# faris-k/self-supervised-wafermaps

Hardware: AMD Instinct MI355X
Metric: imgs/sec (SimCLR ResNet18, bs=256, 224^2) (higher is better)
Workload: dtype bf16; 1 GPU; SimCLR ResNet-18, 256 wafers/GPU/step, two 3x224x224 views, NT-Xent in-batch negatives, SGD (BASELINE.json configs[1]); per_gpu_batch=256, global_batch=256, parallelism=dp1, hip_graph=True, backward_stage_graphs=1, parallel_branches=two views through the backbone

## Files before the change

include/wafer_hip.h:

```cpp
#ifndef WAFER_HIP_H
#define WAFER_HIP_H

#include <stddef.h>
#include <stdint.h>

#ifdef __cplusplus
extern "C" {
#endif

#define WM_ABI_VERSION 4

#define WM_OK 0
#define WM_EINVAL (-1)
#define WM_EUNSUPPORTED (-2)
#define WM_EWORKSPACE (-3)
#define WM_EALIGN (-4)

#define WM_F32 0
#define WM_BF16 1

int wm_version(void);
const char* wm_error_string(int code);
int wm_fill_zero(void* p, size_t bytes, void* stream);
int wm_mean_f32(const float* x, long long n, float scale, int sqrt_of, float* out, void* stream);
// ... 8 lines not shown
#define WM_IMG_NCHW_F32 0
#define WM_IMG_NHWC_BF16 1
#define WM_IMG_HW_U8 2
#define WM_IMG_S2D_BF16 3

typedef struct WmViewParams {
  int32_t sample;
  int32_t out_slot;
  int32_t op;
  uint32_t noise_seed;
  float noise_p;
  int32_t dpw_h;
  int32_t dpw_w;
  int32_t rot90;
  int32_t vflip;
  int32_t hflip;
  int32_t crop;
  int32_t crop_i, crop_j, crop_h, crop_w;
  int32_t reserved;
} WmViewParams;

int wm_augment_views(const uint8_t* wafers, const int64_t* offsets, const int32_t* heights,
                     const int32_t* widths, int n_wafers, int max_wafer_elems,
                     const WmViewParams* params, int n_views, int img_size, int out_size,
                     int out_format, int normalize, float mean, float std, void* out,
                     void* stream);


size_t wm_knn_topk_workspace_bytes(int nq, int n, int d, int k);
int wm_knn_topk(const void* query, const void* bank, int nq, int n, int d, int dtype, int k,
                int bank_index_base, float* out_sim, int32_t* out_idx, void* workspace,
                size_t workspace_bytes, void* stream);

size_t wm_knn_topk_general_workspace_bytes(int nq, int n, int d, int k);
int wm_knn_topk_general(const float* query, const float* bank, const float* bias, int nq, int n, int d, int k,
                        int bank_index_base, float* out_sim, int32_t* out_idx, void* workspace,
                        size_t workspace_bytes, void* stream);
int wm_knn_topk_general_after(const float* query, const float* bank, const float* bias, int nq, int n, int d, int k,
                              int bank_index_base, const float* after_sim, const int32_t* after_idx, float* out_sim,
                              int32_t* out_idx, void* workspace, size_t workspace_bytes, void* stream);

int wm_knn_topk_many(const void* query, const void* bank, int nq, int n, int d, int dtype, int k, int bank_index_base,
                     float* out_sim, int32_t* out_idx, int batch, void* workspaces, size_t workspace_bytes_per_lane,
                     void* const* streams, int n_streams);

int wm_knn_merge(const float* in_sim, const int32_t* in_idx, int parts, int nq, int k,
                 float* out_sim, int32_t* out_idx, void* stream);

int wm_knn_vote(const float* sim, const int32_t* idx, const int64_t* bank_labels, long long n_labels, int nq, int k,
                int num_classes, float temperature, int64_t* pred_labels, float* scores,
                void* stream);

int wm_l2_normalize(const void* x, int in_dtype, int rows, int d, float eps, void* y,
                    int out_dtype, float* inv_norm, void* stream);
int wm_l2_normalize_bwd(const void* dy, int dy_dtype, const float* y, const float* inv_norm, int rows, int d,
                        void* dx, int out_dtype, const float* scale_dev, void* stream);

int wm_ntxent_fwd(const float* zn, const float* zall, int b_local, int b_global, int rank_offset,
                  int d, float temperature, float* lse, float* loss_rows, void* stream);
size_t wm_ntxent_bwd_workspace_bytes(int b_local, int b_global, int d);
int wm_ntxent_bwd(const float* zn, const float* zall, const float* lse_all, int b_local,
                  int b_global, int rank_offset, int d, float temperature, float grad_scale,
                  float* dzn, void* workspace, size_t workspace_bytes, void* stream);


int wm_conv2d_fwd(const void* x, const void* w_krsc, void* y, int N, int H, int W, int C, int K,
                  int R, int S, int P, int Q, int stride, int pad, void* stream);
int wm_conv2d_fwd_stats_tiles(int N, int H, int W, int C, int K, int R, int S, int P, int Q, int stride, int pad,
                              int rows_per_group);
int wm_conv2d_fwd_stats(const void* x, const void* w_krsc, void* y, int N, int H, int W, int C, int K,
                        int R, int S, int P, int Q, int stride, int pad, float* stat_part,
                        int stat_tiles, int rows_per_group, void* stream);
int wm_conv2d_dgrad(const void* dy, const void* w_crsk, void* dx, int N, int H, int W, int C, int K,
                    int R, int S, int P, int Q, int stride, int pad, void* stream);
int wm_conv2d_dgrad_add(const void* dy, const void* w_crsk, const void* residual, void* dx, int N, int H,
                        int W, int C, int K, int R, int S, int P, int Q, int stride, int pad, void* stream);
int wm_conv2d_dgrad_bnstat_ok(int N, int H, int W, int C, int K, int R, int S, int P, int Q, int stride, int pad,
                              int G);
int wm_conv2d_dgrad_bnstat(const void* dy, const void* w_crsk, const void* residual, void* dx, int N, int H, int W,
                           int C, int K, int R, int S, int P, int Q, int stride, int pad, const void* bn_y,
                           const void* relu_x, const void* relu_mask, const float* gamma, const float* beta,
                           const float* save_mean, const float* save_invstd, int G, float* stat_part, int stat_tiles,
                           void* stream);
int wm_conv2d_wgrad_splits(int N, int H, int W, int C, int K, int R, int S, int P, int Q, int stride, int pad);
int wm_conv2d_wgrad(const void* dy, const void* x, float* dw_slabs, int N, int H, int W, int C, int K,
                    int R, int S, int P, int Q, int stride, int pad, void* stream);
#define WM_ROUTE_F_STATS 1
#define WM_ROUTE_F_RESIDUAL 2
#define WM_ROUTE_F_BIAS 4
#define WM_ROUTE_F_BNB 8
#define WM_ROUTE_F_ACT 16
#define WM_ROUTE_PANEL 1
#define WM_ROUTE_STEM_PATCH 2
#define WM_ROUTE_WGRAD_PATCH64 3
#define WM_ROUTE_PATCH(MODE, BNB) (10 + 2 * (MODE) + ((BNB) ? 1 : 0))
#define WM_ROUTE_IGEMM(BN, CPT, MODE, EPI, BNB) \
  (10000 + ((BN) / 64) * 1000 + (CPT) * 100 + (MODE) * 10 + ((EPI) ? 2 : 0) + ((BNB) ? 1 : 0))
#define WM_ROUTE_WGRAD(BMO, CPT, NT, BIAS) (20000 + ((BMO) / 64) * 1000 + (CPT) * 100 + (NT) * 10 + ((BIAS) ? 1 : 0))
int wm_conv2d_route(int pass, int N, int H, int W, int C, int K, int R, int S, int P, int Q, int stride, int pad,
                    int flags, int group_arg);
int wm_conv2d_fwd_bias_res(const void* x, const void* w_krsc, const float* bias, const void* residual, void* y,
                           int N, int H, int W, int C, int K, int R, int S, int P, int Q, int stride, int pad,
                           void* stream);
int wm_conv2d_wgrad_bias(const void* dy, const void* x, float* dw_slabs, float* dbias_slabs, int N, int H, int W, int C,
                         int K, int R, int S, int P, int Q, int stride, int pad, void* stream);

int wm_linear_bias_gelu_fwd(const void* x, const void* w_krsc, const float* bias, void* pre_out, void* y, int rows,
                            int C, int K, void* stream);
int wm_linear_dgrad_gelu(const void* dy, const void* w_crsk, const void* pre, void* dx, int rows, int C, int K,
                         void* stream);

int wm_mlp_fused_fwd_ok(int rows, int C, int H);
int wm_mlp_fused_fwd(const void* x, const void* w1_krsc, const float* b1, const void* w2_krsc, const float* b2,
                     const void* residual, void* y, int rows, int C, int H, void* stream);
int wm_ln_linear_fwd_ok(int rows, int C, int N);
int wm_ln_linear_fwd(const void* x, const float* ln_gamma, const float* ln_beta, float ln_eps, const void* w_krsc,
                     const float* bias, void* y, int rows, int C, int N, void* stream);
int wm_ln_mlp_fused_fwd(const void* x, const float* ln_gamma, const float* ln_beta, float ln_eps, const void* w1_krsc,
                        const float* b1, const void* w2_krsc, const float* b2, const void* residual, void* y, int rows,
                        int C, int H, void* stream);

int wm_weights_prepare(const float* w_oihw, int K, int C, int R, int S, void* w_krsc, void* w_crsk,
                       void* stream);
typedef struct WmLayoutDesc {
  const float* w;
  uint16_t* krsc;
  uint16_t* crsk;
  float* ws;
  float* grad;
  int32_t K, C, RS, tiles_c, tile0, nsplit;
} WmLayoutDesc;
int wm_layouts_refresh(const WmLayoutDesc* descs_dev, int n_desc, int total_tiles, void* stream);
int wm_wgrad_fold(const WmLayoutDesc* descs_dev, int n_desc, int total_tiles, void* stream);

int wm_wgrad_finalize(const float* dw_slabs, int nsplit, int K, int C, int R, int S, float* grad_oihw,
                      int accumulate, void* stream);
int wm_stem_weights_prepare(const float* w_oihw, int K, void* w_s2d, void* stream);
int wm_stem_wgrad_finalize(const float* dw_s2d_slabs, int nsplit, int K, float* grad_oihw, int accumulate, void* stream);
int wm_image_to_s2d(const void* img, int fmt, int N, int H, int W, void* out, void* stream);
int wm_cast_f32_bf16(const float* x, long long n, void* y, void* stream);

size_t wm_bn_workspace_bytes(long long rows, int C, int G);
int wm_bn_train_fwd(const void* y, const void* residual, const float* gamma, const float* beta,
                    float* running_mean, float* running_var, long long* num_batches_tracked, long long rows, int C, int G, float eps,
                    float momentum, int relu, float* save_mean, float* save_invstd, void* out, void* relu_mask,
                    void* workspace, size_t workspace_bytes, void* stream);
int wm_bn_train_fwd_from_stats(const void* y, const void* residual, const float* gamma, const float* beta,
                               float* running_mean, float* running_var, long long* num_batches_tracked,
                               long long rows, int C, int G, float eps, float momentum, int relu, float* save_mean,
                               float* save_invstd,
                               void* out, void* relu_mask, const float* stat_part, int stat_tiles, void* workspace,
                               size_t workspace_bytes, void* stream);
int wm_bn_train_stats(const void* y, const float* gamma, const float* beta, float* running_mean,
                      float* running_var, long long* num_batches_tracked, long long rows, int C, int G, float eps, float momentum,
                      float* save_mean, float* save_invstd, float* scale, float* shift, const float* stat_part,
                      int stat_tiles, void* workspace, size_t workspace_bytes, void* stream);
int wm_bn_eval_scale_shift(const float* gamma, const float* beta, const float* running_mean,
                           const float* running_var, int C, float eps, float* scale, float* shift, void* stream);
int wm_bn_eval_fwd(const void* y, const void* residual, const float* gamma, const float* beta,
                   const float* running_mean, const float* running_var, long long rows, int C, float eps,
                   int relu, void* out, void* workspace, size_t workspace_bytes, void* stream);
int wm_bn_train_bwd(const void* y, const void* dout, const void* out_relu, int relu_from_y,
                    const float* gamma, const float* beta, const float* save_mean, const float* save_invstd,
                    long long rows, int C, int G, float* dgamma, float* dbeta, int accumulate, void* dy,
                    void* dz, void* workspace, size_t workspace_bytes, void* stream);
int wm_bn_train_bwd_from_stats(const void* y, const void* g, const float* gamma, const float* beta,
                               const float* save_mean, const float* save_invstd, long long rows, int C, int G,
                               float* dgamma, float* dbeta, int accumulate, void* dy, const float* stat_part,
                               int stat_tiles, void* workspace, size_t workspace_bytes, void* stream);
int wm_bn_sync_fwd_sums(const void* y, long long rows, int C, int G, const float* stat_part, int stat_tiles,
                        float* sums, void* workspace, size_t workspace_bytes, void* stream);
int wm_bn_sync_fwd_apply(const void* y, const void* residual, const float* gamma, const float* beta,
                         float* running_mean, float* running_var, long long* num_batches_tracked, long long rows, int C,
                         int G, long long group_count, float eps, float momentum, int relu, float* save_mean,
                         float* save_invstd, void* out, const float* sums, void* workspace, size_t workspace_bytes,
                         void* stream);
int wm_bn_sync_bwd_sums(const void* y, const void* dout, const void* out_relu, int relu_from_y, const float* gamma,
                        const float* beta, const float* save_mean, const float* save_invstd, long long rows, int C,
                        int G, float* dgamma, float* dbeta, int accumulate, float* sums, void* workspace,
                        size_t workspace_bytes, void* stream);
int wm_bn_sync_bwd_apply(const void* y, const void* dout, const void* out_relu, int relu_from_y, const float* gamma,
                         const float* beta, const float* save_mean, const float* save_invstd, long long rows, int C,
                         int G, long long group_count, const float* sums, void* dy, void* dz, void* workspace,
                         size_t workspace_bytes, void* stream);
int wm_bn_relu_maxpool_bwd(const void* y, const void* ysel, const void* pooled_dy, const void* pool_idx, int N,
                           int H, int W, int C, const float* gamma, const float* beta, const float* save_mean,
                           const float* save_invstd, int G, float* dgamma, float* dbeta, int accumulate,
                           void* dy, void* workspace, size_t workspace_bytes, void* stream);
int wm_add_bf16(const void* a, const void* b, long long n, void* out, void* stream);

int wm_maxpool3x3s2_fwd(const void* x, int N, int H, int W, int C, void* y, void* idx, void* stream);
int wm_bn_relu_maxpool3x3s2_fwd(const void* x, const float* scale, const float* shift, int N, int H, int W, int C,
                                int G, void* y, void* idx, void* xsel, void* stream);
int wm_maxpool3x3s2_bwd(const void* dy, const void* idx, int N, int H, int W, int C, void* dx, void* stream);
int wm_gap_fwd(const void* x, int N, int HW, int C, void* y, void* stream);
int wm_gap_bwd(const void* dy, int N, int HW, int C, void* dx, void* stream);

int wm_sgd_step(float* params, const float* grads, float* momentum_buf, long long n, const float* hyper,
                void* stream);

int wm_cross_entropy_fwd_bwd(const void* logits, int dtype, const long long* labels, const float* weight, int B, int C,
                             float* acc2, float* dlogits, void* stream);
int wm_bce_logits_fwd_bwd(const void* logits, int dtype, const float* target, const float* pos_weight, int B, int C,
                          float* loss, float* dlogits, void* stream);

int wm_neg_cosine_fwd_bwd(const void* x0, const void* x1, int dtype, int B, int D, float eps, float* loss, float* dx0,
                          float* dx1, void* stream);

size_t wm_dcl_workspace_bytes(int B);
int wm_dcl_fwd_bwd(const float* z0, const float* z1, int B, int D, float temperature, float sigma, int weighted,
                   float* loss, float* dz0, float* dz1, void* workspace, size_t workspace_bytes, void* stream);

int wm_barlow_twins_fwd_bwd(const float* raw_cc, int D, float scale, float lambda, float diag_weight, float* loss,
                            float* draw_cc, void* stream);
int wm_center_columns(const void* z, const float* mean, long long rows, int C, void* out, void* stream);
int wm_vicreg_variance(const float* var_biased, int N, int D, float eps, float* loss, float* coef, void* stream);

int wm_sinkhorn(const void* out, int dtype, int B, int K, float eps, int iters, float* Q, float* workspace,
                void* stream);

int wm_ntxent_bank_fwd_bwd(const float* q, const float* kpos, const float* bank, int B, int D, int K,
                           float temperature, float* loss, float* dq, float* dk, void* stream);


int wm_layernorm_fwd(const void* x, const float* gamma, const float* beta, float eps, long long rows, int C,
                     void* y, float* mean, float* rstd, void* stream);
int wm_layernorm_bwd(const void* x, const void* dy, const float* gamma, const float* mean, const float* rstd,
                     long long rows, int C, void* dx, float* dgamma, float* dbeta, void* stream);
int wm_layernorm_bwd_add(const void* x, const void* dy, const float* gamma, const float* mean, const float* rstd,
                         long long rows, int C, const void* dres, void* dx, float* dgamma, float* dbeta, void* stream);
int wm_colsum_blocks(long long rows, int C);
int wm_bias_act_bwd_parts(const void* x, const float* bias, const void* dy, int act, long long rows, int C, void* dx,
                          float* part, void* stream);
int wm_layernorm_bwd_blocks(long long rows, int C);
int wm_layernorm_bwd_parts(const void* x, const void* dy, const float* gamma, const float* mean, const float* rstd,
                           long long rows, int C, const void* dres, void* dx, float* part, void* stream);

#define WM_ACT_NONE 0
#define WM_ACT_GELU 1
#define WM_ACT_RELU 2
#define WM_ACT_MISH 3
int wm_bias_act_fwd(const void* x, const float* bias, const void* residual, int act, long long rows, int C,
                    void* y, void* stream);
int wm_bias_act_bwd(const void* x, const float* bias, const void* dy, int act, long long rows, int C, void* dx,
                    float* dbias, void* stream);
int wm_colsum_bf16(const void* x, long long rows, int C, float* out, int accumulate, void* stream);

int wm_tokens_assemble(const void* patches, const float* cls, const float* pos, int N, int np, int D, void* tokens,
                       void* stream);
int wm_patchify(const void* images, int N, int S, int p, void* rows, void* stream);

int wm_attention_fwd(const void* qkv, int B, int S, int H, int head_dim, float scale, void* out, float* lse,
// ... 157 lines not shown
```

self-supervised-wafermaps_amd/_lib.py:

```python
from __future__ import annotations

import ctypes
import os
from ctypes import c_char_p, c_double, c_float, c_int, c_int32, c_longlong, c_size_t, c_uint32, c_void_p
from pathlib import Path

_HERE = Path(__file__).resolve().parent
LIB_PATH = Path(os.environ["WM_HIP_LIB"]) if os.environ.get("WM_HIP_LIB") else _HERE / "libwafer_hip.so"

WM_F32, WM_BF16 = 0, 1
WM_AUG_NONE, WM_AUG_DIENOISE, WM_AUG_DPW, WM_AUG_MEDIAN3 = 0, 1, 2, 3
WM_IMG_NCHW_F32, WM_IMG_NHWC_BF16, WM_IMG_HW_U8, WM_IMG_S2D_BF16 = 0, 1, 2, 3


class WaferHipError(RuntimeError):
    pass


class WmViewParams(ctypes.Structure):

    _fields_ = [
        ("sample", c_int32),
        ("out_slot", c_int32),
        ("op", c_int32),
# ... 32 lines not shown
    "wm_f32_conv2d_dgrad": (c_int, [c_void_p, c_void_p, c_void_p, c_int, c_int, c_int, c_int, c_int, c_int, c_int, c_int, c_int,
                                    c_int, c_int, c_void_p, c_size_t, c_void_p]),
    "wm_f32_conv2d_wgrad_workspace_bytes": (c_size_t, [c_int] * 7),
    "wm_f32_conv2d_wgrad": (c_int, [c_void_p, c_void_p, c_void_p, c_int, c_int, c_int, c_int, c_int, c_int, c_int, c_int, c_int,
                                    c_int, c_int, c_void_p, c_size_t, c_void_p]),
    "wm_f32_colsum": (c_int, [c_void_p, c_longlong, c_int, c_void_p, c_void_p]),
    "wm_f32_bn_bwd": (c_int, [c_void_p, c_void_p, c_void_p, c_void_p, c_void_p, c_void_p, c_longlong, c_int, c_int, c_void_p,
                              c_void_p, c_void_p, c_void_p, c_void_p, c_size_t, c_void_p]),
    "wm_f32_maxpool3x3s2_bwd": (c_int, [c_void_p, c_void_p, c_int, c_int, c_int, c_int, c_void_p, c_void_p]),
    "wm_f32_gap_bwd": (c_int, [c_void_p, c_int, c_int, c_int, c_void_p, c_void_p]),
    "wm_f32_layernorm_bwd_workspace_bytes": (c_size_t, [c_longlong, c_int]),
    "wm_f32_layernorm_bwd": (c_int, [c_void_p, c_void_p, c_void_p, c_float, c_longlong, c_int, c_void_p, c_void_p, c_void_p,
                                     c_void_p, c_size_t, c_void_p]),
    "wm_f32_bias_act_bwd": (c_int, [c_void_p, c_void_p, c_void_p, c_int, c_longlong, c_int, c_void_p, c_void_p]),
    "wm_f32_attention_bwd": (c_int, [c_void_p, c_void_p, c_void_p, c_int, c_int, c_int, c_int, c_float, c_void_p, c_void_p]),
    "wm_f32_loss_bwd": (c_int, [c_void_p, c_void_p, c_longlong, c_int, c_double, c_void_p, c_void_p, c_void_p]),
    "wm_version": (c_int, []),
    "wm_error_string": (c_char_p, [c_int]),
    "wm_ln_linear_fwd_ok": (c_int, [c_int, c_int, c_int]),
    "wm_ln_linear_fwd": (c_int, [c_void_p, c_void_p, c_void_p, c_float, c_void_p, c_void_p, c_void_p, c_int, c_int, c_int, c_void_p]),
    "wm_ln_mlp_fused_fwd": (c_int, [c_void_p, c_void_p, c_void_p, c_float, c_void_p, c_void_p, c_void_p, c_void_p, c_void_p,
                                    c_void_p, c_int, c_int, c_int, c_void_p]),
    "wm_layernorm_bwd_blocks": (c_int, [c_longlong, c_int]),
    "wm_layernorm_bwd_parts": (c_int, [c_void_p, c_void_p, c_void_p, c_void_p, c_void_p, c_longlong, c_int, c_void_p, c_void_p,
                                       c_void_p, c_void_p]),
    "wm_colsum_blocks": (c_int, [c_longlong, c_int]),
    "wm_bias_act_bwd_parts": (c_int, [c_void_p, c_void_p, c_void_p, c_int, c_longlong, c_int, c_void_p, c_void_p, c_void_p]),
    "wm_scale_bf16": (c_int, [c_void_p, c_longlong, c_void_p, c_void_p, c_void_p]),
    "wm_fill_zero": (c_int, [c_void_p, c_size_t, c_void_p]),
    "wm_mean_f32": (c_int, [c_void_p, c_longlong, c_float, c_int, c_void_p, c_void_p]),
    "wm_augment_views": (
        c_int,
        [c_void_p, c_void_p, c_void_p, c_void_p, c_int, c_int, c_void_p, c_int, c_int, c_int, c_int,
         c_int, c_float, c_float, c_void_p, c_void_p],
    ),
    "wm_knn_topk_workspace_bytes": (c_size_t, [c_int, c_int, c_int, c_int]),
    "wm_knn_topk": (
        c_int,
        [c_void_p, c_void_p, c_int, c_int, c_int, c_int, c_int, c_int, c_void_p, c_void_p, c_void_p,
         c_size_t, c_void_p],
    ),
    "wm_knn_topk_many": (
        c_int,
        [c_void_p, c_void_p, c_int, c_int, c_int, c_int, c_int, c_int, c_void_p, c_void_p, c_int, c_void_p, c_size_t,
         c_void_p, c_int],
    ),
    "wm_knn_merge": (c_int, [c_void_p, c_void_p, c_int, c_int, c_int, c_void_p, c_void_p, c_void_p]),
    "wm_knn_vote": (
        c_int,
        [c_void_p, c_void_p, c_void_p, c_longlong, c_int, c_int, c_int, c_float, c_void_p, c_void_p, c_void_p],
    ),
    "wm_l2_normalize": (c_int, [c_void_p, c_int, c_int, c_int, c_float, c_void_p, c_int, c_void_p, c_void_p]),
    "wm_l2_normalize_bwd": (c_int, [c_void_p, c_int, c_void_p, c_void_p, c_int, c_int, c_void_p, c_int, c_void_p, c_void_p]),
    "wm_ntxent_fwd": (
        c_int,
        [c_void_p, c_void_p, c_int, c_int, c_int, c_int, c_float, c_void_p, c_void_p, c_void_p],
    ),
    "wm_ntxent_bwd_workspace_bytes": (c_size_t, [c_int, c_int, c_int]),
    "wm_ntxent_bwd": (
        c_int,
        [c_void_p, c_void_p, c_void_p, c_int, c_int, c_int, c_int, c_float, c_float, c_void_p, c_void_p, c_size_t,
         c_void_p],
    ),
    "wm_conv2d_fwd": (c_int, [c_void_p, c_void_p, c_void_p, c_int, c_int, c_int, c_int, c_int, c_int, c_int, c_int, c_int, c_int, c_int, c_void_p]),
    "wm_conv2d_fwd_stats": (c_int, [c_void_p, c_void_p, c_void_p, c_int, c_int, c_int, c_int, c_int, c_int, c_int, c_int, c_int, c_int, c_int, c_void_p, c_int, c_int, c_void_p]),
    "wm_conv2d_dgrad": (c_int, [c_void_p, c_void_p, c_void_p, c_int, c_int, c_int, c_int, c_int, c_int, c_int, c_int, c_int, c_int, c_int, c_void_p]),
    "wm_conv2d_dgrad_add": (c_int, [c_void_p, c_void_p, c_void_p, c_void_p, c_int, c_int, c_int, c_int, c_int, c_int, c_int, c_int, c_int, c_int, c_int, c_void_p]),
    "wm_conv2d_wgrad": (c_int, [c_void_p, c_void_p, c_void_p, c_int, c_int, c_int, c_int, c_int, c_int, c_int, c_int, c_int, c_int, c_int, c_void_p]),
    "wm_conv2d_fwd_bias_res": (c_int, [c_void_p, c_void_p, c_void_p, c_void_p, c_void_p, c_int, c_int, c_int, c_int, c_int,
                                       c_int, c_int, c_int, c_int, c_int, c_int, c_void_p]),
    "wm_conv2d_wgrad_bias": (c_int, [c_void_p, c_void_p, c_void_p, c_void_p, c_int, c_int, c_int, c_int, c_int, c_int, c_int,
                                     c_int, c_int, c_int, c_int, c_void_p]),
    "wm_weights_prepare": (c_int, [c_void_p, c_int, c_int, c_int, c_int, c_void_p, c_void_p, c_void_p]),
    "wm_wgrad_finalize": (c_int, [c_void_p, c_int, c_int, c_int, c_int, c_int, c_void_p, c_int, c_void_p]),
    "wm_conv2d_wgrad_splits": (c_int, [c_int] * 11),
    "wm_conv2d_route": (c_int, [c_int] * 14),
    "wm_mlp_fused_fwd_ok": (c_int, [c_int, c_int, c_int]),
    "wm_mlp_fused_fwd": (c_int, [c_void_p, c_void_p, c_void_p, c_void_p, c_void_p, c_void_p, c_void_p, c_int, c_int, c_int,
                                c_void_p]),
    "wm_conv2d_fwd_stats_tiles": (c_int, [c_int] * 12),
    "wm_conv2d_dgrad_bnstat_ok": (c_int, [c_int] * 12),
    "wm_conv2d_dgrad_bnstat": (c_int, [c_void_p, c_void_p, c_void_p, c_void_p] + [c_int] * 11 +
                               [c_void_p, c_void_p, c_void_p, c_void_p, c_void_p, c_void_p, c_void_p, c_int, c_void_p, c_int, c_void_p]),
    "wm_bn_train_bwd_from_stats": (
        c_int,
        [c_void_p, c_void_p, c_void_p, c_void_p, c_void_p, c_void_p, c_longlong, c_int, c_int, c_void_p, c_void_p, c_int,
         c_void_p, c_void_p, c_int, c_void_p, c_size_t, c_void_p],
    ),
    "wm_bn_sync_fwd_sums": (c_int, [c_void_p, c_longlong, c_int, c_int, c_void_p, c_int, c_void_p, c_void_p, c_size_t, c_void_p]),
    "wm_bn_sync_fwd_apply": (
        c_int,
        [c_void_p, c_void_p, c_void_p, c_void_p, c_void_p, c_void_p, c_void_p, c_longlong, c_int, c_int, c_longlong,
         c_float, c_float, c_int, c_void_p, c_void_p, c_void_p, c_void_p, c_void_p, c_size_t, c_void_p],
    ),
    "wm_bn_sync_bwd_sums": (
        c_int,
        [c_void_p, c_void_p, c_void_p, c_int, c_void_p, c_void_p, c_void_p, c_void_p, c_longlong, c_int, c_int,
         c_void_p, c_void_p, c_int, c_void_p, c_void_p, c_size_t, c_void_p],
    ),
    "wm_bn_sync_bwd_apply": (
        c_int,
        [c_void_p, c_void_p, c_void_p, c_int, c_void_p, c_void_p, c_void_p, c_void_p, c_longlong, c_int, c_int,
         c_longlong, c_void_p, c_void_p, c_void_p, c_void_p, c_size_t, c_void_p],
    ),
    "wm_stem_weights_prepare": (c_int, [c_void_p, c_int, c_void_p, c_void_p]),
    "wm_stem_wgrad_finalize": (c_int, [c_void_p, c_int, c_int, c_void_p, c_int, c_void_p]),
    "wm_image_to_s2d": (c_int, [c_void_p, c_int, c_int, c_int, c_int, c_void_p, c_void_p]),
    "wm_cast_f32_bf16": (c_int, [c_void_p, c_longlong, c_void_p, c_void_p]),
    "wm_bn_workspace_bytes": (c_size_t, [c_longlong, c_int, c_int]),
    "wm_bn_train_fwd": (
        c_int,
        [c_void_p, c_void_p, c_void_p, c_void_p, c_void_p, c_void_p, c_void_p, c_longlong, c_int, c_int, c_float, c_float,
         c_int, c_void_p, c_void_p, c_void_p, c_void_p, c_void_p, c_size_t, c_void_p],
    ),
    "wm_bn_train_fwd_from_stats": (
        c_int,
        [c_void_p, c_void_p, c_void_p, c_void_p, c_void_p, c_void_p, c_void_p, c_longlong, c_int, c_int, c_float, c_float,
         c_int, c_void_p, c_void_p, c_void_p, c_void_p, c_void_p, c_int, c_void_p, c_size_t, c_void_p],
    ),
    "wm_bn_train_stats": (
        c_int,
        [c_void_p, c_void_p, c_void_p, c_void_p, c_void_p, c_void_p, c_longlong, c_int, c_int, c_float, c_float, c_void_p,
         c_void_p, c_void_p, c_void_p, c_void_p, c_int, c_void_p, c_size_t, c_void_p],
    ),
    "wm_bn_eval_scale_shift": (c_int, [c_void_p, c_void_p, c_void_p, c_void_p, c_int, c_float, c_void_p, c_void_p, c_void_p]),
    "wm_bn_eval_fwd": (
        c_int,
        [c_void_p, c_void_p, c_void_p, c_void_p, c_void_p, c_void_p, c_longlong, c_int, c_float, c_int, c_void_p,
         c_void_p, c_size_t, c_void_p],
    ),
    "wm_bn_train_bwd": (
        c_int,
        [c_void_p, c_void_p, c_void_p, c_int, c_void_p, c_void_p, c_void_p, c_void_p, c_longlong, c_int, c_int,
         c_void_p, c_void_p, c_int, c_void_p, c_void_p, c_void_p, c_size_t, c_void_p],
    ),
    "wm_bn_relu_maxpool_bwd": (
        c_int,
        [c_void_p, c_void_p, c_void_p, c_void_p, c_int, c_int, c_int, c_int, c_void_p, c_void_p, c_void_p, c_void_p, c_int,
         c_void_p, c_void_p, c_int, c_void_p, c_void_p, c_size_t, c_void_p],
    ),
    "wm_add_bf16": (c_int, [c_void_p, c_void_p, c_longlong, c_void_p, c_void_p]),
    "wm_maxpool3x3s2_fwd": (c_int, [c_void_p, c_int, c_int, c_int, c_int, c_void_p, c_void_p, c_void_p]),
    "wm_bn_relu_maxpool3x3s2_fwd": (
        c_int, [c_void_p, c_void_p, c_void_p, c_int, c_int, c_int, c_int, c_int, c_void_p, c_void_p, c_void_p, c_void_p]),
    "wm_maxpool3x3s2_bwd": (c_int, [c_void_p, c_void_p, c_int, c_int, c_int, c_int, c_void_p, c_void_p]),
    "wm_gap_fwd": (c_int, [c_void_p, c_int, c_int, c_int, c_void_p, c_void_p]),
    "wm_gap_bwd": (c_int, [c_void_p, c_int, c_int, c_int, c_void_p, c_void_p]),
    "wm_sgd_step": (c_int, [c_void_p, c_void_p, c_void_p, c_longlong, c_void_p, c_void_p]),
    "wm_cross_entropy_fwd_bwd": (c_int, [c_void_p, c_int, c_void_p, c_void_p, c_int, c_int, c_void_p, c_void_p, c_void_p]),
    "wm_bce_logits_fwd_bwd": (c_int, [c_void_p, c_int, c_void_p, c_void_p, c_int, c_int, c_void_p, c_void_p, c_void_p]),
    "wm_neg_cosine_fwd_bwd": (c_int, [c_void_p, c_void_p, c_int, c_int, c_int, c_float, c_void_p, c_void_p, c_void_p,
                                      c_void_p]),
    "wm_barlow_twins_fwd_bwd": (c_int, [c_void_p, c_int, c_float, c_float, c_float, c_void_p, c_void_p, c_void_p]),
    "wm_center_columns": (c_int, [c_void_p, c_void_p, c_longlong, c_int, c_void_p, c_void_p]),
    "wm_vicreg_variance": (c_int, [c_void_p, c_int, c_int, c_float, c_void_p, c_void_p, c_void_p]),
    "wm_lars_step": (c_int, [c_void_p, c_void_p, c_void_p, c_void_p, c_int, c_void_p, c_void_p, c_void_p]),
    "wm_sinkhorn": (c_int, [c_void_p, c_int, c_int, c_int, c_float, c_int, c_void_p, c_void_p, c_void_p]),
    "wm_dcl_workspace_bytes": (c_size_t, [c_int]),
    "wm_dcl_fwd_bwd": (c_int, [c_void_p, c_void_p, c_int, c_int, c_float, c_float, c_int, c_void_p, c_void_p, c_void_p,
                               c_void_p, c_size_t, c_void_p]),
    "wm_ntxent_bank_fwd_bwd": (c_int, [c_void_p, c_void_p, c_void_p, c_int, c_int, c_int, c_float, c_void_p, c_void_p,
                                       c_void_p, c_void_p]),
    "wm_layernorm_fwd": (c_int, [c_void_p, c_void_p, c_void_p, c_float, c_longlong, c_int, c_void_p, c_void_p, c_void_p,
                                 c_void_p]),
    "wm_layernorm_bwd": (c_int, [c_void_p, c_void_p, c_void_p, c_void_p, c_void_p, c_longlong, c_int, c_void_p, c_void_p,
                                 c_void_p, c_void_p]),
    "wm_layernorm_bwd_add": (c_int, [c_void_p, c_void_p, c_void_p, c_void_p, c_void_p, c_longlong, c_int, c_void_p,
                                     c_void_p, c_void_p, c_void_p, c_void_p]),
    "wm_bias_act_fwd": (c_int, [c_void_p, c_void_p, c_void_p, c_int, c_longlong, c_int, c_void_p, c_void_p]),
    "wm_bias_act_bwd": (c_int, [c_void_p, c_void_p, c_void_p, c_int, c_longlong, c_int, c_void_p, c_void_p, c_void_p]),
# ... 145 lines not shown
```

self-supervised-wafermaps_amd/csrc/bn.hip:

```cpp
#include "common.h"

namespace {

constexpr int BN_THREADS = 256;

__device__ __forceinline__ void unpack8(const uint4 v, float (&f)[8]) {
  f[0] = bf2f((uint16_t)(v.x & 0xffff)); f[1] = bf2f((uint16_t)(v.x >> 16));
  f[2] = bf2f((uint16_t)(v.y & 0xffff)); f[3] = bf2f((uint16_t)(v.y >> 16));
  f[4] = bf2f((uint16_t)(v.z & 0xffff)); f[5] = bf2f((uint16_t)(v.z >> 16));
  f[6] = bf2f((uint16_t)(v.w & 0xffff)); f[7] = bf2f((uint16_t)(v.w >> 16));
}
__device__ __forceinline__ uint4 pack8(const float (&f)[8]) {
  return make_uint4(pack_bf2(f[0], f[1]), pack_bf2(f[2], f[3]), pack_bf2(f[4], f[5]), pack_bf2(f[6], f[7]));
}

struct PoolSrc {
  const uint16_t* dy;
  const uint8_t* idx;
  int H, W, P, Q;
};

__device__ __forceinline__ void pool_grad8(const PoolSrc& ps, uint32_t row, int C, int c0, float (&g)[8]) {
  const uint32_t hw = (uint32_t)(ps.H * ps.W);
  const int n = (int)(row / hw);
// ... 246 lines not shown
  }
  if (owner) {
    if (running_mean) running_mean[c] = rm;
    if (running_var) running_var[c] = rv;
  }
}

__global__ __launch_bounds__(1024) void bn_sums_finalize(float* __restrict__ part, int nblk, int G, int C,
                                                          float* __restrict__ sums) {
  __shared__ double red[2][2][32][33];
  const int bl = threadIdx.x >> 5, cl = threadIdx.x & 31;
  const int c = blockIdx.x * 32 + cl;
  const bool owner = bl == 0 && c < C;
  for (int g0 = 0; g0 < G; g0 += 2) {
    const int ng = G - g0 < 2 ? G - g0 : 2;
    double a[2], b[2];
    finalize_sums2(part, nblk, g0, ng, C, c, bl, cl, red, a, b);
    if (owner) {
      for (int u = 0; u < ng; ++u) {
        sums[((size_t)(g0 + u) * 2 + 0) * C + c] = (float)a[u];
        sums[((size_t)(g0 + u) * 2 + 1) * C + c] = (float)b[u];
      }
    }
  }
}

__global__ void bn_eval_params(const float* __restrict__ gamma, const float* __restrict__ beta,
                               const float* __restrict__ running_mean,
                               const float* __restrict__ running_var, float eps, int C,
                               float* __restrict__ scale, float* __restrict__ shift) {
  for (int c = threadIdx.x; c < C; c += blockDim.x) {
    const float is = 1.0f / sqrtf(running_var[c] + eps);
    const float sc = (gamma ? gamma[c] : 1.f) * is;
    scale[c] = sc;
    shift[c] = (beta ? beta[c] : 0.f) - running_mean[c] * sc;
  }
}

template <bool POW2>
__global__ __launch_bounds__(BN_THREADS) void bn_apply(const uint16_t* __restrict__ y,
                                                       const uint16_t* __restrict__ residual,
                                                       const float* __restrict__ scale,
                                                       const float* __restrict__ shift,
                                                       long long rows, int C, int rows_per_group,
                                                       int relu, int cshift, uint16_t* __restrict__ out,
                                                       uint8_t* __restrict__ relu_mask) {
  const int cpr = C >> 3;
  const long long total = rows * cpr;
  int cur_g = -1;
  float sc[8], sh[8];
  for (long long p = (long long)blockIdx.x * BN_THREADS + threadIdx.x; p < total;
       p += (long long)gridDim.x * BN_THREADS) {
    long long row;
    int c0, g;
    if (POW2) {
      row = p >> cshift;
      c0 = (int)(p & (cpr - 1)) * 8;
      g = 0;
      for (long long lim = rows_per_group; row >= lim; lim += rows_per_group) ++g;
    } else {
      row = p / cpr;
      c0 = (int)(p - row * cpr) * 8;
      g = (int)(row / rows_per_group);
    }
    if (!POW2 || g != cur_g) {
      const float4 sa = *reinterpret_cast<const float4*>(scale + (size_t)g * C + c0);
      const float4 sb = *reinterpret_cast<const float4*>(scale + (size_t)g * C + c0 + 4);
      const float4 ha = *reinterpret_cast<const float4*>(shift + (size_t)g * C + c0);
      const float4 hb = *reinterpret_cast<const float4*>(shift + (size_t)g * C + c0 + 4);
      sc[0] = sa.x; sc[1] = sa.y; sc[2] = sa.z; sc[3] = sa.w; sc[4] = sb.x; sc[5] = sb.y; sc[6] = sb.z; sc[7] = sb.w;
      sh[0] = ha.x; sh[1] = ha.y; sh[2] = ha.z; sh[3] = ha.w; sh[4] = hb.x; sh[5] = hb.y; sh[6] = hb.z; sh[7] = hb.w;
      cur_g = g;
    }
    float f[8];
    unpack8(*reinterpret_cast<const uint4*>(y + row * C + c0), f);
#pragma unroll
    for (int e = 0; e < 8; ++e) f[e] = fmaf(f[e], sc[e], sh[e]);
    if (residual) {
      float r[8];
      unpack8(*reinterpret_cast<const uint4*>(residual + row * C + c0), r);
#pragma unroll
      for (int e = 0; e < 8; ++e) f[e] += r[e];
    }
    if (relu) {
#pragma unroll
      for (int e = 0; e < 8; ++e) f[e] = fmaxf(f[e], 0.f);
    }
    const uint4 pk = pack8(f);
    *reinterpret_cast<uint4*>(out + row * C + c0) = pk;
    if (relu_mask != nullptr) {
      float r8[8];
      unpack8(pk, r8);
      uint32_t m = 0;
#pragma unroll
      for (int e = 0; e < 8; ++e) m |= (r8[e] > 0.f ? 1u : 0u) << e;
      relu_mask[row * cpr + (c0 >> 3)] = (uint8_t)m;
    }
  }
}

__global__ __launch_bounds__(1024) void bn_bwd_finalize(
    float* __restrict__ part, int nblk, int G, int C, int rows_per_group,
    const float* __restrict__ gamma, const float* __restrict__ beta, const float* __restrict__ mean,
    const float* __restrict__ invstd, float* __restrict__ dgamma, float* __restrict__ dbeta, int accumulate,
    float* __restrict__ coef, int fx) {
  __shared__ double red[2][2][32][33];
  const int bl = threadIdx.x >> 5, cl = threadIdx.x & 31;
  const int c = blockIdx.x * 32 + cl;
  const bool owner = bl == 0 && c < C;
  double tg = 0.0, tb = 0.0;
  for (int g0 = 0; g0 < G; g0 += 2) {
    const int ng = G - g0 < 2 ? G - g0 : 2;
    double s1v[2], s2v[2];
    finalize_sums2(part, nblk, g0, ng, C, c, bl, cl, red, s1v, s2v);
    if (owner) {
      for (int u = 0; u < ng; ++u) {
        const int g = g0 + u;
        double s1 = s1v[u], s2 = s2v[u];
        if (fx) {
          s2 = (double)invstd[(size_t)g * C + c] * s2;
        }
        tb += s1;
        tg += s2;
        const float is = invstd[(size_t)g * C + c];
        const float mu = mean[(size_t)g * C + c];
        const float sc = (gamma ? gamma[c] : 1.f) * is;
        coef[((size_t)g * 7 + 0) * C + c] = mu;
        coef[((size_t)g * 7 + 1) * C + c] = is;
        coef[((size_t)g * 7 + 2) * C + c] = sc;
        coef[((size_t)g * 7 + 3) * C + c] = (float)(s1 / rows_per_group);
        coef[((size_t)g * 7 + 4) * C + c] = (float)(s2 / rows_per_group);
        coef[((size_t)g * 7 + 5) * C + c] = sc;
        coef[((size_t)g * 7 + 6) * C + c] = (beta ? beta[c] : 0.f) - mu * sc;
      }
    }
  }
  if (owner) {
    if (dgamma) dgamma[c] = (accumulate ? dgamma[c] : 0.f) + (float)tg;
    if (dbeta) dbeta[c] = (accumulate ? dbeta[c] : 0.f) + (float)tb;
  }
}

template <bool POW2, int FORM>
__global__ __launch_bounds__(BN_THREADS, FORM == 0 ? 4 : 1) void bn_bwd_apply(const uint16_t* __restrict__ y,
                                                           const uint16_t* __restrict__ dout,
                                                           const uint16_t* __restrict__ out,
                                                           const float* __restrict__ coef,
                                                           long long rows, int C, int rows_per_group,
                                                           int remask, int cshift, uint16_t* __restrict__ dy,
                                                           uint16_t* __restrict__ dz, const PoolSrc ps) {
  const int cpr = C >> 3;
  const long long total = rows * cpr;
  int cur_g = -1;
  constexpr int NK = FORM == 0 ? 5 : 7;
  float k[NK][8];
  for (long long p = (long long)blockIdx.x * BN_THREADS + threadIdx.x; p < total;
       p += (long long)gridDim.x * BN_THREADS) {
    long long row;
    int c0, g;
    if (POW2) {
      row = p >> cshift;
      c0 = (int)(p & (cpr - 1)) * 8;
      g = 0;
      for (long long lim = rows_per_group; row >= lim; lim += rows_per_group) ++g;
    } else {
      row = p / cpr;
      c0 = (int)(p - row * cpr) * 8;
      g = (int)(row / rows_per_group);
    }
    if (!POW2 || g != cur_g) {
      const float* cf = coef + (size_t)g * 7 * C + c0;
#pragma unroll
      for (int t = 0; t < NK; ++t) {
        const float4 a = *reinterpret_cast<const float4*>(cf + (size_t)t * C);
        const float4 b = *reinterpret_cast<const float4*>(cf + (size_t)t * C + 4);
        k[t][0] = a.x; k[t][1] = a.y; k[t][2] = a.z; k[t][3] = a.w;
        k[t][4] = b.x; k[t][5] = b.y; k[t][6] = b.z; k[t][7] = b.w;
      }
      cur_g = g;
    }
    const size_t off = row * C + c0;
    float fy[8], fd[8];
    unpack8(*reinterpret_cast<const uint4*>(y + off), fy);
    if constexpr (FORM == 2) pool_grad8(ps, (uint32_t)row, C, c0, fd);
    else unpack8(*reinterpret_cast<const uint4*>(dout + off), fd);
    if constexpr (FORM != 0) {
      if (out) {
        float fo[8];
        unpack8(*reinterpret_cast<const uint4*>(out + off), fo);
#pragma unroll
        for (int e = 0; e < 8; ++e) fd[e] = fo[e] > 0.f ? fd[e] : 0.f;
      }
      if (!out && remask) {
#pragma unroll
        for (int e = 0; e < 8; ++e) fd[e] = bf2f(f2bf(fmaf(fy[e], k[NK - 2][e], k[NK - 1][e]))) > 0.f ? fd[e] : 0.f;
      }
      if (dz) *reinterpret_cast<uint4*>(dz + off) = pack8(fd);
    }
    float r[8];
#pragma unroll
    for (int e = 0; e < 8; ++e) {
      const float xh = (fy[e] - k[0][e]) * k[1][e];
      r[e] = k[2][e] * (fd[e] - k[3][e] - xh * k[4][e]);
    }
    *reinterpret_cast<uint4*>(dy + off) = pack8(r);
  }
}

__global__ __launch_bounds__(BN_THREADS) void bn_pool_bwd_apply(const uint16_t* __restrict__ y,
                                                                const float* __restrict__ coef, int n_coef, int N, int C,
                                                                int imgs_per_group, int remask,
                                                                uint16_t* __restrict__ dy, const PoolSrc ps,
                                                                const WmDiv d_cpr, const WmDiv d_wb, const WmDiv d_ha,
                                                                const WmDiv d_ipg) {
  const uint32_t cpr = (uint32_t)C >> 3;
  const uint32_t HA = (uint32_t)ps.H >> 1, WB = (uint32_t)ps.W >> 1;
  const uint32_t total = (uint32_t)N * HA * WB * cpr;
  extern __shared__ __attribute__((aligned(16))) float pool_coef[];
  for (int i = threadIdx.x; i < n_coef; i += BN_THREADS) pool_coef[i] = coef[i];
  __syncthreads();
  for (uint32_t t = blockIdx.x * BN_THREADS + threadIdx.x; t < total; t += gridDim.x * BN_THREADS) {
    uint32_t rc, rb, ra;
    uint32_t u = wm_divmod(t, d_cpr, rc);
    const int c0 = (int)rc * 8;
    u = wm_divmod(u, d_wb, rb);
    const int n = (int)wm_divmod(u, d_ha, ra);
    const int b = (int)rb, a = (int)ra;
    const int g = (int)wm_div((uint32_t)n, d_ipg);
    const float* kk = pool_coef + (size_t)g * 7 * C + c0;
    auto krow = [&](int q, float (&v)[8]) {
      const float4 lo = *reinterpret_cast<const float4*>(kk + q * C);
      const float4 hi = *reinterpret_cast<const float4*>(kk + q * C + 4);
      v[0] = lo.x; v[1] = lo.y; v[2] = lo.z; v[3] = lo.w; v[4] = hi.x; v[5] = hi.y; v[6] = hi.z; v[7] = hi.w;
    };
    uint2 pk[4];
    uint4 dv[4];
    bool wok[4];
#pragma unroll
    for (int j = 0; j < 4; ++j) {
      const int p = a + (j >> 1), q = b + (j & 1);
      wok[j] = p < ps.P && q < ps.Q;
      const int pc = p < ps.P ? p : ps.P - 1, qc = q < ps.Q ? q : ps.Q - 1;
      const size_t o = ((size_t)(n * ps.P + pc) * ps.Q + qc) * C + c0;
      pk[j] = *reinterpret_cast<const uint2*>(ps.idx + o);
      dv[j] = *reinterpret_cast<const uint4*>(ps.dy + o);
    }
    float dw[4][8];
#pragma unroll
    for (int j = 0; j < 4; ++j) unpack8(dv[j], dw[j]);
#pragma unroll
    for (int pix = 0; pix < 4; ++pix) {
      const int dh = pix >> 1, dwp = pix & 1;
      float fd[8];
#pragma unroll
      for (int e = 0; e < 8; ++e) fd[e] = 0.f;
#pragma unroll
      for (int j = 0; j < 4; ++j) {
        const int kh = dh + 1 - 2 * (j >> 1), kw = dwp + 1 - 2 * (j & 1);
        if (kh < 0 || kw < 0) continue;
        const int code = kh * 3 + kw;
        if (wok[j]) {
#pragma unroll
          for (int e = 0; e < 8; ++e) {
            const int ie = (int)(((e < 4 ? pk[j].x : pk[j].y) >> (8 * (e & 3))) & 0xff);
            fd[e] += ie == code ? dw[j][e] : 0.f;
          }
        }
      }
#pragma unroll
      for (int e = 0; e < 8; ++e) fd[e] = bf2f(f2bf(fd[e]));
      const size_t off = ((size_t)(n * ps.H + 2 * a + dh) * ps.W + 2 * b + dwp) * C + c0;
      float fy[8];
      unpack8(*reinterpret_cast<const uint4*>(y + off), fy);
      if (remask) {
        float k5[8], k6[8];
        krow(5, k5);
        krow(6, k6);
#pragma unroll
        for (int e = 0; e < 8; ++e) fd[e] = bf2f(f2bf(fmaf(fy[e], k5[e], k6[e]))) > 0.f ? fd[e] : 0.f;
      }
      float r[8], k0[8], k1[8];
      krow(0, k0);
      krow(1, k1);
#pragma unroll
      for (int e = 0; e < 8; ++e) r[e] = (fy[e] - k0[e]) * k1[e];
      krow(4, k0);
      krow(3, k1);
#pragma unroll
      for (int e = 0; e < 8; ++e) r[e] = fd[e] - k1[e] - r[e] * k0[e];
      krow(2, k0);
#pragma unroll
// ... 28 lines not shown

constexpr int STAT_SLOTS_DIRECT = 512, STAT_SLOTS_REDUCED = 128;
inline size_t stat_scratch_floats(int T, int G, int C) {
  return T > STAT_SLOTS_DIRECT ? (size_t)G * STAT_SLOTS_REDUCED * 2 * C : 0;
}

inline const float* stat_partials(const float* stat_part, int T, int G, int C, float* scratch, int* nblk, hipStream_t st) {
  if (T <= STAT_SLOTS_DIRECT) {
    *nblk = T;
    return stat_part;
  }
  int R = 1;
  while ((T + R - 1) / R > STAT_SLOTS_REDUCED) R *= 2;
  const int To = (T + R - 1) / R;
  const long long total = (long long)G * To * 2 * C;
  stats_prereduce<<<wm_cdiv(total, BN_THREADS), BN_THREADS, 0, st>>>(stat_part, T, R, To, G * 2 * C, 2 * C, scratch);
  *nblk = To;
  return scratch;
}

inline bool chunk_pow2(int C, int* shift) {
  const int cpr = C >> 3;
  if (cpr <= 0 || (cpr & (cpr - 1)) || BN_THREADS % cpr) return false;
  int sft = 0;
  while ((1 << sft) < cpr) ++sft;
  *shift = sft;
  return true;
}

__global__ __launch_bounds__(BN_THREADS) void add_bf16_kernel(const uint16_t* __restrict__ a,
                                                              const uint16_t* __restrict__ b,
                                                              long long n8, uint16_t* __restrict__ o) {
  for (long long p = (long long)blockIdx.x * BN_THREADS + threadIdx.x; p < n8;
       p += (long long)gridDim.x * BN_THREADS) {
    float fa[8], fb[8];
    unpack8(reinterpret_cast<const uint4*>(a)[p], fa);
    unpack8(reinterpret_cast<const uint4*>(b)[p], fb);
#pragma unroll
    for (int e = 0; e < 8; ++e) fa[e] += fb[e];
    reinterpret_cast<uint4*>(o)[p] = pack8(fa);
  }
}

inline int reduce_blocks(int rows_per_group, int C) {
  const int tpr = C >> 3;
  const int rpp = BN_THREADS / tpr > 0 ? BN_THREADS / tpr : 1;
  int nblk = wm_cdiv(rows_per_group, rpp * 16);
  if (nblk > 256) nblk = 256;
  if (nblk < 1) nblk = 1;
  return nblk;
}

inline int stream_grid(long long items) {
  long long b = (items + BN_THREADS - 1) / BN_THREADS;
  if (b > 256 * 16) b = 256 * 16;
  if (b < 1) b = 1;
  return (int)b;
}

inline const uint16_t* bf16(const void* p) { return static_cast<const uint16_t*>(p); }
inline uint16_t* bf16(void* p) { return static_cast<uint16_t*>(p); }

inline void launch_bn_apply(const uint16_t* y, const uint16_t* residual, const float* scale, const float* shift,
                            long long rows, int C, int rpg, int relu, uint16_t* out, hipStream_t st,
                            uint8_t* relu_mask = nullptr) {
  int csh = 0;
  const auto kernel = chunk_pow2(C, &csh) ? bn_apply<true> : bn_apply<false>;
  kernel<<<stream_grid(rows * (C >> 3)), BN_THREADS, 0, st>>>(y, residual, scale, shift, rows, C, rpg, relu, csh, out,
                                                              relu_mask);
}

inline void launch_bn_bwd_apply(int form, const uint16_t* y, const uint16_t* dout, const uint16_t* out_relu,
                                const float* coef, long long rows, int C, int rpg, bool remask, uint16_t* dy, uint16_t* dz,
                                const PoolSrc& ps, hipStream_t st) {
  int csh = 0;
  const bool pow2 = chunk_pow2(C, &csh);
  const auto kernel = form == 0   ? (pow2 ? bn_bwd_apply<true, 0> : bn_bwd_apply<false, 0>)
                      : form == 1 ? (pow2 ? bn_bwd_apply<true, 1> : bn_bwd_apply<false, 1>)
                                  : (pow2 ? bn_bwd_apply<true, 2> : bn_bwd_apply<false, 2>);
  kernel<<<stream_grid(rows * (C >> 3)), BN_THREADS, 0, st>>>(y, dout, out_relu, coef, rows, C, rpg, remask ? 1 : 0, csh, dy,
                                                              dz, ps);
}

constexpr int BN_WIDE_MAX_C = 16384;

__global__ __launch_bounds__(BN_THREADS) void bn_col_fwd(const uint16_t* __restrict__ y, const uint16_t* __restrict__ res,
                                                         const float* __restrict__ gamma, const float* __restrict__ beta,
                                                         float* __restrict__ rmean, float* __restrict__ rvar,
                                                         long long* __restrict__ num_batches_tracked, int rpg,
                                                         int C, int G, float eps, float momentum, int relu, int training,
                                                         float* __restrict__ save_mean, float* __restrict__ save_invstd,
                                                         uint16_t* __restrict__ out) {
  const int c = blockIdx.x * BN_THREADS + threadIdx.x;
  if (training && num_batches_tracked != nullptr && c == 0)
    atomicAdd(reinterpret_cast<unsigned long long*>(num_batches_tracked), (unsigned long long)G);
  if (c >= C) return;
  const float ga = gamma ? gamma[c] : 1.f, be = beta ? beta[c] : 0.f;
  for (int g = 0; g < G; ++g) {
    const size_t base = (size_t)g * rpg;
    float mu, is;
    if (training) {
      float s = 0.f;
      for (int r = 0; r < rpg; ++r) s += bf2f(y[(base + r) * C + c]);
      mu = s / (float)rpg;
      float q = 0.f;
      for (int r = 0; r < rpg; ++r) {
        const float d = bf2f(y[(base + r) * C + c]) - mu;
        q = fmaf(d, d, q);
      }
      const float var = q / (float)rpg;
      is = rsqrtf(var + eps);
      save_mean[(size_t)g * C + c] = mu;
      save_invstd[(size_t)g * C + c] = is;
      if (rmean) {
        rmean[c] = (1.f - momentum) * rmean[c] + momentum * mu;
        rvar[c] = (1.f - momentum) * rvar[c] + momentum * (rpg > 1 ? var * (float)rpg / (float)(rpg - 1) : var);
      }
    } else {
      mu = rmean[c];
      is = rsqrtf(rvar[c] + eps);
    }
    const float sc = ga * is, sh = be - mu * sc;
    for (int r = 0; r < rpg; ++r) {
      const size_t o = (base + r) * C + c;
      float v = fmaf(bf2f(y[o]), sc, sh);
      if (res) v += bf2f(res[o]);
      if (relu) v = fmaxf(v, 0.f);
      out[o] = f2bf(v);
    }
  }
}

__global__ __launch_bounds__(BN_THREADS) void bn_col_bwd(const uint16_t* __restrict__ y, const uint16_t* __restrict__ dout,
                                                         const uint16_t* __restrict__ out_relu, int remask,
                                                         const float* __restrict__ gamma, const float* __restrict__ beta,
                                                         const float* __restrict__ mean, const float* __restrict__ invstd,
                                                         int rpg, int C, int G, float* __restrict__ dgamma,
                                                         float* __restrict__ dbeta, int accumulate,
                                                         uint16_t* __restrict__ dy, uint16_t* __restrict__ dz) {
  const int c = blockIdx.x * BN_THREADS + threadIdx.x;
  if (c >= C) return;
  const float ga = gamma ? gamma[c] : 1.f, be = beta ? beta[c] : 0.f;
  float dg = 0.f, db = 0.f;
  for (int g = 0; g < G; ++g) {
    const size_t base = (size_t)g * rpg;
    const float mu = mean[(size_t)g * C + c], is = invstd[(size_t)g * C + c];
    const float sc = ga * is, sh = be - mu * sc;
    float s1 = 0.f, s2 = 0.f;
    for (int r = 0; r < rpg; ++r) {
      const size_t o = (base + r) * C + c;
      const float yv = bf2f(y[o]);
      float d = bf2f(dout[o]);
      if (out_relu) d = bf2f(out_relu[o]) > 0.f ? d : 0.f;
      else if (remask) d = bf2f(f2bf(fmaf(yv, sc, sh))) > 0.f ? d : 0.f;
      s1 += d;
      s2 = fmaf(d, (yv - mu) * is, s2);
    }
    dg += s2;
    db += s1;
    const float c1 = s1 / (float)rpg, c2 = s2 / (float)rpg;
    for (int r = 0; r < rpg; ++r) {
      const size_t o = (base + r) * C + c;
      const float yv = bf2f(y[o]);
      float d = bf2f(dout[o]);
      if (out_relu) d = bf2f(out_relu[o]) > 0.f ? d : 0.f;
      else if (remask) d = bf2f(f2bf(fmaf(yv, sc, sh))) > 0.f ? d : 0.f;
// ... 219 lines not shown
                           stream);
}

extern "C" int wm_bn_train_stats(const void* y, const float* gamma, const float* beta, float* running_mean,
                                 float* running_var, long long* num_batches_tracked, long long rows, int C, int G, float eps, float momentum,
                                 float* save_mean, float* save_invstd, float* scale, float* shift, const float* stat_part,
                                 int stat_tiles, void* workspace, size_t workspace_bytes, void* stream) {
  WM_REQUIRE(y && save_mean && save_invstd && scale && shift && workspace, WM_EINVAL);
  const int rc = bn_shape_check(rows, C, G);
  if (rc != WM_OK) return rc;
  WM_REQUIRE(!stat_part || stat_tiles > 0, WM_EINVAL);
  WM_REQUIRE(workspace_bytes >= fwd_partials_bytes(stat_part, stat_tiles, rows, C, G), WM_EWORKSPACE);
  return bn_fwd_stats(bf16(y), stat_part, stat_tiles, gamma, beta, running_mean, running_var, num_batches_tracked,
                      (int)(rows / G), C, G, eps, momentum, save_mean, save_invstd, scale, shift,
                      static_cast<float*>(workspace), static_cast<hipStream_t>(stream));
}

extern "C" int wm_bn_eval_scale_shift(const float* gamma, const float* beta, const float* running_mean,
                                      const float* running_var, int C, float eps, float* scale, float* shift,
                                      void* stream) {
  WM_REQUIRE(running_mean && running_var && scale && shift && C > 0, WM_EINVAL);
  launch_eval_params(gamma, beta, running_mean, running_var, eps, C, scale, shift, static_cast<hipStream_t>(stream));
  WM_LAUNCH_CHECK();
  return WM_OK;
}

extern "C" int wm_bn_eval_fwd(const void* y_, const void* residual, const float* gamma, const float* beta,
                              const float* running_mean, const float* running_var, long long rows, int C,
                              float eps, int relu, void* out_, void* workspace, size_t workspace_bytes,
                              void* stream) {
  WM_REQUIRE(y_ && out_ && running_mean && running_var && workspace, WM_EINVAL);
  const int rc = bn_shape_check(rows, C, 1);
  if (rc != WM_OK) return rc;
  WM_REQUIRE(workspace_bytes >= (size_t)2 * C * sizeof(float), WM_EWORKSPACE);
  hipStream_t st = static_cast<hipStream_t>(stream);
  const uint16_t *y = bf16(y_), *res = bf16(residual);
  uint16_t* out = bf16(out_);
  if (bn_wide(rows, C, 1)) {
    bn_col_fwd<<<wm_cdiv(C, BN_THREADS), BN_THREADS, 0, st>>>(y, res, gamma, beta, const_cast<float*>(running_mean),
                                                              const_cast<float*>(running_var), nullptr, (int)rows, C, 1, eps,
                                                              0.f, relu, 0, nullptr, nullptr, out);
    WM_LAUNCH_CHECK();
    return WM_OK;
  }
  float* scale = static_cast<float*>(workspace);
  float* shift = scale + C;
  launch_eval_params(gamma, beta, running_mean, running_var, eps, C, scale, shift, st);
  WM_LAUNCH_CHECK();
  launch_bn_apply(y, res, scale, shift, rows, C, (int)(rows < (1ll << 31) - 1 ? rows : (1ll << 31) - 1), relu, out, st);
  WM_LAUNCH_CHECK();
  return WM_OK;
}

extern "C" int wm_bn_train_bwd(const void* y, const void* dout, const void* out_relu, int relu_from_y,
                               const float* gamma, const float* beta, const float* save_mean,
                               const float* save_invstd, long long rows, int C, int G, float* dgamma,
                               float* dbeta, int accumulate, void* dy, void* dz, void* workspace,
                               size_t workspace_bytes, void* stream) {
  WM_REQUIRE(dout, WM_EINVAL);
  return bn_bwd_impl(y, dout, out_relu, relu_from_y, gamma, beta, save_mean, save_invstd, rows, C, G, dgamma, dbeta,
                     accumulate, dy, dz, workspace, workspace_bytes, stream, PoolSrc{}, nullptr);
}

extern "C" int wm_bn_train_bwd_from_stats(const void* y, const void* g, const float* gamma, const float* beta,
                                          const float* save_mean, const float* save_invstd, long long rows, int C,
                                          int G, float* dgamma, float* dbeta, int accumulate, void* dy,
                                          const float* stat_part, int stat_tiles, void* workspace,
                                          size_t workspace_bytes, void* stream) {
  WM_REQUIRE(y && g && save_mean && save_invstd && dy && stat_part && workspace && stat_tiles > 0, WM_EINVAL);
  const int rc = bn_shape_check(rows, C, G);
  if (rc != WM_OK) return rc;
  WM_REQUIRE(!bn_wide(rows, C, G), WM_EUNSUPPORTED);
  WM_REQUIRE(workspace_bytes >= ((size_t)7 * G * C + stat_scratch_floats(stat_tiles, G, C)) * sizeof(float), WM_EWORKSPACE);
  hipStream_t st = static_cast<hipStream_t>(stream);
  const int rpg = (int)(rows / G);
  float* coef = static_cast<float*>(workspace);
  int nblk = 0;
  const float* part = stat_partials(stat_part, stat_tiles, G, C, coef + (size_t)7 * G * C, &nblk, st);
  WM_LAUNCH_CHECK();
  launch_finalize(bn_bwd_finalize, C, st, part, nblk, G, C, rpg, gamma, beta, save_mean, save_invstd, dgamma, dbeta, accumulate,
                  coef, 1);
  WM_LAUNCH_CHECK();
  launch_bn_bwd_apply(0, bf16(y), bf16(g), nullptr, coef, rows, C, rpg, false, bf16(dy), nullptr, PoolSrc{}, st);
  WM_LAUNCH_CHECK();
  return WM_OK;
}

extern "C" int wm_bn_relu_maxpool_bwd(const void* y, const void* ysel, const void* pooled_dy, const void* pool_idx,
                                      int N, int H, int W, int C, const float* gamma, const float* beta,
                                      const float* save_mean,
                                      const float* save_invstd, int G, float* dgamma, float* dbeta, int accumulate,
                                      void* dy, void* workspace, size_t workspace_bytes, void* stream) {
  WM_REQUIRE(pooled_dy && pool_idx && gamma && beta, WM_EINVAL);
  WM_REQUIRE(N > 0 && H > 1 && W > 1 && (long long)N * H * W < (1ll << 31), WM_EINVAL);
  PoolSrc ps;
  ps.dy = bf16(pooled_dy);
  ps.idx = static_cast<const uint8_t*>(pool_idx);
  ps.H = H; ps.W = W; ps.P = (H + 2 - 3) / 2 + 1; ps.Q = (W + 2 - 3) / 2 + 1;
  return bn_bwd_impl(y, nullptr, nullptr, 1, gamma, beta, save_mean, save_invstd, (long long)N * H * W, C, G, dgamma,
                     dbeta, accumulate, dy, nullptr, workspace, workspace_bytes, stream, ps, ysel);
}

extern "C" int wm_bn_sync_fwd_sums(const void* y, long long rows, int C, int G, const float* stat_part, int stat_tiles,
                                   float* sums, void* workspace, size_t workspace_bytes, void* stream) {
  WM_REQUIRE(y && sums && workspace, WM_EINVAL);
  const int rc = bn_shape_check(rows, C, G);
  if (rc != WM_OK) return rc;
  hipStream_t st = static_cast<hipStream_t>(stream);
  const int rpg = (int)(rows / G);
  if (bn_wide(rows, C, G)) {
    bn_col_sums<0><<<wm_cdiv(C, BN_THREADS), BN_THREADS, 0, st>>>(bf16(y), nullptr, nullptr, 0, nullptr, nullptr, nullptr,
                                                                 nullptr, rpg, C, G, sums);
    WM_LAUNCH_CHECK();
    return WM_OK;
  }
  WM_REQUIRE(!stat_part || stat_tiles > 0, WM_EINVAL);
  WM_REQUIRE(workspace_bytes >= fwd_partials_bytes(stat_part, stat_tiles, rows, C, G), WM_EWORKSPACE);
  int nblk = 0;
  const float* part = fwd_partials(bf16(y), stat_part, stat_tiles, rpg, C, G, static_cast<float*>(workspace), &nblk, st);
  WM_LAUNCH_CHECK();
  launch_finalize(bn_sums_finalize, C, st, part, nblk, G, C, sums);
  WM_LAUNCH_CHECK();
  return WM_OK;
}

extern "C" int wm_bn_sync_fwd_apply(const void* y, const void* residual, const float* gamma, const float* beta,
                                    float* running_mean, float* running_var, long long* num_batches_tracked,
                                    long long rows, int C, int G, long long group_count, float eps, float momentum,
                                    int relu, float* save_mean, float* save_invstd, void* out, const float* sums,
                                    void* workspace, size_t workspace_bytes, void* stream) {
  WM_REQUIRE(y && out && save_mean && save_invstd && sums && workspace, WM_EINVAL);
  const int rc = bn_shape_check(rows, C, G);
  if (rc != WM_OK) return rc;
  WM_REQUIRE(group_count >= rows / G && group_count < (1ll << 31), WM_EINVAL);
  WM_REQUIRE(workspace_bytes >= (size_t)2 * G * C * sizeof(float), WM_EWORKSPACE);
  hipStream_t st = static_cast<hipStream_t>(stream);
  float* scale = static_cast<float*>(workspace);
  float* shift = scale + (size_t)G * C;
  launch_finalize(bn_fwd_finalize, C, st, sums, 1, G, C, (int)group_count, 0, gamma, beta, eps, momentum, running_mean,
                  running_var, num_batches_tracked, save_mean, save_invstd, scale, shift);
  WM_LAUNCH_CHECK();
  launch_bn_apply(bf16(y), bf16(residual), scale, shift, rows, C, (int)(rows / G), relu, bf16(out), st);
  WM_LAUNCH_CHECK();
  return WM_OK;
}

extern "C" int wm_bn_sync_bwd_sums(const void* y_, const void* dout_, const void* out_relu_, int relu_from_y,
                                   const float* gamma, const float* beta, const float* save_mean,
                                   const float* save_invstd, long long rows, int C, int G, float* dgamma, float* dbeta,
                                   int accumulate, float* sums, void* workspace, size_t workspace_bytes, void* stream) {
  WM_REQUIRE(y_ && dout_ && save_mean && save_invstd && sums && workspace, WM_EINVAL);
  const int rc = bn_shape_check(rows, C, G);
  if (rc != WM_OK) return rc;
  WM_REQUIRE(workspace_bytes >= wm_bn_workspace_bytes(rows, C, G), WM_EWORKSPACE);
  hipStream_t st = static_cast<hipStream_t>(stream);
  const uint16_t *y = bf16(y_), *dout = bf16(dout_), *out_relu = bf16(out_relu_);
  const int rpg = (int)(rows / G);
  const int nblk = reduce_blocks(rpg, C);
  float* part = static_cast<float*>(workspace);
  float* coef = part + (size_t)G * nblk * 2 * C;
  const bool remask = relu_remask(relu_from_y, out_relu);
  WM_REQUIRE(!remask || (gamma && beta), WM_EINVAL);
  if (bn_wide(rows, C, G)) {
    bn_col_sums<1><<<wm_cdiv(C, BN_THREADS), BN_THREADS, 0, st>>>(y, dout, out_relu, remask ? 1 : 0, gamma, beta, save_mean,
                                                                 save_invstd, rpg, C, G, sums);
    WM_LAUNCH_CHECK();
// ... 46 lines not shown
```

self-supervised-wafermaps_amd/csrc/conv.hip:

```cpp
#include "common.h"
#include "panel.h"
#include <stdlib.h>

namespace {

#ifndef WM_CONV_ABLATE
#define WM_CONV_ABLATE 0
#endif

constexpr int CV_THREADS = 256;
constexpr int CV_ROW = 128;

struct ConvArgs {
  const uint16_t* src;
  const uint16_t* wt;
  uint16_t* dst;
  int N, SH, SW, SC, DH, DW, DC, R, S, stride, pad, M, nkt;
  float* stat;
  int stat_nb, stat_rpg;
  const uint16_t* bn_y;
  const uint16_t* bn_x;
  const uint8_t* bn_mask;
  const float* bn_mean;
  const float* bn_invstd;
  const float* bn_gamma;
  const float* bn_beta;
  const uint16_t* res;
  const float* bias;
  const uint16_t* pre_in;
  uint16_t* pre_out;
  int act;
  WmDiv d_dhw, d_dw, d_h2w2, d_w2;
  int xcd;
};

__device__ __forceinline__ float cv_gelu(float v) { return wm_gelu(v); }
__device__ __forceinline__ float cv_gelu_grad(float v) { return wm_gelu_grad(v); }

__device__ __attribute__((aligned(256))) uint16_t conv_zero_page[128];

struct ClassRow {
  int n, h2, w2;
};
__device__ __forceinline__ ClassRow class_row(const ConvArgs& a, int m) {
  uint32_t urem2, uw2;
  const int n = (int)wm_divmod((uint32_t)m, a.d_h2w2, urem2);
  const int h2 = (int)wm_divmod(urem2, a.d_w2, uw2);
  return {n, h2, (int)uw2};
}

template <typename F>
__device__ __forceinline__ uint4 bf16x8_map(uint4 v, F f) {
  const uint32_t vv[4] = {v.x, v.y, v.z, v.w};
  uint32_t o[4];
#pragma unroll
  for (int q = 0; q < 4; ++q)
    o[q] = pack_bf2(f(2 * q, bf2f((uint16_t)(vv[q] & 0xffff))), f(2 * q + 1, bf2f((uint16_t)(vv[q] >> 16))));
  return make_uint4(o[0], o[1], o[2], o[3]);
}
template <typename F>
__device__ __forceinline__ uint4 bf16x8_zip(uint4 v, uint4 r, F f) {
  const uint32_t rr[4] = {r.x, r.y, r.z, r.w};
  return bf16x8_map(v, [&](int e, float x) {
    return f(x, bf2f((uint16_t)((e & 1) ? rr[e >> 1] >> 16 : rr[e >> 1] & 0xffff)));
  });
}
__device__ __forceinline__ uint4 bf16x8_add(uint4 v, uint4 r) {
  return bf16x8_zip(v, r, [](float x, float y) { return x + y; });
}

__device__ __forceinline__ void stage_acc_frag(uint8_t* tile, int CS, f32x4_t acc, int pix, int ch) {
  const uint2 v = make_uint2(pack_bf2(acc[0], acc[1]), pack_bf2(acc[2], acc[3]));
  *reinterpret_cast<uint2*>(tile + pix * CS + ch * 2) = v;
}

__device__ __forceinline__ size_t pair_origin(const ConvArgs& a, int n, int h0, int w0) {
  return ((size_t)n * a.DH + h0) * a.DW + w0;
}
__device__ __forceinline__ size_t pair_pixel(const size_t (&org)[2], int row, int DW) {
  return org[row >> 6] + (size_t)((row >> 3) & 7) * DW + (row & 7);
}

struct StatSlot {
  int g, t;
};
__device__ __forceinline__ int stat_tile(const ConvArgs& a, int g, int row0) { return (row0 - g * a.stat_rpg) / 128; }
__device__ __forceinline__ StatSlot stat_slot(const ConvArgs& a, int row0, int t0 = 0) {
  const int g = row0 / a.stat_rpg;
  return {g, t0 + stat_tile(a, g, row0)};
}
__device__ __forceinline__ StatSlot stat_slot_pair(const ConvArgs& a, int n0, int pair) {
  const int g = (int)(((long long)n0 * a.DH * a.DW) / a.stat_rpg);
  return {g, pair - g * (a.stat_rpg >> 7)};
}
__device__ __forceinline__ float* stat_slot_ptr(const ConvArgs& a, int idx, int DC) { return a.stat + ((size_t)idx * 2) * DC; }
__device__ __forceinline__ float* stat_slot_ptr(const ConvArgs& a, StatSlot s, int DC) {
  return stat_slot_ptr(a, s.g * a.stat_nb + s.t, DC);
}
__device__ __forceinline__ float* stat_slot_ptr_row(const ConvArgs& a, int row0, int DC) {
  const int g = row0 / a.stat_rpg;
  return stat_slot_ptr(a, g * a.stat_nb + stat_tile(a, g, row0), DC);
}

template <int CPR>
__device__ __forceinline__ float strided_lane_sum(float v) {
  static_assert(CPR == 8 || CPR == 16, "chunk columns per row");
  if constexpr (CPR == 8) v += wm_dpp<0x128>(v);
  v = wm_xor16_sum(v);
  v = wm_xor32_sum(v);
  return v;
}
template <int BNC>
__device__ __forceinline__ void block_colsums_store(float (&s1)[8], float (&s2)[8], float* red, float* slot, int DC,
                                                    int c_base, int tid) {
  constexpr int CPR = BNC / 8;
  const int lane = tid & 63, wave = tid >> 6;
#pragma unroll
  for (int e = 0; e < 8; ++e) {
    s1[e] = strided_lane_sum<CPR>(s1[e]);
    s2[e] = strided_lane_sum<CPR>(s2[e]);
  }
  if (lane < CPR) {
#pragma unroll
    for (int e = 0; e < 8; ++e) {
      red[wave * BNC + lane * 8 + e] = s1[e];
      red[(4 + wave) * BNC + lane * 8 + e] = s2[e];
    }
  }
  __syncthreads();
  if (tid < 2 * BNC) {
    const int which = tid / BNC, cc = tid % BNC;
    const float* r = red + (size_t)which * 4 * BNC + cc;
    slot[(size_t)which * DC + c_base + cc] = ((r[0] + r[BNC]) + r[2 * BNC]) + r[3 * BNC];
  }
}

template <int BNC, typename PixOf>
__device__ __forceinline__ void store_tile_with_stats(const uint8_t* smem, int CS, uint16_t* dst, int DC, int n0, float* red,
                                                      float* slot, int tid, PixOf pix_of) {
  constexpr int CPR = BNC / 8;
  constexpr int NIT = 128 * CPR / CV_THREADS;
  const int chl = tid % CPR;
  float s1[8], s2[8];
#pragma unroll
  for (int e = 0; e < 8; ++e) s1[e] = s2[e] = 0.f;
#pragma unroll
  for (int it = 0; it < NIT; ++it) {
    const int row = (tid + it * CV_THREADS) / CPR;
    const uint4 v = *reinterpret_cast<const uint4*>(smem + row * CS + chl * 16);
    const uint32_t vv[4] = {v.x, v.y, v.z, v.w};
#pragma unroll
    for (int q = 0; q < 4; ++q) {
      const float lo = __builtin_bit_cast(float, vv[q] << 16), hi = __builtin_bit_cast(float, vv[q] & 0xffff0000u);
      s1[2 * q] += lo;
      s2[2 * q] = fmaf(lo, lo, s2[2 * q]);
      s1[2 * q + 1] += hi;
      s2[2 * q + 1] = fmaf(hi, hi, s2[2 * q + 1]);
    }
    *reinterpret_cast<uint4*>(dst + pix_of(row) * DC + n0 + chl * 8) = v;
  }
  block_colsums_store<BNC>(s1, s2, red, slot, DC, n0, tid);
}

typedef __attribute__((ext_vector_type(4))) unsigned int u32x4_t;
template <int BNC>
struct BnbRegs {
  static constexpr int NIT = 128 * (BNC / 8) / CV_THREADS;
  u32x4_t yv[NIT], rv[NIT], xv[NIT];
  uint32_t mk[NIT];
  size_t pixs[NIT];
};
__device__ __forceinline__ void bnb_load16(u32x4_t& dst, const void* p) {
  dst = __builtin_nontemporal_load(reinterpret_cast<const u32x4_t*>(p));
}
template <int BNC, typename PixOf>
__device__ __forceinline__ void bnb_prefetch(const ConvArgs& a, BnbRegs<BNC>& R, int n0, int tid, PixOf pix_of) {
  constexpr int CPR = BNC / 8;
  const int c0 = n0 + (tid % CPR) * 8;
#pragma unroll
  for (int it = 0; it < BnbRegs<BNC>::NIT; ++it) {
    const int row = (tid + it * CV_THREADS) / CPR;
    const size_t pix = pix_of(row);
    R.pixs[it] = pix;
    bnb_load16(R.yv[it], a.bn_y + pix * a.DC + c0);
    if (a.res != nullptr) bnb_load16(R.rv[it], a.res + pix * a.DC + c0);
    if (a.bn_x != nullptr) bnb_load16(R.xv[it], a.bn_x + pix * a.DC + c0);
    R.mk[it] = a.bn_mask != nullptr ? a.bn_mask[pix * (a.DC >> 3) + (c0 >> 3)] : 0u;
  }
}

template <int BNC>
__device__ __forceinline__ void bnb_epilogue(const ConvArgs& a, const BnbRegs<BNC>& R, const uint8_t* smem, int CS, float* red,
                                             StatSlot slot, int n0, int tid) {
  constexpr int CPR = BNC / 8;
  constexpr int NIT = BnbRegs<BNC>::NIT;
  const int chl = tid % CPR;
  const int c0 = n0 + chl * 8;
  const bool remask = a.bn_x == nullptr && a.bn_mask == nullptr;
  const bool bitmask = a.bn_mask != nullptr;
  float sc[8], sh[8], mu[8];
  const int g = slot.g;
  const float* pm = a.bn_mean + (size_t)g * a.DC + c0;
#pragma unroll
  for (int e = 0; e < 8; ++e) {
    sc[e] = sh[e] = 0.f;
    mu[e] = pm[e];
  }
  if (remask) {
    const float* pi = a.bn_invstd + (size_t)g * a.DC + c0;
#pragma unroll
    for (int e = 0; e < 8; ++e) {
      sc[e] = a.bn_gamma[c0 + e] * pi[e];
      sh[e] = a.bn_beta[c0 + e] - mu[e] * sc[e];
    }
  }
  float s1[8], s2[8];
#pragma unroll
  for (int e = 0; e < 8; ++e) s1[e] = s2[e] = 0.f;
#pragma unroll
  for (int it = 0; it < NIT; ++it) {
    const int row = (tid + it * CV_THREADS) / CPR;
    const uint4 v4 = *reinterpret_cast<const uint4*>(smem + row * CS + chl * 16);
    const uint32_t vv[4] = {v4.x, v4.y, v4.z, v4.w};
    const uint32_t rr[4] = {R.rv[it][0], R.rv[it][1], R.rv[it][2], R.rv[it][3]};
    const uint32_t yy[4] = {R.yv[it][0], R.yv[it][1], R.yv[it][2], R.yv[it][3]};
    const uint32_t xx[4] = {R.xv[it][0], R.xv[it][1], R.xv[it][2], R.xv[it][3]};
    uint32_t o[4];
#pragma unroll
    for (int q = 0; q < 4; ++q) {
      float gv[2];
#pragma unroll
      for (int h = 0; h < 2; ++h) {
        const int e = q * 2 + h;
        float v = __builtin_bit_cast(float, h ? (vv[q] & 0xffff0000u) : (vv[q] << 16));
        if (a.res != nullptr) v += __builtin_bit_cast(float, h ? (rr[q] & 0xffff0000u) : (rr[q] << 16));
        const float y = __builtin_bit_cast(float, h ? (yy[q] & 0xffff0000u) : (yy[q] << 16));
        const bool keep = remask ? fmaf(y, sc[e], sh[e]) > 0.f
                          : bitmask ? ((R.mk[it] >> e) & 1u) != 0u
                                    : __builtin_bit_cast(float, h ? (xx[q] & 0xffff0000u) : (xx[q] << 16)) > 0.f;
        v = keep ? v : 0.f;
        s1[e] += v;
        s2[e] = fmaf(v, y - mu[e], s2[e]);
        gv[h] = v;
      }
      o[q] = pack_bf2(gv[0], gv[1]);
    }
    *reinterpret_cast<uint4*>(a.dst + R.pixs[it] * a.DC + c0) = make_uint4(o[0], o[1], o[2], o[3]);
  }
  block_colsums_store<BNC>(s1, s2, red, stat_slot_ptr(a, slot, a.DC), a.DC, n0, tid);
}

template <int BM, int BN, int CPT, int MODE, bool EPI = false, bool BNB = false>
__global__ __launch_bounds__(CV_THREADS) void conv_igemm(const ConvArgs a) {
  constexpr bool DGRAD = MODE != 0;
  static_assert(!BNB || (DGRAD && !EPI && BM == 128), "BatchNorm-backward epilogue: dgrad tiles of 128 rows");
  extern __shared__ __attribute__((aligned(16))) uint8_t cv_smem[];
  static_assert(BM == 128, "2 x 2 waves of 64 pixels");
  constexpr int A_BYTES = BM * CV_ROW;
  constexpr int B_BYTES = BN * CV_ROW;
  constexpr int STAGE = A_BYTES + B_BYTES;
  constexpr int NR = BM / 32;
  constexpr int NB = BN / 32;
  constexpr int NJ = BN / 2 / 16;

  const int tid = threadIdx.x, lane = tid & 63;
  const int wave = __builtin_amdgcn_readfirstlane(tid >> 6);
  const int wm = wave >> 1, wn = wave & 1;
  int bm = blockIdx.x, bn = blockIdx.y;
  if (a.xcd) {
    const uint32_t lin = wm_xcd_swizzle(blockIdx.x + gridDim.x * blockIdx.y, gridDim.x * gridDim.y);
    bm = (int)(lin / gridDim.y);
    bn = (int)(lin - (uint32_t)bm * gridDim.y);
    if constexpr (MODE == 2) {
      const int tpc = (int)(gridDim.x >> 2);
      if (a.xcd == 3 && (gridDim.x & 3) == 0) bm = (bm & 3) * tpc + (bm >> 2);
      else { bm = blockIdx.x; bn = blockIdx.y; }
    }
  }
  const int m0 = bm * BM, n0 = bn * BN;
  auto row_pixel = [&](int row) -> size_t {
    if constexpr (MODE == 2) {
      const int cls = a.M >> 2;
      const int pc = m0 / cls;
      const ClassRow c = class_row(a, m0 + row - pc * cls);
      return ((size_t)c.n * a.DH + 2 * c.h2 + (pc >> 1)) * a.DW + 2 * c.w2 + (pc & 1);
    } else {
      return (size_t)(m0 + row);
    }
  };
  const int rowl = tid >> 3;
  const int chunk = (tid & 7) ^ (rowl & 7);

  int bh[NR], bw[NR], nb[NR];
  bool mv[NR];
  const uint16_t* p0[NR];
  int r0 = 0, s0 = 0, nr = 0, ns = 0, nkt = a.nkt;
  if constexpr (MODE == 2) {
    const int cls = a.M >> 2;
    const int pc = m0 / cls;
    const int ph = pc >> 1, pw = pc & 1;
    r0 = (ph + a.pad) & 1;
    s0 = (pw + a.pad) & 1;
    nr = r0 < a.R ? (a.R - r0 + 1) >> 1 : 0;
    ns = s0 < a.S ? (a.S - s0 + 1) >> 1 : 0;
    nkt = nr * ns * (a.SC >> 6);
#pragma unroll
    for (int i = 0; i < NR; ++i) {
      const ClassRow c = class_row(a, m0 + rowl + 32 * i - pc * cls);
      mv[i] = true;
      bh[i] = c.h2 + ((ph + a.pad - r0) >> 1);
      bw[i] = c.w2 + ((pw + a.pad - s0) >> 1);
      nb[i] = c.n * a.SH * a.SW;
      p0[i] = a.src + ((long long)(nb[i] + bh[i] * a.SW + bw[i]) * a.SC + chunk * 8);
    }
  } else {
#pragma unroll
    for (int i = 0; i < NR; ++i) {
      const int m = m0 + rowl + 32 * i;
      mv[i] = m < a.M;
      const int mm = mv[i] ? m : 0;
      uint32_t urem, udw;
      const int n = (int)wm_divmod((uint32_t)mm, a.d_dhw, urem);
      const int dh = (int)wm_divmod(urem, a.d_dw, udw), dw = (int)udw;
      if constexpr (!DGRAD) {
        bh[i] = dh * a.stride - a.pad;
        bw[i] = dw * a.stride - a.pad;
      } else {
        bh[i] = dh + a.pad;
        bw[i] = dw + a.pad;
      }
      nb[i] = n * a.SH * a.SW;
      p0[i] = a.src + ((long long)(nb[i] + bh[i] * a.SW + bw[i]) * a.SC + chunk * 8);
    }
  }
  const size_t wrow = (size_t)a.R * a.S * a.SC;
  const uint16_t* pb[NB];
#pragma unroll
  for (int i = 0; i < NB; ++i) pb[i] = a.wt + (size_t)(n0 + rowl + 32 * i) * wrow + chunk * 8;

  int it_c0 = 0, it_r = 0, it_s = 0;
  const uint32_t smem_base = lds_addr(cv_smem);
  auto issue = [&](int kt, uint32_t stage) {
    int r, s;
    long long koff;
    const int c0 = it_c0;
    if constexpr (MODE == 2) {
      const int jr = it_r, js = it_s;
      it_c0 += 64;
      if (it_c0 == a.SC) {
        it_c0 = 0;
        if (++it_s == ns) {
          it_s = 0;
          ++it_r;
        }
      }
      r = jr;
      s = js;
      koff = (long long)(-jr * a.SW - js) * a.SC + c0;
#pragma unroll
      for (int i = 0; i < NR; ++i) {
        const int sh = bh[i] - jr, sw = bw[i] - js;
        const bool ok = (unsigned)sh < (unsigned)a.SH && (unsigned)sw < (unsigned)a.SW;
        const uint16_t* src = ok ? p0[i] + koff : conv_zero_page + chunk * 8;
        glds16_at(src, stage + (wave * 8 + 32 * i) * CV_ROW);
      }
      const size_t wk = ((size_t)((r0 + 2 * jr) * a.S + (s0 + 2 * js)) * a.SC) + c0;
#pragma unroll
      for (int i = 0; i < NB; ++i)
        glds16_at(pb[i] + wk, stage + A_BYTES + (wave * 8 + 32 * i) * CV_ROW);
      return;
    } else if constexpr (CPT == 8) {
      r = it_r;
      s = it_s;
      it_c0 += 64;
      if (it_c0 == a.SC) {
        it_c0 = 0;
        if (++it_s == a.S) {
          it_s = 0;
          ++it_r;
        }
      }
      koff = DGRAD ? ((long long)(-r * a.SW - s) * a.SC + c0) : ((long long)(r * a.SW + s) * a.SC + c0);
    } else {
      r = kt;
      s = chunk >> 1;
      koff = (long long)r * a.SW * a.SC;
    }
#pragma unroll
    for (int i = 0; i < NR; ++i) {
      bool ok = mv[i];
      const uint16_t* src;
      if constexpr (!DGRAD) {
        const int sh = bh[i] + r, sw = bw[i] + s;
        ok = ok && (unsigned)sh < (unsigned)a.SH && (unsigned)sw < (unsigned)a.SW;
        src = p0[i] + koff;
      } else {
        const int th = bh[i] - r, tw = bw[i] - s;
        ok = ok && th >= 0 && tw >= 0;
        if (MODE == 1 && a.stride == 2) {
          ok = ok && (((th | tw) & 1) == 0);
          const int sh = th >> 1, sw = tw >> 1;
          ok = ok && sh < a.SH && sw < a.SW;
          src = a.src + ((long long)(nb[i] + sh * a.SW + sw) * a.SC + c0 + chunk * 8);
        } else {
          ok = ok && th < a.SH && tw < a.SW;
          src = p0[i] + koff;
        }
      }
      if (!ok) src = conv_zero_page + chunk * 8;
      glds16_at(src, stage + (wave * 8 + 32 * i) * CV_ROW);
    }
#pragma unroll
    for (int i = 0; i < NB; ++i)
      glds16_at(pb[i] + (size_t)kt * 64, stage + A_BYTES + (wave * 8 + 32 * i) * CV_ROW);
  };

  f32x4_t acc[NJ][4];
#pragma unroll
  for (int j = 0; j < NJ; ++j)
#pragma unroll
    for (int i = 0; i < 4; ++i) acc[j][i] = f32x4_t{0.f, 0.f, 0.f, 0.f};

  const int fr = lane & 15, fg = lane >> 4;
  auto compute = [&](const uint8_t* buf) {
#pragma unroll
    for (int ks = 0; ks < 2; ++ks) {
      const int c = ks * 4 + fg;
      bf16x8_t xf[4], wf[NJ];
#pragma unroll
      for (int i = 0; i < 4; ++i) {
        const int row = wm * 64 + i * 16 + fr;
        xf[i] = *reinterpret_cast<const bf16x8_t*>(buf + row * CV_ROW + ((c ^ (row & 7)) << 4));
      }
#pragma unroll
      for (int j = 0; j < NJ; ++j) {
        const int row = wn * (BN / 2) + j * 16 + fr;
        wf[j] = *reinterpret_cast<const bf16x8_t*>(buf + A_BYTES + row * CV_ROW + ((c ^ (row & 7)) << 4));
      }
#pragma unroll
      for (int j = 0; j < NJ; ++j)
#pragma unroll
        for (int i = 0; i < 4; ++i)
          acc[j][i] = __builtin_amdgcn_mfma_f32_16x16x32_bf16(wf[j], xf[i], acc[j][i], 0, 0, 0);
    }
  };

  BnbRegs<BNB ? BN : 64> bnb;
  if constexpr (BNB) {
    bnb_prefetch<BN>(a, bnb, n0, tid, row_pixel);
  }
  if (nkt > 0) issue(0, smem_base);
  for (int kt = 0; kt < nkt; ++kt) {
    asm volatile("s_waitcnt vmcnt(0)" ::: "memory");
    wm_barrier();
    if (kt + 1 < nkt && !(WM_CONV_ABLATE & 1)) issue(kt + 1, smem_base + ((kt + 1) & 1) * STAGE);
    else wm_barrier();
    if (!(WM_CONV_ABLATE & 2)) compute(cv_smem + (kt & 1) * STAGE);
  }
  __syncthreads();

  constexpr int CS = BN * 2 + 16;
#pragma unroll
  for (int j = 0; j < NJ; ++j)
#pragma unroll
    for (int i = 0; i < 4; ++i)
      stage_acc_frag(cv_smem, CS, acc[j][i], wm * 64 + i * 16 + fr, wn * (BN / 2) + j * 16 + fg * 4);
  __syncthreads();
  if constexpr (MODE == 0 && !EPI) {
    if (a.stat != nullptr) {
      store_tile_with_stats<BN>(cv_smem, CS, a.dst, a.DC, n0, reinterpret_cast<float*>(cv_smem + BM * CS),
                                stat_slot_ptr_row(a, m0, a.DC), tid,
                                [&](int row) -> size_t { return (size_t)(m0 + row); });
      return;
    }
  }
  if constexpr (BNB) {
    StatSlot slot;
    if constexpr (MODE == 2) {
      const int cls = a.M >> 2;
      const int pc = m0 / cls;
      slot = stat_slot(a, m0 - pc * cls, pc * (a.stat_rpg / BM));
    } else {
      slot = stat_slot(a, m0);
    }
    bnb_epilogue<BN>(a, bnb, cv_smem, CS, reinterpret_cast<float*>(cv_smem + BM * CS), slot, n0, tid);
    return;
  }
  if constexpr (EPI) {
    constexpr int CPR = BN / 8;
    constexpr int NIT = BM * CPR / CV_THREADS;
    size_t pixs[NIT];
    uint4 rv[NIT];
  #pragma unroll
    for (int it = 0; it < NIT; ++it) {
      const int p = tid + it * CV_THREADS;
      const int row = p / CPR, ch = p - row * CPR;
      const size_t pix = row_pixel(row);
      pixs[it] = pix;
      rv[it] = make_uint4(0, 0, 0, 0);
      if (a.res != nullptr && m0 + row < a.M) rv[it] = *reinterpret_cast<const uint4*>(a.res + pix * a.DC + n0 + ch * 8);
      if (a.act == 2 && m0 + row < a.M) rv[it] = *reinterpret_cast<const uint4*>(a.pre_in + pix * a.DC + n0 + ch * 8);
    }
    static_assert(CV_THREADS % CPR == 0, "chunk column constant per lane");
    float4 b0 = make_float4(0.f, 0.f, 0.f, 0.f), b1 = b0;
    if constexpr (MODE == 0) {
      if (a.bias != nullptr) {
        b0 = *reinterpret_cast<const float4*>(a.bias + n0 + (tid % CPR) * 8);
        b1 = *reinterpret_cast<const float4*>(a.bias + n0 + (tid % CPR) * 8 + 4);
      }
    }
  #pragma unroll
    for (int it = 0; it < NIT; ++it) {
      const int p = tid + it * CV_THREADS;
      const int row = p / CPR, ch = p - row * CPR;
      const size_t pix = pixs[it];
      if (m0 + row < a.M) {
        uint4 v = *reinterpret_cast<const uint4*>(cv_smem + row * CS + ch * 16);
        if constexpr (MODE == 0) {
          if (a.bias != nullptr) {
            const float b[8] = {b0.x, b0.y, b0.z, b0.w, b1.x, b1.y, b1.z, b1.w};
            v = bf16x8_map(v, [&](int e, float x) { return x + b[e]; });
          }
        }
        if (a.act == 1) {
          *reinterpret_cast<uint4*>(a.pre_out + pix * a.DC + n0 + ch * 8) = v;
          v = bf16x8_map(v, [](int, float x) { return cv_gelu(x); });
        } else if (a.act == 2) {
          v = bf16x8_zip(v, rv[it], [](float x, float pre) { return x * cv_gelu_grad(pre); });
        } else if (a.res != nullptr) {
          v = bf16x8_add(v, rv[it]);
        }
        *reinterpret_cast<uint4*>(a.dst + pix * a.DC + n0 + ch * 8) = v;
      }
    }
  } else {
    constexpr int CPR = BN / 8;
    for (int p = tid; p < BM * CPR; p += CV_THREADS) {
      const int row = p / CPR, ch = p - row * CPR;
      const size_t pix = row_pixel(row);
      if (m0 + row < a.M) {
        uint4 v = *reinterpret_cast<const uint4*>(cv_smem + row * CS + ch * 16);
        if (a.res != nullptr) v = bf16x8_add(v, *reinterpret_cast<const uint4*>(a.res + pix * a.DC + n0 + ch * 8));
        *reinterpret_cast<uint4*>(a.dst + pix * a.DC + n0 + ch * 8) = v;
      }
    }
  }
}

constexpr int PT_PITCH = 11;
constexpr int PT_PIX = 10 * PT_PITCH;
constexpr int PT_SLOTS = 224;
constexpr int PT_PATCH_BYTES = PT_SLOTS * CV_ROW;
constexpr int PT_W_BYTES = 64 * CV_ROW;
constexpr int PT_WSTAGES = 3;

constexpr int PT_LDS = PT_PATCH_BYTES + PT_WSTAGES * PT_W_BYTES;

template <int MODE, bool BNB = false>
__global__ __launch_bounds__(CV_THREADS, BNB ? 3 : 1) void conv3x3_patch(const ConvArgs a) {
  constexpr bool DGRAD = MODE != 0;
  static_assert(!BNB || DGRAD, "BatchNorm-backward epilogue: dgrad only");
  extern __shared__ __attribute__((aligned(16))) uint8_t cv_smem[];
  const int tid = threadIdx.x, lane = tid & 63;
  const int wave = __builtin_amdgcn_readfirstlane(tid >> 6);
  const int wm = wave >> 1, wn = wave & 1;
  const int tw_n = a.DW >> 3, tiles_img = (a.DH >> 3) * tw_n;
  const uint32_t smem_base = lds_addr(cv_smem);

  const int bx = a.xcd == 2 ? (int)wm_xcd_swizzle(blockIdx.x, gridDim.x) : (int)blockIdx.x;
  int tn[2], th0[2], tw0[2];
#pragma unroll
  for (int t = 0; t < 2; ++t) {
    const int T = bx * 2 + t;
    tn[t] = T / tiles_img;
    const int tr = T - tn[t] * tiles_img;
    const int th = tr / tw_n;
    th0[t] = th * 8;
    tw0[t] = (tr - th * tw_n) * 8;
  }
  {
    const int sl = lane & 7;
#pragma unroll
    for (int i = 0; i < 7; ++i) {
      const int j = wave + 4 * i;
      const int gp = 8 * j + (lane >> 3);
      const int t = gp >= PT_PIX ? 1 : 0;
      const int pp = gp - t * PT_PIX;
      const int py = pp / PT_PITCH, px = pp - py * PT_PITCH;
      const int h = (t ? th0[1] : th0[0]) - 1 + py, w = (t ? tw0[1] : tw0[0]) - 1 + px;
      const bool ok = gp < 2 * PT_PIX && px < 10 && (unsigned)h < (unsigned)a.SH && (unsigned)w < (unsigned)a.SW;
      const int chunk = sl ^ (px & 7);
      const uint16_t* src = ok ? a.src + ((size_t)((t ? tn[1] : tn[0]) * a.SH + h) * a.SW + w) * 64 + chunk * 8
                               : conv_zero_page + chunk * 8;
      glds16_at(src, smem_base + j * 1024);
    }
  }
  BnbRegs<64> bnb;
  if constexpr (BNB) {
    const size_t org[2] = {pair_origin(a, tn[0], th0[0], tw0[0]), pair_origin(a, tn[1], th0[1], tw0[1])};
    bnb_prefetch<64>(a, bnb, 0, tid, [&](int row) -> size_t { return pair_pixel(org, row, a.DW); });
  }
  const int rowl = tid >> 3;
  const int wchunk = (tid & 7) ^ (rowl & 7);
  const size_t wrow = (size_t)9 * 64;
  const uint16_t* pb0 = a.wt + (size_t)rowl * wrow + wchunk * 8;
  const uint16_t* pb1 = pb0 + 32 * wrow;
  auto issue_w = [&](int tap, uint32_t stage) {
    glds16_at(pb0 + tap * 64, stage + (wave * 8) * CV_ROW);
    glds16_at(pb1 + tap * 64, stage + (wave * 8 + 32) * CV_ROW);
  };
  issue_w(0, smem_base + PT_PATCH_BYTES);
  issue_w(1, smem_base + PT_PATCH_BYTES + PT_W_BYTES);

  f32x4_t acc[2][4];
#pragma unroll
  for (int j = 0; j < 2; ++j)
#pragma unroll
    for (int i = 0; i < 4; ++i) acc[j][i] = f32x4_t{0.f, 0.f, 0.f, 0.f};

  const int fr = lane & 15, fg = lane >> 4;
  const int dy = fr >> 3, dx = fr & 7;
  uint32_t xoff[3][2];
#pragma unroll
  for (int sh = 0; sh < 3; ++sh)
#pragma unroll
    for (int ks = 0; ks < 2; ++ks)
      xoff[sh][ks] = (uint32_t)((wm * PT_PIX + dy * PT_PITCH + dx + sh) * CV_ROW + (((ks * 4 + fg) ^ ((dx + sh) & 7)) << 4));
  uint32_t woff[2][2];
#pragma unroll
  for (int j = 0; j < 2; ++j)
#pragma unroll
    for (int ks = 0; ks < 2; ++ks) {
      const int row = wn * 32 + j * 16 + fr;
      woff[j][ks] = (uint32_t)(PT_PATCH_BYTES + row * CV_ROW + (((ks * 4 + fg) ^ (row & 7)) << 4));
    }

#pragma unroll
  for (int tap = 0; tap < 9; ++tap) {
    static_assert(PT_WSTAGES == 3, "two taps in flight: this one and the next");
    if (tap + 1 < 9) asm volatile("s_waitcnt vmcnt(2)" ::: "memory");
    else asm volatile("s_waitcnt vmcnt(0)" ::: "memory");
    wm_barrier();
    if (tap + 2 < 9) issue_w(tap + 2, smem_base + PT_PATCH_BYTES + ((tap + 2) % PT_WSTAGES) * PT_W_BYTES);
    const int r = tap / 3, sx = tap % 3;
    const int prow = DGRAD ? 2 - r : r;
    const int pcol = DGRAD ? 2 - sx : sx;
#pragma unroll
    for (int ks = 0; ks < 2; ++ks) {
      bf16x8_t xf[4], wf[2];
#pragma unroll
      for (int i = 0; i < 4; ++i)
        xf[i] = *reinterpret_cast<const bf16x8_t*>(cv_smem + xoff[pcol][ks] + (2 * i + prow) * PT_PITCH * CV_ROW);
#pragma unroll
      for (int j = 0; j < 2; ++j)
        wf[j] = *reinterpret_cast<const bf16x8_t*>(cv_smem + woff[j][ks] + (tap % PT_WSTAGES) * PT_W_BYTES);
#pragma unroll
      for (int j = 0; j < 2; ++j)
#pragma unroll
        for (int i = 0; i < 4; ++i)
          acc[j][i] = __builtin_amdgcn_mfma_f32_16x16x32_bf16(wf[j], xf[i], acc[j][i], 0, 0, 0);
    }
  }
  __syncthreads();

  constexpr int CS = 64 * 2 + 16;
#pragma unroll
  for (int j = 0; j < 2; ++j)
#pragma unroll
    for (int i = 0; i < 4; ++i)
      stage_acc_frag(cv_smem, CS, acc[j][i], wm * 64 + i * 16 + fr, wn * 32 + j * 16 + fg * 4);
  __syncthreads();
  if constexpr (BNB) {
    bnb_epilogue<64>(a, bnb, cv_smem, CS, reinterpret_cast<float*>(cv_smem + 128 * CS), stat_slot_pair(a, tn[0], bx), 0, tid);
    return;
  }
  const size_t org[2] = {pair_origin(a, tn[0], th0[0], tw0[0]), pair_origin(a, tn[1], th0[1], tw0[1])};
  if constexpr (MODE == 0) {
    if (a.stat != nullptr) {
      store_tile_with_stats<64>(cv_smem, CS, a.dst, 64, 0, reinterpret_cast<float*>(cv_smem + 128 * CS),
                                stat_slot_ptr(a, stat_slot_pair(a, tn[0], bx), 64), tid,
                                [&](int row) -> size_t { return pair_pixel(org, row, a.DW); });
      return;
    }
  }
#pragma unroll
  for (int q = 0; q < 128 * 8 / CV_THREADS; ++q) {
    const int p = tid + q * CV_THREADS;
    const int row = p >> 3, ch = p & 7;
    const size_t pix = pair_pixel(org, row, a.DW);
    uint4 v = *reinterpret_cast<const uint4*>(cv_smem + row * CS + ch * 16);
    if (a.res != nullptr) v = bf16x8_add(v, *reinterpret_cast<const uint4*>(a.res + pix * 64 + ch * 8));
    *reinterpret_cast<uint4*>(a.dst + pix * 64 + ch * 8) = v;
  }
}

constexpr int ST_PITCH = 12;
constexpr int ST_PIX = 11 * ST_PITCH;
constexpr int ST_PATCH_INSTR = 9;
constexpr int ST_PATCH_BYTES = ST_PATCH_INSTR * 1024;
constexpr int ST_CS = 64 * 2 + 16;
constexpr int ST_LDS = 2 * ST_PATCH_BYTES + 128 * ST_CS + 2 * 4 * 64 * 4;

__global__ __launch_bounds__(CV_THREADS, 3) void conv_stem_patch(const ConvArgs a, int npairs, const WmDiv d_timg,
                                                                 const WmDiv d_twn) {
  extern __shared__ __attribute__((aligned(16))) uint8_t cv_smem[];
  const int tid = threadIdx.x, lane = tid & 63;
  const int wave = __builtin_amdgcn_readfirstlane(tid >> 6);
  const int wm = wave >> 1, wn = wave & 1;
  const uint32_t smem_base = lds_addr(cv_smem);
  uint8_t* stage = cv_smem + 2 * ST_PATCH_BYTES;
  const int fr = lane & 15, fg = lane >> 4;

  bf16x8_t wreg[2][4][2];
#pragma unroll
  for (int j = 0; j < 2; ++j)
#pragma unroll
    for (int r = 0; r < 4; ++r)
#pragma unroll
      for (int ks = 0; ks < 2; ++ks)
        wreg[j][r][ks] = *reinterpret_cast<const bf16x8_t*>(a.wt + (size_t)(wn * 32 + j * 16 + fr) * 256 + (r * 8 + ks * 4 + fg) * 8);

  int pc_t[3], pc_py[3], pc_px[3], pc_half[3];
  bool pc_on[3];
#pragma unroll
  for (int i = 0; i < 3; ++i) {
    const int piece = 64 * (wave + 4 * i) + lane;
    const int gp = piece >> 1;
    pc_half[i] = piece & 1;
    pc_t[i] = gp >= ST_PIX ? 1 : 0;
    const int pp = gp - pc_t[i] * ST_PIX;
    pc_py[i] = pp / ST_PITCH;
    pc_px[i] = pp - pc_py[i] * ST_PITCH;
    pc_on[i] = gp < 2 * ST_PIX && pc_px[i] < 11;
  }
  auto tile_origin = [&](int T, int& n, int& h0, int& w0) {
    T = __builtin_amdgcn_readfirstlane(T);
    uint32_t tr, tw;
    n = (int)wm_divmod((uint32_t)T, d_timg, tr);
    h0 = (int)wm_divmod(tr, d_twn, tw) * 8;
    w0 = (int)tw * 8;
  };
  auto issue_patch = [&](int pair, uint32_t buf) {
    int n[2], h0[2], w0[2];
    tile_origin(pair * 2, n[0], h0[0], w0[0]);
    tile_origin(pair * 2 + 1, n[1], h0[1], w0[1]);
#pragma unroll
    for (int i = 0; i < 3; ++i) {
      const int j = wave + 4 * i;
      if (j < ST_PATCH_INSTR) {
        const int t = pc_t[i];
        const int h = (t ? h0[1] : h0[0]) - a.pad + pc_py[i], w = (t ? w0[1] : w0[0]) - a.pad + pc_px[i];
        const bool ok = pc_on[i] && (unsigned)h < (unsigned)a.SH && (unsigned)w < (unsigned)a.SW;
        const uint16_t* src = ok ? a.src + ((size_t)((t ? n[1] : n[0]) * a.SH + h) * a.SW + w) * 16 + pc_half[i] * 8
                                 : conv_zero_page + pc_half[i] * 8;
        glds16_at(src, buf + j * 1024);
      }
// ... 669 lines not shown
  if (c.patch) { c.bmo = 64; c.cpt = 8; c.nt = 9; }
  else wgrad_tiles(g, c);
  wgrad_plan(g, c);
  return c;
}

template <int BMO, int CPT, int NT, bool BIAS>
int launch_wgrad_impl(const WgradArgs& a, int nsplit, hipStream_t st) {
  constexpr int lds = 2 * (WG_PIX * BMO * 2 + NT * WG_PIX * 128);
  const int rc = ensure_lds<&conv_wgrad<BMO, CPT, NT, BIAS>>(lds);
  if (rc != WM_OK) return rc;
  dim3 grid(a.R * a.S * a.C / 64 / NT, a.K / BMO, nsplit);
  conv_wgrad<BMO, CPT, NT, BIAS><<<grid, CV_THREADS, lds, st>>>(a);
  WM_LAUNCH_CHECK();
  return WM_OK;
}
int launch_wgrad_patch(const WgradArgs& a, int nsplit, hipStream_t st) {
  const int rc = ensure_lds<&conv_wgrad_patch64>(WP_LDS);
  if (rc != WM_OK) return rc;
  const int tiles_w = a.W >> 3, tpi = (a.H >> 3) * tiles_w;
  conv_wgrad_patch64<<<nsplit, CV_THREADS, WP_LDS, st>>>(a, wm_div_make((uint32_t)tpi), wm_div_make((uint32_t)tiles_w));
  WM_LAUNCH_CHECK();
  return WM_OK;
}

inline int wgrad_route(const WgradChoice& c, bool has_bias) {
  if (c.patch) return has_bias ? WM_EUNSUPPORTED : WM_ROUTE_WGRAD_PATCH64;
  if (c.cpt == 2 && has_bias) return WM_EUNSUPPORTED;
  return WM_ROUTE_WGRAD(c.bmo, c.cpt, c.nt, has_bias);
}
int launch_wgrad_route(int route, const WgradArgs& a, int nsplit, hipStream_t st) {
#define WM_WGRAD_CASE(BMO, CPT, NT, BIAS) \
  case WM_ROUTE_WGRAD(BMO, CPT, NT, BIAS): return launch_wgrad_impl<BMO, CPT, NT, BIAS>(a, nsplit, st);
  switch (route) {
    case WM_ROUTE_WGRAD_PATCH64: return launch_wgrad_patch(a, nsplit, st);
    WM_WGRAD_CASE(128, 2, 2, false) WM_WGRAD_CASE(128, 2, 1, false)
    WM_WGRAD_CASE(64, 2, 4, false) WM_WGRAD_CASE(64, 2, 1, false)
    WM_WGRAD_CASE(128, 8, 3, false) WM_WGRAD_CASE(128, 8, 3, true)
    WM_WGRAD_CASE(128, 8, 2, false) WM_WGRAD_CASE(128, 8, 2, true)
    WM_WGRAD_CASE(128, 8, 1, false) WM_WGRAD_CASE(128, 8, 1, true)
    WM_WGRAD_CASE(64, 8, 3, false) WM_WGRAD_CASE(64, 8, 3, true)
    WM_WGRAD_CASE(64, 8, 1, false) WM_WGRAD_CASE(64, 8, 1, true)
    default: return route < 0 ? route : WM_EUNSUPPORTED;
  }
#undef WM_WGRAD_CASE
}

int conv_fwd_impl(const void* x, const void* w_krsc, void* y, const ConvGeom& g, float* stat, int stat_nb, int stat_rpg,
                  void* stream, const float* bias = nullptr, const void* residual = nullptr, void* pre_out = nullptr) {
  WM_REQUIRE(pre_out == nullptr || (residual == nullptr && g.R == 1 && g.S == 1), WM_EUNSUPPORTED);
  WM_REQUIRE(x && w_krsc && y, WM_EINVAL);
  const int rc = conv_check(g);
  if (rc != WM_OK) return rc;
  WM_REQUIRE(aligned16(x) && aligned16(w_krsc) && aligned16(y), WM_EALIGN);
  ConvArgs a = conv_args(g, false);
  a.src = static_cast<const uint16_t*>(x);
  a.wt = static_cast<const uint16_t*>(w_krsc);
  a.dst = static_cast<uint16_t*>(y);
  a.stat = stat; a.stat_nb = stat_nb; a.stat_rpg = stat_rpg;
  a.res = static_cast<const uint16_t*>(residual);
  a.bias = bias;
  a.pre_out = static_cast<uint16_t*>(pre_out);
  a.act = pre_out != nullptr ? 1 : 0;
  hipStream_t st = static_cast<hipStream_t>(stream);
  const int route = conv_fwd_route(g, stat != nullptr ? stat_rpg : 0, bias != nullptr, residual != nullptr, pre_out != nullptr);
  if (route == WM_ROUTE_PANEL) {
    WmPanelArgs pa{a.src, a.wt, bias, a.res, nullptr, a.pre_out, a.dst, a.M, g.K, a.act, 0, nullptr, nullptr, 0.f};
    return wm_panel_launch(pa, st);
  }
  return launch_conv_route(route, a, st);
}

struct BnbArgs {
  const void* bn_y;
  const void* bn_x;
  const void* bn_mask;
  const float *mean, *invstd, *gamma, *beta;
  int G;
  float* stat;
  int stat_nb;
};

int conv_dgrad_impl(const void* dy, const void* w_crsk, void* dx, const void* residual, const ConvGeom& g, void* stream,
                    const void* pre_in = nullptr, const BnbArgs* bnb = nullptr) {
  WM_REQUIRE(dy && w_crsk && dx, WM_EINVAL);
  WM_REQUIRE(pre_in == nullptr || (residual == nullptr && g.R == 1 && g.S == 1 && g.stride == 1 && aligned16(pre_in)), WM_EUNSUPPORTED);
  const int rc = conv_check(g);
  if (rc != WM_OK) return rc;
  WM_REQUIRE(g.C % 64 == 0, WM_EUNSUPPORTED);
  WM_REQUIRE(aligned16(dy) && aligned16(w_crsk) && aligned16(dx), WM_EALIGN);
  ConvArgs a = conv_args(g, true);
  a.src = static_cast<const uint16_t*>(dy);
  a.wt = static_cast<const uint16_t*>(w_crsk);
  a.dst = static_cast<uint16_t*>(dx);
  a.res = static_cast<const uint16_t*>(residual);
  a.pre_in = static_cast<const uint16_t*>(pre_in);
  a.act = pre_in != nullptr ? 2 : 0;
  hipStream_t st = static_cast<hipStream_t>(stream);
  const int route = conv_dgrad_route(g, residual != nullptr, pre_in != nullptr, bnb != nullptr ? bnb->G : 0);
  if (bnb != nullptr) {
    WM_REQUIRE(pre_in == nullptr, WM_EUNSUPPORTED);
    a.bn_y = static_cast<const uint16_t*>(bnb->bn_y);
    a.bn_x = static_cast<const uint16_t*>(bnb->bn_x);
    a.bn_mask = static_cast<const uint8_t*>(bnb->bn_mask);
    a.bn_mean = bnb->mean; a.bn_invstd = bnb->invstd; a.bn_gamma = bnb->gamma; a.bn_beta = bnb->beta;
    a.stat = bnb->stat; a.stat_nb = bnb->stat_nb;
    a.stat_rpg = (int)(dgrad_stat_rows(g, dgrad_mode(g)) / bnb->G);
  }
  if (route == WM_ROUTE_PANEL) {
    WmPanelArgs pa{a.src, a.wt, nullptr, a.res, a.pre_in, nullptr, a.dst, a.M, g.C, a.act, 0, nullptr, nullptr, 0.f};
    return wm_panel_launch(pa, st);
  }
  return launch_conv_route(route, a, st);
}

}

extern "C" int wm_conv2d_fwd(const void* x, const void* w_krsc, void* y, int N, int H, int W, int C,
                             int K, int R, int S, int P, int Q, int stride, int pad, void* stream) {
  return conv_fwd_impl(x, w_krsc, y, {N, H, W, C, K, R, S, P, Q, stride, pad}, nullptr, 0, 0, stream);
}

extern "C" int wm_conv2d_fwd_bias_res(const void* x, const void* w_krsc, const float* bias, const void* residual,
                                      void* y, int N, int H, int W, int C, int K, int R, int S, int P, int Q,
                                      int stride, int pad, void* stream) {
  WM_REQUIRE(aligned16(bias) && aligned16(residual), WM_EALIGN);
  return conv_fwd_impl(x, w_krsc, y, {N, H, W, C, K, R, S, P, Q, stride, pad}, nullptr, 0, 0, stream, bias, residual);
}

extern "C" int wm_conv2d_fwd_stats_tiles(int N, int H, int W, int C, int K, int R, int S, int P, int Q, int stride,
                                         int pad, int rows_per_group) {
  const ConvGeom g{N, H, W, C, K, R, S, P, Q, stride, pad};
  if (conv_check(g) != WM_OK || rows_per_group <= 0) return WM_EINVAL;
  if (rows_per_group % 128 != 0 || g.rows_y() % rows_per_group != 0) return WM_EUNSUPPORTED;
  if (stem_patch_ok(g, false, false, rows_per_group)) return stem_patch_group_slots(rows_per_group / 128);
  return rows_per_group / 128;
}

extern "C" int wm_conv2d_fwd_stats(const void* x, const void* w_krsc, void* y, int N, int H, int W, int C,
                                   int K, int R, int S, int P, int Q, int stride, int pad, float* stat_part,
                                   int stat_tiles, int rows_per_group, void* stream) {
  WM_REQUIRE(stat_part && rows_per_group > 0, WM_EINVAL);
  WM_REQUIRE(rows_per_group % 128 == 0 && ((long long)N * P * Q) % rows_per_group == 0, WM_EUNSUPPORTED);
  WM_REQUIRE(stat_tiles == wm_conv2d_fwd_stats_tiles(N, H, W, C, K, R, S, P, Q, stride, pad, rows_per_group), WM_EINVAL);
  return conv_fwd_impl(x, w_krsc, y, {N, H, W, C, K, R, S, P, Q, stride, pad}, stat_part, stat_tiles, rows_per_group, stream);
}

extern "C" int wm_linear_bias_gelu_fwd(const void* x, const void* w_krsc, const float* bias, void* pre_out, void* y,
                                       int rows, int C, int K, void* stream) {
  WM_REQUIRE(pre_out && bias, WM_EINVAL);
  WM_REQUIRE(aligned16(bias) && aligned16(pre_out), WM_EALIGN);
  return conv_fwd_impl(x, w_krsc, y, {rows, 1, 1, C, K, 1, 1, 1, 1, 1, 0}, nullptr, 0, 0, stream, bias, nullptr, pre_out);
}

extern "C" int wm_linear_dgrad_gelu(const void* dy, const void* w_crsk, const void* pre, void* dx, int rows, int C,
                                    int K, void* stream) {
  WM_REQUIRE(pre, WM_EINVAL);
  return conv_dgrad_impl(dy, w_crsk, dx, nullptr, {rows, 1, 1, C, K, 1, 1, 1, 1, 1, 0}, stream, pre);
}

extern "C" int wm_conv2d_dgrad(const void* dy, const void* w_crsk, void* dx, int N, int H, int W,
                               int C, int K, int R, int S, int P, int Q, int stride, int pad,
                               void* stream) {
  return conv_dgrad_impl(dy, w_crsk, dx, nullptr, {N, H, W, C, K, R, S, P, Q, stride, pad}, stream);
}

extern "C" int wm_conv2d_dgrad_add(const void* dy, const void* w_crsk, const void* residual, void* dx, int N,
                                   int H, int W, int C, int K, int R, int S, int P, int Q, int stride, int pad,
                                   void* stream) {
  WM_REQUIRE(residual, WM_EINVAL);
  WM_REQUIRE(aligned16(residual), WM_EALIGN);
  return conv_dgrad_impl(dy, w_crsk, dx, residual, {N, H, W, C, K, R, S, P, Q, stride, pad}, stream);
}

extern "C" int wm_conv2d_dgrad_bnstat_ok(int N, int H, int W, int C, int K, int R, int S, int P, int Q, int stride,
                                         int pad, int G) {
  const ConvGeom g{N, H, W, C, K, R, S, P, Q, stride, pad};
  return conv_check(g) == WM_OK && dgrad_bnstat_ok(g, G) ? 1 : 0;
}

extern "C" int wm_conv2d_dgrad_bnstat(const void* dy, const void* w_crsk, const void* residual, void* dx, int N, int H,
                                      int W, int C, int K, int R, int S, int P, int Q, int stride, int pad,
                                      const void* bn_y, const void* relu_x, const void* relu_mask, const float* gamma,
                                      const float* beta, const float* save_mean, const float* save_invstd, int G,
                                      float* stat_part, int stat_tiles, void* stream) {
  WM_REQUIRE(bn_y && save_mean && save_invstd && stat_part, WM_EINVAL);
  WM_REQUIRE(G > 0 && stat_tiles == (int)((long long)N * H * W / G / 128), WM_EINVAL);
  WM_REQUIRE(relu_x || relu_mask || (gamma && beta), WM_EINVAL);
  WM_REQUIRE(!(relu_x && relu_mask), WM_EINVAL);
  WM_REQUIRE(wm_conv2d_dgrad_bnstat_ok(N, H, W, C, K, R, S, P, Q, stride, pad, G), WM_EUNSUPPORTED);
  WM_REQUIRE(aligned16(bn_y) && aligned16(save_mean) && aligned16(save_invstd) && aligned16(relu_x) && aligned16(residual),
             WM_EALIGN);
  BnbArgs b{bn_y, relu_x, relu_mask, save_mean, save_invstd, gamma, beta, G, stat_part, stat_tiles};
  return conv_dgrad_impl(dy, w_crsk, dx, residual, {N, H, W, C, K, R, S, P, Q, stride, pad}, stream, nullptr, &b);
}

extern "C" int wm_conv2d_wgrad(const void* dy, const void* x, float* dw_krsc, int N, int H, int W,
                               int C, int K, int R, int S, int P, int Q, int stride, int pad,
                               void* stream) {
  return wm_conv2d_wgrad_bias(dy, x, dw_krsc, nullptr, N, H, W, C, K, R, S, P, Q, stride, pad, stream);
}

extern "C" int wm_conv2d_wgrad_bias(const void* dy, const void* x, float* dw_krsc, float* dbias, int N, int H,
                                    int W, int C, int K, int R, int S, int P, int Q, int stride, int pad,
                                    void* stream) {
  WM_REQUIRE(dy && x && dw_krsc, WM_EINVAL);
  const ConvGeom g{N, H, W, C, K, R, S, P, Q, stride, pad};
  const int rc = conv_check(g);
  if (rc != WM_OK) return rc;
  WM_REQUIRE(aligned16(dy) && aligned16(x) && aligned16(dw_krsc), WM_EALIGN);
  WM_REQUIRE(g.rows_x() * C < (1ll << 32) - (1 << 20) && g.rows_y() * K < (1ll << 32) - (1 << 20), WM_EUNSUPPORTED);
  const WgradChoice c = wgrad_choice(g);
  WM_REQUIRE(!(dbias != nullptr && c.patch), WM_EUNSUPPORTED);
  WgradArgs a;
  a.xcd = xcd_order();
  a.dy = static_cast<const uint16_t*>(dy);
  a.x = static_cast<const uint16_t*>(x);
  a.dw = dw_krsc;
  a.dbias = dbias;
  a.N = N; a.H = H; a.W = W; a.C = C; a.K = K; a.R = R; a.S = S; a.P = P; a.Q = Q;
  a.stride = stride; a.pad = pad; a.M = N * P * Q;
  a.chunks_per_split = c.chunks_per_split; a.total_chunks = c.total_chunks;
  hipStream_t st = static_cast<hipStream_t>(stream);
  return launch_wgrad_route(wgrad_route(c, dbias != nullptr), a, c.nsplit, st);
}

extern "C" int wm_conv2d_wgrad_splits(int N, int H, int W, int C, int K, int R, int S, int P, int Q, int stride, int pad) {
  const ConvGeom g{N, H, W, C, K, R, S, P, Q, stride, pad};
  const int rc = conv_check(g);
  if (rc != WM_OK) return rc;
  return wgrad_choice(g).nsplit;
}

extern "C" int wm_conv2d_route(int pass, int N, int H, int W, int C, int K, int R, int S, int P, int Q, int stride, int pad,
                               int flags, int group_arg) {
  const ConvGeom g{N, H, W, C, K, R, S, P, Q, stride, pad};
  const int rc = conv_check(g);
  if (rc != WM_OK) return rc;
  const bool stats = flags & WM_ROUTE_F_STATS, res = flags & WM_ROUTE_F_RESIDUAL, bias = flags & WM_ROUTE_F_BIAS;
  const bool bnb = flags & WM_ROUTE_F_BNB, act = flags & WM_ROUTE_F_ACT;
  WM_REQUIRE((flags & ~31) == 0, WM_EINVAL);
  if (pass == 0) {
    WM_REQUIRE(!bnb && !(stats && (res || bias || act)), WM_EINVAL);
    if (stats) {
      WM_REQUIRE(group_arg > 0, WM_EINVAL);
      WM_REQUIRE(group_arg % 128 == 0 && g.rows_y() % group_arg == 0, WM_EUNSUPPORTED);
    }
    return conv_fwd_route(g, stats ? group_arg : 0, bias, res, act);
  }
  if (pass == 1) {
    WM_REQUIRE(!stats && !bias, WM_EINVAL);
    if (bnb) {
      WM_REQUIRE(group_arg > 0, WM_EINVAL);
      WM_REQUIRE(dgrad_bnstat_ok(g, group_arg), WM_EUNSUPPORTED);
    }
    return conv_dgrad_route(g, res, act, bnb ? group_arg : 0);
  }
  WM_REQUIRE(pass == 2 && !stats && !res && !bnb && !act, WM_EINVAL);
  WM_REQUIRE(g.rows_x() * C < (1ll << 32) - (1 << 20) && g.rows_y() * K < (1ll << 32) - (1 << 20), WM_EUNSUPPORTED);
  return wgrad_route(wgrad_choice(g), bias);
}
```

self-supervised-wafermaps_amd/models/resnet.py:

```python
from __future__ import annotations

import os

import torch
import torch.nn as nn

from .. import nn as hnn
from .. import ops


def conv_bn(conv, bn, x, relu=False, residual=None):
    if bn.training:
        g = ops.current_bn_groups()
        st = bn.stats_buffer(g)
        return bn(conv(x, stats=st, groups=g), residual=residual, relu=relu, stats=st)
    return bn(conv(x), residual=residual, relu=relu)


class BasicBlock(nn.Module):
    expansion = 1

    def __init__(self, inplanes, planes, stride=1):
        super().__init__()
        self.conv1 = hnn.Conv2d(inplanes, planes, 3, stride, 1)
        self.bn1 = hnn.BatchNorm2d(planes)
        self.conv2 = hnn.Conv2d(planes, planes, 3, 1, 1)
        self.bn2 = hnn.BatchNorm2d(planes)
        self.downsample = None
        if stride != 1 or inplanes != planes:
            self.downsample = nn.Sequential(hnn.Conv2d(inplanes, planes, 1, stride, 0), hnn.BatchNorm2d(planes))
        nn.init.zeros_(self.bn2.weight)

    def forward(self, x):
        if self.downsample is not None and torch.is_grad_enabled() and x.requires_grad:
            g = ops.current_bn_groups()
            st = self.bn1.stats_buffer(g) if self.bn1.training else None
            y, x_alias = self.conv1(x, stats=st, groups=g, passthrough=True)
            out = self.bn1(y, relu=True, stats=st)
            shortcut = conv_bn(self.downsample[0], self.downsample[1], x_alias)
        elif self.downsample is not None:
            out = conv_bn(self.conv1, self.bn1, x, relu=True)
            shortcut = conv_bn(self.downsample[0], self.downsample[1], x)
        elif torch.is_grad_enabled() and x.requires_grad:
            g = ops.current_bn_groups()
            st = self.bn1.stats_buffer(g) if self.bn1.training else None
            y, shortcut = self.conv1(x, stats=st, groups=g, passthrough=True)
            out = self.bn1(y, relu=True, stats=st)
        else:
            out = conv_bn(self.conv1, self.bn1, x, relu=True)
            shortcut = x
        return conv_bn(self.conv2, self.bn2, out, relu=True, residual=shortcut)


class ResNet18(nn.Module):
    num_features = 512

    def __init__(self, num_classes: int = 0):
        super().__init__()
        if num_classes != 0:
            raise NotImplementedError("only the headless backbone (num_classes=0) is built")
        self.conv1 = hnn.StemConv(64)
        self.bn1 = hnn.BatchNorm2d(64)
        self.layer1 = nn.Sequential(BasicBlock(64, 64), BasicBlock(64, 64))
        self.layer2 = nn.Sequential(BasicBlock(64, 128, 2), BasicBlock(128, 128))
        self.layer3 = nn.Sequential(BasicBlock(128, 256, 2), BasicBlock(256, 256))
        self.layer4 = nn.Sequential(BasicBlock(256, 512, 2), BasicBlock(512, 512))

    def forward_features(self, x):
        if self.bn1.training:
            g = ops.current_bn_groups()
            st = self.bn1.stats_buffer(g)
            x = self.bn1.forward_relu_maxpool(self.conv1(x, stats=st, groups=g), stats=st)
        else:
            x = self.bn1.forward_relu_maxpool(self.conv1(x))
        x = self.layer1(x)
        x = self.layer2(x)
        x = self.layer3(ops.cut_point(x, "layer3"))
        return self.layer4(ops.cut_point(x, "layer4"))

    view_branches = True

    def forward(self, x):
        if self._branch_ok(x):
            return self._forward_branches(x)
        return ops.global_avg_pool(self.forward_features(x))

    def _branch_ok(self, x) -> bool:
        from .. import precision

        if os.environ.get("WM_EVAL_BRANCHES", "1") != "0" and not self.training and not torch.is_grad_enabled() \
                and x.is_cuda and x.shape[0] % 2 == 0 and x.shape[0] >= 64 and ops.current_branch() == 0 \
                and self.view_branches and not precision.is_f32():
            if getattr(self, "_branches", None) is None or not self._branches.valid():
                if torch.cuda.is_current_stream_capturing():
                    return False
                try:
                    self._branches = hnn.ViewBranches(self)
                except ValueError:
                    self.view_branches = False
                    return False
            return True
        if not (self.view_branches and self.training and x.is_cuda and ops.current_bn_groups() == 2
                and x.shape[0] % 2 == 0 and ops.current_branch() == 0):
            return False
        if os.environ.get("WM_VIEW_BRANCHES", "1") == "0" or precision.is_f32():
            return False
        vb = getattr(self, "_branches", None)
        if vb is None or not vb.valid():
            if torch.cuda.is_current_stream_capturing():
                return False
            try:
                vb = self._branches = hnn.ViewBranches(self)
            except ValueError:
                self.view_branches = False
                return False
        return not any(m._synced() for m in vb.modules)

    def _forward_branches(self, x):
        vb = self._branches
        b = x.shape[0] // 2
        cur = torch.cuda.current_stream(x.device)
        vb.prepare()
        vb.side.wait_stream(cur)
        with ops.bn_groups(1):
            f0 = ops.global_avg_pool(self.forward_features(x[:b]))
            with torch.cuda.stream(vb.side), ops.branch(1):
                f1 = ops.global_avg_pool(self.forward_features(x[b:]))
        cur.wait_stream(vb.side)
        if self.training:
            vb.merge()
        return ops.stack_rows(f0.flatten(start_dim=1), f1.flatten(start_dim=1))


def create_model(name: str, num_classes: int = 0, pretrained: bool = False, **kw):
# ... 6 lines not shown
```

self-supervised-wafermaps_amd/nn.py:

```python
from __future__ import annotations

import math

import os

import torch
import torch.nn as nn

from . import evalops, ops, vit_ops
from . import precision as _precision


class Conv2d(nn.Module):

    def __init__(self, in_channels, out_channels, kernel_size, stride=1, padding=0):
        super().__init__()
        self.in_channels, self.out_channels = in_channels, out_channels
        self.kernel_size, self.stride, self.padding = kernel_size, stride, padding
        self.weight = nn.Parameter(torch.empty(out_channels, in_channels, kernel_size, kernel_size))
        nn.init.kaiming_normal_(self.weight, mode="fan_out", nonlinearity="relu")

    def forward(self, x, stats=None, groups=1, passthrough=False):
        if passthrough:
            return ops.conv2d_passthrough(x, self.weight, self.stride, self.padding, stats=stats, groups=groups)
        return ops.conv2d(x, self.weight, self.stride, self.padding, stats=stats, groups=groups)


class StemConv(Conv2d):

    def __init__(self, out_channels=64):
        super().__init__(3, out_channels, 7, 2, 3)

    def forward(self, x, stats=None, groups=1):
        return ops.stem_conv(x, self.weight, stats=stats, groups=groups)


class _BatchNorm(nn.Module):
    def __init__(self, num_features, eps=1e-5, momentum=0.1, affine=True):
        super().__init__()
        self.num_features, self.eps, self.momentum, self.affine = num_features, eps, momentum, affine
        if affine:
            self.weight = nn.Parameter(torch.ones(num_features))
            self.bias = nn.Parameter(torch.zeros(num_features))
        else:
            self.register_buffer("weight", torch.ones(num_features), persistent=False)
            self.register_buffer("bias", torch.zeros(num_features), persistent=False)
        self.register_buffer("running_mean", torch.zeros(num_features))
        self.register_buffer("running_var", torch.ones(num_features))
        self.register_buffer("num_batches_tracked", torch.tensor(0, dtype=torch.long))
        self.sync, self.process_group = False, None

    def _synced(self) -> bool:
        if not (self.sync and self.training):
            return False
        import torch.distributed as dist

        return dist.is_available() and dist.is_initialized() and dist.get_world_size(self.process_group) > 1

    def stats_buffer(self, groups: int = 0, which: str = "_stat_buf"):
        if ops.current_branch():
            which = f"{which}_b{ops.current_branch()}"
        slots = getattr(self, which, None)
        if slots is None:
            slots = ops.StatSlots(self.num_features)
            setattr(self, which, slots)
        return slots

    def forward(self, x, residual=None, relu=False, stats=None):
        if self._synced():
            return ops.sync_batch_norm(x, self.weight, self.bias, self.running_mean, self.running_var, residual=residual,
                                       relu=relu, eps=self.eps, momentum=self.momentum, stats=stats,
                                       num_batches_tracked=self.num_batches_tracked, process_group=self.process_group)
        bwd = None
        if self.training and relu and x.dim() == 4 and torch.is_grad_enabled():
            bwd = self.stats_buffer(ops.current_bn_groups(), "_stat_buf_bwd")
        rm, rv, mom = self._running()
        return ops.batch_norm(x, self.weight, self.bias, rm, rv, self.training,
                              residual=residual, relu=relu, eps=self.eps, momentum=mom, stats=stats,
                              num_batches_tracked=self.num_batches_tracked, bwd_stats=bwd)

    def _running(self):
        if ops.current_branch() and self.training:
            br = getattr(self, "_branch_running", None)
            if br is None:
                raise RuntimeError("BatchNorm on a side branch without branch buffers: build nn.ViewBranches(model) first")
            return br[0], br[1], 1.0
        return self.running_mean, self.running_var, self.momentum


class BatchNorm2d(_BatchNorm):
    def forward_relu_maxpool(self, x, stats=None):
        if self._synced():
            return ops.max_pool3x3s2(self.forward(x, relu=True, stats=stats))
        rm, rv, mom = self._running()
        return ops.bn_relu_maxpool(x, self.weight, self.bias, rm, rv, self.training,
                                   eps=self.eps, momentum=mom, stats=stats,
                                   num_batches_tracked=self.num_batches_tracked)


class BatchNorm1d(_BatchNorm):
    pass


class ViewBranches:

    _ALIGN = 64

    def __init__(self, root: nn.Module):
        bns = [m for m in root.modules() if isinstance(m, _BatchNorm) and m.running_mean is not None]
        if not bns:
            raise ValueError("ViewBranches: no BatchNorm layers")
        moms = {m.momentum for m in bns}
        if len(moms) != 1 or None in moms:
            raise ValueError("ViewBranches: the BatchNorm layers must share one momentum")
        self.momentum = float(moms.pop())
        dev = bns[0].running_mean.device
        offs, total = [], 0
        for m in bns:
            for _ in range(2):
                offs.append(total)
                total += (m.num_features + self._ALIGN - 1) // self._ALIGN * self._ALIGN
        self.real = torch.zeros(total, dtype=torch.float32, device=dev)
        self.tmp = torch.zeros(total, dtype=torch.float32, device=dev)
        with torch.no_grad():
            for i, m in enumerate(bns):
                c = m.num_features
                om, ov = offs[2 * i], offs[2 * i + 1]
                self.real[om:om + c].copy_(m.running_mean)
                self.real[ov:ov + c].copy_(m.running_var)
                m.running_mean.data = self.real[om:om + c]
                m.running_var.data = self.real[ov:ov + c]
                m._branch_running = (self.tmp[om:om + c], self.tmp[ov:ov + c])
        self.n = total
        self.side = torch.cuda.Stream(device=dev)
        self.modules = bns
        self.convs = [m for m in root.modules() if isinstance(m, Conv2d)]

    def prepare(self) -> None:
        for m in self.convs:
            if isinstance(m, StemConv):
                ops._WCACHE.get(m.weight, kind="stem")
            else:
                ops._WCACHE.get(m.weight, need_crsk=True)

    def __deepcopy__(self, memo):
        return None

    def valid(self) -> bool:
        m = self.modules[0]
        return m.running_mean.data_ptr() == self.real.data_ptr() and m.running_mean.device == self.real.device

    def merge(self) -> None:
        from . import _lib
        from ._lib import check, stream_ptr

        check(_lib.load().wm_ema_update(self.real.data_ptr(), self.tmp.data_ptr(), self.n, 1.0 - self.momentum, stream_ptr()),
              "wm_ema_update(bn running statistics)")


def convert_sync_batchnorm(module: nn.Module, process_group=None) -> nn.Module:
    for m in module.modules():
        if isinstance(m, _BatchNorm):
            m.sync, m.process_group = True, process_group
    return module


class Linear(nn.Module):

    def __init__(self, in_features, out_features, bias=False):
        super().__init__()
        self.in_features, self.out_features = in_features, out_features
        self.weight = nn.Parameter(torch.empty(out_features, in_features))
        nn.init.kaiming_uniform_(self.weight, a=math.sqrt(5))
        if bias:
            bound = 1 / math.sqrt(in_features)
            self.bias = nn.Parameter(torch.empty(out_features).uniform_(-bound, bound))
        else:
            self.register_parameter("bias", None)

    def forward(self, x, act: int = vit_ops.ACT_NONE, residual=None):
# ... 67 lines not shown
```

self-supervised-wafermaps_amd/ops.py:

```python
from __future__ import annotations

import contextlib
import os
from typing import Optional

import torch

from . import _lib, f32path
from . import precision as _precision
from ._lib import check, ptr, stream_ptr

_WEIGHT_EPOCH = 0


class KernelTimer:

    def __init__(self, external: bool = False):
        self.records = []
        self.external = external
        self.sums = None
        self.replays = 0

    def run(self, name, work, fn, *args):
        if self.external:
# ... 493 lines not shown
    v = _STAT_TILES.get(key)
    if v is None:
        v = int(_lib.load().wm_conv2d_fwd_stats_tiles(*key))
        if v <= 0:
            check(v if v < 0 else _lib.WM_EUNSUPPORTED, "wm_conv2d_fwd_stats_tiles")
        _STAT_TILES[key] = v
    return v


class StatSlots:

    def __init__(self, channels: int):
        self.channels, self.buf, self.tiles, self.groups = channels, None, 0, 0
        self._hip_busy = None

    def get(self, groups: int, tiles: int, device) -> torch.Tensor:
        capturing = torch.cuda.is_current_stream_capturing()
        if self.buf is None or self.tiles != tiles or self.groups != groups or self.buf.device != device:
            if getattr(self, "_captured", False):
                self.__dict__.setdefault("_retired", []).append(self.buf)
                self._captured = False
            self.buf = torch.empty((groups, tiles, 2, self.channels), dtype=torch.float32, device=device)
            self.tiles, self.groups = tiles, groups
        if capturing:
            self._captured = True
        return self.buf


def stats_fusable(rows: int, groups: int) -> bool:
    return groups > 0 and rows % groups == 0 and (rows // groups) % 128 == 0


class BnLink:

    __slots__ = ("y", "mean", "invstd", "gamma", "beta", "groups", "has_res", "stats", "ready", "g_ptr", "g_version", "mask")

    def __init__(self, y, mean, invstd, gamma, beta, groups, has_res, stats, mask=None):
        self.y, self.mean, self.invstd, self.gamma, self.beta = y, mean, invstd, gamma, beta
        self.groups, self.has_res, self.stats = groups, has_res, stats
        self.mask = mask
        self.ready, self.g_ptr, self.g_version = False, 0, -1


_BN_FUSE_BWD = os.environ.get("WM_BN_FUSE_BWD", "1") != "0"
_BN_BITMASK = os.environ.get("WM_BN_BITMASK", "1") != "0"


def _out_hw(h, w, r, s, stride, pad):
    return (h + 2 * pad - r) // stride + 1, (w + 2 * pad - s) // stride + 1


def _conv_fwd(x, wk, y, geom, work, stats, groups, tag: str = "") -> None:
    n, p, q = geom[0], geom[7], geom[8]
    rows = n * p * q
    lib = _lib.load()
    if stats is not None and stats_fusable(rows, groups):
        tiles = fwd_stat_tiles(*geom, rows // groups)
        check(_run("conv_fwd", work, lib.wm_conv2d_fwd_stats, ptr(x), ptr(wk), y.data_ptr(), *geom,
                   ptr(stats.get(groups, tiles, x.device)), tiles, rows // groups, stream_ptr()), "wm_conv2d_fwd_stats" + tag)
    else:
        check(_run("conv_fwd", work, lib.wm_conv2d_fwd, ptr(x), ptr(wk), y.data_ptr(), *geom, stream_ptr()),
              "wm_conv2d_fwd" + tag)


class _Conv2d(torch.autograd.Function):
    @staticmethod
    def forward(ctx, x, weight, stride, pad, stats=None, groups=1, pass_input=False, link=None):
        _need_cuda(x, "conv2d")
        x = _as_nhwc(x)
        n, c, h, w = x.shape
        k, c2, r, s = weight.shape
        if c2 != c or weight.dtype != torch.float32:
            raise ValueError(f"conv2d: input channels {c} vs weight {tuple(weight.shape)} ({weight.dtype})")
        p, q = _out_hw(h, w, r, s, stride, pad)
        train = torch.is_grad_enabled() and (x.requires_grad or weight.requires_grad)
        krsc, _ = _WCACHE.get(weight, need_crsk=train and x.requires_grad)
        y = _empty_nhwc(n, k, p, q, x.device)
        geom = (n, h, w, c, k, r, s, p, q, stride, pad)
        _conv_fwd(x, krsc, y, geom, 2.0 * n * p * q * k * r * s * c, stats, groups)
        ctx.save_for_backward(x)
        ctx.weight = weight
        ctx.geom = geom
        ctx.link = link if (_BN_FUSE_BWD and link is not None and link.y.shape == x.shape) else None
        if pass_input:
            return y, x.view_as(x)
        return y

    @staticmethod
    def backward(ctx, dy, dres=None):
        (x,) = ctx.saved_tensors
        weight = ctx.weight
        n, h, w, c, k, r, s, p, q, stride, pad = ctx.geom
        dy = _as_nhwc(dy)
        lib = _lib.load()
        dx = dw = None
        if ctx.needs_input_grad[0]:
            _, crsk = _WCACHE.get(weight, need_crsk=True)
            dx = _empty_nhwc(n, c, h, w, dy.device)
            if dres is not None:
                dres = _as_nhwc(dres)

            def dgrad(entry, *mid, tail=()):
                check(_run("conv_dgrad", 2.0 * n * p * q * k * r * s * c, getattr(lib, entry), dy.data_ptr(), ptr(crsk), *mid,
                           dx.data_ptr(), *ctx.geom, *tail, stream_ptr()), entry)

            link = ctx.link
            if (link is not None and not link.ready and getattr(link.stats, "_hip_busy", None) is None
                    and lib.wm_conv2d_dgrad_bnstat_ok(n, h, w, c, k, r, s, p, q, stride, pad, link.groups)):
                tiles = n * h * w // link.groups // 128
                dgrad("wm_conv2d_dgrad_bnstat", ptr(dres), tail=(
                    link.y.data_ptr(), x.data_ptr() if (link.has_res and link.mask is None) else 0,
                    ptr(link.mask) if link.has_res else 0, ptr(link.gamma), ptr(link.beta), ptr(link.mean),
                    ptr(link.invstd), link.groups, ptr(link.stats.get(link.groups, tiles, dy.device)), tiles))
                link.ready, link.g_ptr, link.g_version = True, dx.data_ptr(), dx._version
                link.stats._hip_busy = True
            elif dres is not None:
                dgrad("wm_conv2d_dgrad_add", dres.data_ptr())
            else:
                dgrad("wm_conv2d_dgrad")
        if ctx.needs_input_grad[1]:
            slabs, _, ns = wgrad(dy, x, weight, n, h, w, c, k, r, s, p, q, stride, pad)
            dw, _ = wgrad_deliver(weight, slabs, ns, k, c, r, s)
        return _pad_grads(ctx, dx, dw)


def conv2d(x: torch.Tensor, weight: torch.Tensor, stride: int = 1, padding: int = 0,
           stats: Optional[torch.Tensor] = None, groups: int = 1) -> torch.Tensor:
    if _precision.is_f32():
        return f32path.conv2d(x, weight, int(stride), int(padding))
    return _Conv2d.apply(x, weight, int(stride), int(padding), stats, int(groups), False, getattr(x, "_hip_bn", None))


def conv2d_passthrough(x: torch.Tensor, weight: torch.Tensor, stride: int = 1, padding: int = 0,
                       stats: Optional[torch.Tensor] = None, groups: int = 1):
    if _precision.is_f32():
        return f32path.conv2d(x, weight, int(stride), int(padding)), x
    return _Conv2d.apply(x, weight, int(stride), int(padding), stats, int(groups), True, getattr(x, "_hip_bn", None))


class _StemConv(torch.autograd.Function):

    @staticmethod
    def forward(ctx, x, weight, stats=None, groups=1):
        _need_cuda(x, "stem_conv")
        n, c, h, w = x.shape
        k = weight.shape[0]
        s2d_input = c == 16 and x.dtype == torch.bfloat16
        if (c != 3 and not s2d_input) or tuple(weight.shape[1:]) != (3, 7, 7) or (not s2d_input and (h % 2 or w % 2)):
            raise ValueError("stem_conv: expects [N,3,even,even] (or space-to-depth [N,16,H/2,W/2] bf16) input and "
                             "[K,3,7,7] weights")
        if x.requires_grad:
            raise NotImplementedError("stem_conv: no input gradient (images are data)")
        lib = _lib.load()
        if s2d_input:
            h2, w2 = h, w
            xs = _as_nhwc(x)
        else:
            if x.dtype == torch.float32 and x.is_contiguous():
                fmt = _lib.WM_IMG_NCHW_F32
            else:
                x = _as_nhwc(x)
                fmt = _lib.WM_IMG_NHWC_BF16
            h2, w2 = h // 2, w // 2
            xs = torch.empty((n, h2, w2, 16), dtype=torch.bfloat16, device=x.device)
            check(lib.wm_image_to_s2d(x.data_ptr(), fmt, n, h, w, ptr(xs), stream_ptr()), "wm_image_to_s2d")
        ws2d, _ = _WCACHE.get(weight, kind="stem")
        y = _empty_nhwc(n, k, h2, w2, x.device)
        _conv_fwd(xs, ws2d, y, (n, h2, w2, 16, k, 4, 4, h2, w2, 1, 2), 2.0 * n * h2 * w2 * k * 147, stats, groups, "(stem)")
        ctx.save_for_backward(xs)
        ctx.weight = weight
        ctx.geom = (n, h2, w2, k)
        ctx.branch = current_branch()
        return y

    @staticmethod
    def backward(ctx, dy):
        (xs,) = ctx.saved_tensors
        n, h2, w2, k = ctx.geom
        dy = _as_nhwc(dy)
        lib = _lib.load()
        slabs, _, ns = wgrad(dy, xs, ctx.weight, n, h2, w2, 16, k, 4, 4, h2, w2, 1, 2)
        side_join()
        slot = _arena_grad(ctx.weight)
        if slot is not None and ctx.branch != 0:
            tmp = _use_buffer(ctx.weight, "_hip_flat_fold", k * 147, dy.device)
            check(lib.wm_stem_wgrad_finalize(ptr(slabs), ns, k, ptr(tmp), 0, stream_ptr()), "wm_stem_wgrad_finalize")
            _queue_fold(ctx.weight, tmp, 1, slot, 1, k * 147, 1)
            return _pad_grads(ctx)
        return _pad_grads(ctx, None, finalize_into(slabs, ns, k, 3, 7, 7, ctx.weight, (k, 3, 7, 7), stem=True))


def stem_conv(x: torch.Tensor, weight: torch.Tensor, stats: Optional[torch.Tensor] = None, groups: int = 1) -> torch.Tensor:
    if _precision.is_f32():
        if x.shape[1] != 3:
            raise ValueError("stem_conv (float32 preset): give [N,3,H,W] images (augment_views fmt \"nchw_f32\"), not the "
                             "space-to-depth bf16 layout")
        return f32path.conv2d(x, weight, 2, 3)
    return _StemConv.apply(x, weight, stats, int(groups))


_BN_WS = {}


def _bn_workspace(rows: int, c: int, g: int, device) -> torch.Tensor:
    need = _lib.load().wm_bn_workspace_bytes(rows, c, g)
    if need == 0:
        raise ValueError(f"batch_norm: unsupported shape rows={rows} C={c} G={g}")
    key = (device, torch.cuda.current_stream(device).cuda_stream if device.type == "cuda" else 0)
    ws = _BN_WS.get(key)
    if ws is None or ws.numel() < need:
        ws = torch.empty(max(need, 1 << 20), dtype=torch.uint8, device=device)
        _BN_WS[key] = ws
    return ws


def _rows_c(x: torch.Tensor):
    if x.dim() == 4:
        n, c, h, w = x.shape
        return n * h * w, c
    if x.dim() == 2:
# ... 60 lines not shown
            if rows % groups:
                raise ValueError("batch_norm: rows not divisible by groups")
            mean = torch.empty((groups, c), dtype=torch.float32, device=y.device)
            invstd = torch.empty_like(mean)
            will_link = (bwd_stats is not None and relu and y.dim() == 4 and gamma is not None and beta is not None
                         and stats_fusable(rows, groups) and ctx.needs_input_grad[0])
            mask = None
            if will_link and residual is not None and c % 8 == 0 and c <= 2048 and _BN_BITMASK:
                mask = torch.empty((rows, c // 8), dtype=torch.uint8, device=y.device)
            if stats is not None and stats.buf is not None and stats_fusable(rows, groups):
                check(lib.wm_bn_train_fwd_from_stats(y.data_ptr(), ptr(residual) if residual is not None else 0,
                                                     ptr(gamma), ptr(beta), ptr(running_mean), ptr(running_var),
                                                     ptr(counter), rows, c,
                                                     groups, eps, momentum, int(relu), ptr(mean), ptr(invstd),
                                                     out.data_ptr(), ptr(mask), ptr(stats.buf), stats.tiles, ptr(ws),
                                                     ws.numel(), stream_ptr()), "wm_bn_train_fwd_from_stats")
            else:
                check(lib.wm_bn_train_fwd(y.data_ptr(), ptr(residual) if residual is not None else 0, ptr(gamma),
                                          ptr(beta), ptr(running_mean), ptr(running_var), ptr(counter), rows, c, groups, eps,
                                          momentum, int(relu), ptr(mean), ptr(invstd), out.data_ptr(), ptr(mask), ptr(ws),
                                          ws.numel(), stream_ptr()), "wm_bn_train_fwd")
            mask_from_y = _bn_save(ctx, y, out, mean, invstd, gamma, beta, relu, residual is not None)
            ctx.meta = (rows, c, groups, relu, residual is not None, mask_from_y)
            ctx.branch = current_branch()
            if will_link:
                ctx.link = BnLink(y, mean, invstd, gamma, beta, groups, residual is not None, bwd_stats, mask)
        else:
            check(lib.wm_bn_eval_fwd(y.data_ptr(), ptr(residual) if residual is not None else 0, ptr(gamma), ptr(beta),
                                     ptr(running_mean), ptr(running_var), rows, c, eps, int(relu), out.data_ptr(),
                                     ptr(ws), ws.numel(), stream_ptr()), "wm_bn_eval_fwd")
            ctx.meta = None
        return out

    @staticmethod
    def backward(ctx, dout):
        if ctx.meta is None:
            raise NotImplementedError("batch_norm: backward through eval-mode statistics is not implemented")
        y, out, mean, invstd = ctx.saved_tensors
        gamma, beta = ctx.affine
        rows, c, groups, relu, has_res, mask_from_y = ctx.meta
        dout = _as_act(dout)
        lib = _lib.load()
        dy = torch.empty_like(y)
        dgamma, dbeta, direct, finish = _bn_param_grads(gamma, beta, c, y.device, getattr(ctx, "branch", 0))
        ws = _bn_workspace(rows, c, groups, y.device)
        link = ctx.link
        fused = False
        if link is not None and link.ready:
            link.ready = False
            link.stats._hip_busy = None
            if dout.data_ptr() == link.g_ptr and dout._version == link.g_version:
                check(lib.wm_bn_train_bwd_from_stats(y.data_ptr(), dout.data_ptr(), ptr(gamma), ptr(beta), ptr(mean),
                                                     ptr(invstd), rows, c, groups, ptr(dgamma), ptr(dbeta), int(direct),
                                                     dy.data_ptr(), ptr(link.stats.buf), link.stats.tiles, ptr(ws),
                                                     ws.numel(), stream_ptr()), "wm_bn_train_bwd_from_stats")
                dz = dout if has_res else None
                fused = True
            else:
                pass
        if not fused:
            dz = torch.empty_like(y) if has_res else None
            check(lib.wm_bn_train_bwd(y.data_ptr(), dout.data_ptr(), out.data_ptr() if (relu and not mask_from_y) else 0,
                                      int(mask_from_y), ptr(gamma), ptr(beta), ptr(mean), ptr(invstd), rows, c, groups,
                                      ptr(dgamma), ptr(dbeta), int(direct), dy.data_ptr(), dz.data_ptr() if has_res else 0,
                                      ptr(ws), ws.numel(), stream_ptr()), "wm_bn_train_bwd")
        return _pad_grads(ctx, dy, dz, *finish())


def batch_norm(y, gamma, beta, running_mean, running_var, training: bool, residual=None, relu: bool = False,
               eps: float = 1e-5, momentum: float = 0.1, groups: Optional[int] = None, stats=None,
               num_batches_tracked=None, bwd_stats=None):
    g = current_bn_groups() if groups is None else groups
    if _precision.is_f32():
        return f32path.batch_norm(y, gamma, beta, running_mean, running_var, bool(training), residual, bool(relu), eps, momentum,
                                  int(g), num_batches_tracked)
    out = _BatchNorm.apply(y, residual, gamma, beta, running_mean, running_var, bool(training), int(g), float(eps),
                           float(momentum), bool(relu), stats, num_batches_tracked, bwd_stats)
    link = getattr(out.grad_fn, "link", None) if out.grad_fn is not None else None
    if link is not None:
        out._hip_bn = link
    return out


class _SyncBatchNorm(torch.autograd.Function):

    @staticmethod
    def forward(ctx, y, residual, gamma, beta, running_mean, running_var, groups, eps, momentum, relu, stats, counter,
                group):
        import torch.distributed as dist

        y, residual, rows, c = _bn_inputs(y, residual, "sync_batch_norm")
        if rows % groups:
            raise ValueError("sync_batch_norm: rows not divisible by groups")
        lib = _lib.load()
        world = dist.get_world_size(group)
        out = torch.empty_like(y)
        ws = _bn_workspace(rows, c, groups, y.device)
        sums = torch.empty((groups, 2, c), dtype=torch.float32, device=y.device)
        fused = stats is not None and stats.buf is not None and stats_fusable(rows, groups)
        check(lib.wm_bn_sync_fwd_sums(y.data_ptr(), rows, c, groups, ptr(stats.buf) if fused else 0,
                                      stats.tiles if fused else 0, ptr(sums), ptr(ws), ws.numel(), stream_ptr()),
              "wm_bn_sync_fwd_sums")
        dist.all_reduce(sums, group=group)
        mean = torch.empty((groups, c), dtype=torch.float32, device=y.device)
        invstd = torch.empty_like(mean)
        count = rows // groups * world
        check(lib.wm_bn_sync_fwd_apply(y.data_ptr(), ptr(residual) if residual is not None else 0, ptr(gamma), ptr(beta),
                                       ptr(running_mean), ptr(running_var), ptr(counter), rows, c, groups, count, eps,
                                       momentum, int(relu), ptr(mean), ptr(invstd), out.data_ptr(), ptr(sums), ptr(ws),
                                       ws.numel(), stream_ptr()), "wm_bn_sync_fwd_apply")
        mask_from_y = _bn_save(ctx, y, out, mean, invstd, gamma, beta, relu, residual is not None)
        ctx.meta = (rows, c, groups, relu, residual is not None, mask_from_y, count, group)
        return out

    @staticmethod
    def backward(ctx, dout):
        import torch.distributed as dist

        y, out, mean, invstd = ctx.saved_tensors
        gamma, beta = ctx.affine
        rows, c, groups, relu, has_res, mask_from_y, count, group = ctx.meta
        dout = _as_act(dout)
        lib = _lib.load()
        dy = torch.empty_like(y)
        dgamma, dbeta, direct, finish = _bn_param_grads(gamma, beta, c, y.device, 0)
        ws = _bn_workspace(rows, c, groups, y.device)
        sums = torch.empty((groups, 2, c), dtype=torch.float32, device=y.device)
        mask = out.data_ptr() if (relu and not mask_from_y) else 0
        check(lib.wm_bn_sync_bwd_sums(y.data_ptr(), dout.data_ptr(), mask, int(mask_from_y), ptr(gamma), ptr(beta),
                                      ptr(mean), ptr(invstd), rows, c, groups, ptr(dgamma), ptr(dbeta), int(direct),
                                      ptr(sums), ptr(ws), ws.numel(), stream_ptr()), "wm_bn_sync_bwd_sums")
        dist.all_reduce(sums, group=group)
        dz = torch.empty_like(y) if has_res else None
        check(lib.wm_bn_sync_bwd_apply(y.data_ptr(), dout.data_ptr(), mask, int(mask_from_y), ptr(gamma), ptr(beta),
                                       ptr(mean), ptr(invstd), rows, c, groups, count, ptr(sums), dy.data_ptr(),
                                       dz.data_ptr() if has_res else 0, ptr(ws), ws.numel(), stream_ptr()),
              "wm_bn_sync_bwd_apply")
        return _pad_grads(ctx, dy, dz, *finish())


def sync_batch_norm(y, gamma, beta, running_mean, running_var, residual=None, relu: bool = False, eps: float = 1e-5,
                    momentum: float = 0.1, groups: Optional[int] = None, stats=None, num_batches_tracked=None,
                    process_group=None):
    g = current_bn_groups() if groups is None else groups
    if _precision.is_f32():
        raise NotImplementedError("sync_batch_norm: not part of the float32 (parity) preset")
    return _SyncBatchNorm.apply(y, residual, gamma, beta, running_mean, running_var, int(g), float(eps), float(momentum),
                                bool(relu), stats, num_batches_tracked, process_group)


class _BnReluMaxPool(torch.autograd.Function):

    @staticmethod
    def forward(ctx, y, gamma, beta, running_mean, running_var, training, groups, eps, momentum, stats=None,
                counter=None):
        _need_cuda(y, "bn_relu_maxpool")
        y = _as_nhwc(y)
        n, c, h, w = y.shape
        rows = n * h * w
        lib = _lib.load()
        g = groups if training else 1
        if n % g:
            raise ValueError("bn_relu_maxpool: batch not divisible by the statistics groups")
        scale = torch.empty((g, c), dtype=torch.float32, device=y.device)
        shift = torch.empty_like(scale)
        if training:
# ... 157 lines not shown
```

Before: 24570 imgs/sec.

## Fuse downsample-shortcut BN with main-branch BN and use compact dgrad residual

After: 24700 imgs/sec, median of 6. No clear change (+0.5%).

```diff
diff --git a/include/wafer_hip.h b/include/wafer_hip.h
--- a/include/wafer_hip.h
+++ b/include/wafer_hip.h
@@ -114,6 +114,14 @@
                            const void* relu_x, const void* relu_mask, const float* gamma, const float* beta,
                            const float* save_mean, const float* save_invstd, int G, float* stat_part, int stat_tiles,
                            void* stream);
+int wm_conv2d_dgrad_compact_ok(int N, int H, int W, int C, int K, int R, int S, int P, int Q, int stride, int pad);
+int wm_conv2d_dgrad_add_compact(const void* dy, const void* w_crsk, const void* residual_compact, void* dx, int N, int H,
+                                int W, int C, int K, int R, int S, int P, int Q, int stride, int pad, void* stream);
+int wm_conv2d_dgrad_bnstat_compact(const void* dy, const void* w_crsk, const void* residual_compact, void* dx, int N, int H,
+                                   int W, int C, int K, int R, int S, int P, int Q, int stride, int pad, const void* bn_y,
+                                   const void* relu_x, const void* relu_mask, const float* gamma, const float* beta,
+                                   const float* save_mean, const float* save_invstd, int G, float* stat_part,
+                                   int stat_tiles, void* stream);
 int wm_conv2d_wgrad_splits(int N, int H, int W, int C, int K, int R, int S, int P, int Q, int stride, int pad);
 int wm_conv2d_wgrad(const void* dy, const void* x, float* dw_slabs, int N, int H, int W, int C, int K,
                     int R, int S, int P, int Q, int stride, int pad, void* stream);
@@ -200,6 +208,21 @@
                                const float* save_mean, const float* save_invstd, long long rows, int C, int G,
                                float* dgamma, float* dbeta, int accumulate, void* dy, const float* stat_part,
                                int stat_tiles, void* workspace, size_t workspace_bytes, void* stream);
+size_t wm_bn_shortcut_workspace_bytes(long long rows, int C, int G, int stat_tiles_a, int stat_tiles_b);
+int wm_bn_train_fwd_from_stats_sc(const void* y, const void* y_d, const float* gamma, const float* beta,
+                                  float* running_mean, float* running_var, long long* num_batches_tracked,
+                                  const float* gamma_d, const float* beta_d, float* running_mean_d, float* running_var_d,
+                                  long long* num_batches_tracked_d, long long rows, int C, int G, float eps, float momentum,
+                                  float eps_d, float momentum_d, int relu, float* save_mean, float* save_invstd,
+                                  float* save_mean_d, float* save_invstd_d, void* out, void* relu_mask,
+                                  const float* stat_part, int stat_tiles, const float* stat_part_d, int stat_tiles_d,
+                                  void* workspace, size_t workspace_bytes, void* stream);
+int wm_bn_train_bwd_from_stats_sc(const void* y, const void* y_d, const void* g, const float* gamma, const float* beta,
+                                  const float* save_mean, const float* save_invstd, const float* gamma_d,
+                                  const float* beta_d, const float* save_mean_d, const float* save_invstd_d, long long rows,
+                                  int C, int G, float* dgamma, float* dbeta, int accumulate, float* dgamma_d, float* dbeta_d,
+                                  int accumulate_d, void* dy, void* dy_d, const float* stat_part, int stat_tiles,
+                                  void* workspace, size_t workspace_bytes, void* stream);
 int wm_bn_sync_fwd_sums(const void* y, long long rows, int C, int G, const float* stat_part, int stat_tiles,
                         float* sums, void* workspace, size_t workspace_bytes, void* stream);
 int wm_bn_sync_fwd_apply(const void* y, const void* residual, const float* gamma, const float* beta,
diff --git a/self-supervised-wafermaps_amd/_lib.py b/self-supervised-wafermaps_amd/_lib.py
--- a/self-supervised-wafermaps_amd/_lib.py
+++ b/self-supervised-wafermaps_amd/_lib.py
@@ -138,10 +138,26 @@
     "wm_conv2d_dgrad_bnstat_ok": (c_int, [c_int] * 12),
     "wm_conv2d_dgrad_bnstat": (c_int, [c_void_p, c_void_p, c_void_p, c_void_p] + [c_int] * 11 +
                                [c_void_p, c_void_p, c_void_p, c_void_p, c_void_p, c_void_p, c_void_p, c_int, c_void_p, c_int, c_void_p]),
+    "wm_conv2d_dgrad_compact_ok": (c_int, [c_int] * 11),
+    "wm_conv2d_dgrad_add_compact": (c_int, [c_void_p, c_void_p, c_void_p, c_void_p] + [c_int] * 11 + [c_void_p]),
+    "wm_conv2d_dgrad_bnstat_compact": (c_int, [c_void_p, c_void_p, c_void_p, c_void_p] + [c_int] * 11 +
+                                       [c_void_p, c_void_p, c_void_p, c_void_p, c_void_p, c_void_p, c_void_p, c_int, c_void_p, c_int,
+                                        c_void_p]),
     "wm_bn_train_bwd_from_stats": (
         c_int,
         [c_void_p, c_void_p, c_void_p, c_void_p, c_void_p, c_void_p, c_longlong, c_int, c_int, c_void_p, c_void_p, c_int,
          c_void_p, c_void_p, c_int, c_void_p, c_size_t, c_void_p],
+    ),
+    "wm_bn_shortcut_workspace_bytes": (c_size_t, [c_longlong, c_int, c_int, c_int, c_int]),
+    "wm_bn_train_fwd_from_stats_sc": (
+        c_int,
+        [c_void_p] * 12 + [c_longlong, c_int, c_int, c_float, c_float, c_float, c_float, c_int] + [c_void_p] * 7 +
+        [c_int, c_void_p, c_int, c_void_p, c_size_t, c_void_p],
+    ),
+    "wm_bn_train_bwd_from_stats_sc": (
+        c_int,
+        [c_void_p] * 11 + [c_longlong, c_int, c_int, c_void_p, c_void_p, c_int, c_void_p, c_void_p, c_int, c_void_p,
+                           c_void_p, c_void_p, c_int, c_void_p, c_size_t, c_void_p],
     ),
     "wm_bn_sync_fwd_sums": (c_int, [c_void_p, c_longlong, c_int, c_int, c_void_p, c_int, c_void_p, c_void_p, c_size_t, c_void_p]),
     "wm_bn_sync_fwd_apply": (
diff --git a/self-supervised-wafermaps_amd/csrc/bn.hip b/self-supervised-wafermaps_amd/csrc/bn.hip
--- a/self-supervised-wafermaps_amd/csrc/bn.hip
+++ b/self-supervised-wafermaps_amd/csrc/bn.hip
@@ -352,6 +352,75 @@
 #pragma unroll
       for (int e = 0; e < 8; ++e) f[e] += r[e];
     }
+    if (relu) {
+#pragma unroll
+      for (int e = 0; e < 8; ++e) f[e] = fmaxf(f[e], 0.f);
+    }
+    const uint4 pk = pack8(f);
+    *reinterpret_cast<uint4*>(out + row * C + c0) = pk;
+    if (relu_mask != nullptr) {
+      float r8[8];
+      unpack8(pk, r8);
+      uint32_t m = 0;
+#pragma unroll
+      for (int e = 0; e < 8; ++e) m |= (r8[e] > 0.f ? 1u : 0u) << e;
+      relu_mask[row * cpr + (c0 >> 3)] = (uint8_t)m;
+    }
+  }
+}
+
+template <bool POW2>
+__global__ __launch_bounds__(BN_THREADS) void bn_apply_sc(const uint16_t* __restrict__ y,
+                                                          const uint16_t* __restrict__ yd,
+                                                          const float* __restrict__ scale,
+                                                          const float* __restrict__ shift,
+                                                          const float* __restrict__ scale_d,
+                                                          const float* __restrict__ shift_d,
+                                                          long long rows, int C, int rows_per_group,
+                                                          int relu, int cshift, uint16_t* __restrict__ out,
+                                                          uint8_t* __restrict__ relu_mask) {
+  const int cpr = C >> 3;
+  const long long total = rows * cpr;
+  int cur_g = -1;
+  float sc[8], sh[8], scd[8], shd[8];
+  for (long long p = (long long)blockIdx.x * BN_THREADS + threadIdx.x; p < total;
+       p += (long long)gridDim.x * BN_THREADS) {
+    long long row;
+    int c0, g;
+    if (POW2) {
+      row = p >> cshift;
+      c0 = (int)(p & (cpr - 1)) * 8;
+      g = 0;
+      for (long long lim = rows_per_group; row >= lim; lim += rows_per_group) ++g;
+    } else {
+      row = p / cpr;
+      c0 = (int)(p - row * cpr) * 8;
+      g = (int)(row / rows_per_group);
+    }
+    if (!POW2 || g != cur_g) {
+      const size_t o = (size_t)g * C + c0;
+      const float4 sa = *reinterpret_cast<const float4*>(scale + o), sb = *reinterpret_cast<const float4*>(scale + o + 4);
+      const float4 ha = *reinterpret_cast<const float4*>(shift + o), hb = *reinterpret_cast<const float4*>(shift + o + 4);
+      sc[0] = sa.x; sc[1] = sa.y; sc[2] = sa.z; sc[3] = sa.w; sc[4] = sb.x; sc[5] = sb.y; sc[6] = sb.z; sc[7] = sb.w;
+      sh[0] = ha.x; sh[1] = ha.y; sh[2] = ha.z; sh[3] = ha.w; sh[4] = hb.x; sh[5] = hb.y; sh[6] = hb.z; sh[7] = hb.w;
+      const float4 da = *reinterpret_cast<const float4*>(scale_d + o), db = *reinterpret_cast<const float4*>(scale_d + o + 4);
+      const float4 ea = *reinterpret_cast<const float4*>(shift_d + o), eb = *reinterpret_cast<const float4*>(shift_d + o + 4);
+      scd[0] = da.x; scd[1] = da.y; scd[2] = da.z; scd[3] = da.w; scd[4] = db.x; scd[5] = db.y; scd[6] = db.z; scd[7] = db.w;
+      shd[0] = ea.x; shd[1] = ea.y; shd[2] = ea.z; shd[3] = ea.w; shd[4] = eb.x; shd[5] = eb.y; shd[6] = eb.z; shd[7] = eb.w;
+      cur_g = g;
+    }
+    float f[8], r[8];
+    const uint4 vy = *reinterpret_cast<const uint4*>(y + row * C + c0);
+    const uint4 vd = *reinterpret_cast<const uint4*>(yd + row * C + c0);
+    unpack8(vd, r);
+#pragma unroll
+    for (int e = 0; e < 8; ++e) r[e] = fmaf(r[e], scd[e], shd[e]);
+    unpack8(pack8(r), r);
+    unpack8(vy, f);
+#pragma unroll
+    for (int e = 0; e < 8; ++e) f[e] = fmaf(f[e], sc[e], sh[e]);
+#pragma unroll
+    for (int e = 0; e < 8; ++e) f[e] += r[e];
     if (relu) {
 #pragma unroll
       for (int e = 0; e < 8; ++e) f[e] = fmaxf(f[e], 0.f);
@@ -477,6 +546,75 @@
   }
 }
 
+template <bool POW2>
+__global__ __launch_bounds__(BN_THREADS, 4) void bn_bwd_apply_sc(const uint16_t* __restrict__ y,
+                                                                 const uint16_t* __restrict__ yd,
+                                                                 const uint16_t* __restrict__ dout,
+                                                                 const float* __restrict__ coef,
+                                                                 const float* __restrict__ coef_d,
+                                                                 long long rows, int C, int rows_per_group, int cshift,
+                                                                 uint16_t* __restrict__ dy, uint16_t* __restrict__ dyd) {
+  const int cpr = C >> 3;
+  const long long total = rows * cpr;
+  const long long stride = (long long)gridDim.x * BN_THREADS;
+  constexpr int NK = 5;
+  float k[NK][8], kd[NK][8];
+  const auto load_coef = [&](int g, int c0) {
+    const float* cf = coef + (size_t)g * 7 * C + c0;
+    const float* cd = coef_d + (size_t)g * 7 * C + c0;
+#pragma unroll
+    for (int t = 0; t < NK; ++t) {
+      const float4 a = *reinterpret_cast<const float4*>(cf + (size_t)t * C);
+      const float4 b = *reinterpret_cast<const float4*>(cf + (size_t)t * C + 4);
+      k[t][0] = a.x; k[t][1] = a.y; k[t][2] = a.z; k[t][3] = a.w;
+      k[t][4] = b.x; k[t][5] = b.y; k[t][6] = b.z; k[t][7] = b.w;
+      const float4 u = *reinterpret_cast<const float4*>(cd + (size_t)t * C);
+      const float4 v = *reinterpret_cast<const float4*>(cd + (size_t)t * C + 4);
+      kd[t][0] = u.x; kd[t][1] = u.y; kd[t][2] = u.z; kd[t][3] = u.w;
+      kd[t][4] = v.x; kd[t][5] = v.y; kd[t][6] = v.z; kd[t][7] = v.w;
+    }
+  };
+  const auto item = [&](size_t off) {
+    const uint4 vy = *reinterpret_cast<const uint4*>(y + off);
+    const uint4 vd = *reinterpret_cast<const uint4*>(yd + off);
+    const uint4 vg = *reinterpret_cast<const uint4*>(dout + off);
+    float fy[8], fd[8], r[8];
+    unpack8(vg, fd);
+    unpack8(vy, fy);
+#pragma unroll
+    for (int e = 0; e < 8; ++e) {
+      const float xh = (fy[e] - k[0][e]) * k[1][e];
+      r[e] = k[2][e] * (fd[e] - k[3][e] - xh * k[4][e]);
+    }
+    *reinterpret_cast<uint4*>(dy + off) = pack8(r);
+    unpack8(vd, fy);
+#pragma unroll
+    for (int e = 0; e < 8; ++e) {
+      const float xh = (fy[e] - kd[0][e]) * kd[1][e];
+      r[e] = kd[2][e] * (fd[e] - kd[3][e] - xh * kd[4][e]);
+    }
+    *reinterpret_cast<uint4*>(dyd + off) = pack8(r);
+  };
+  long long p = (long long)blockIdx.x * BN_THREADS + threadIdx.x;
+  if (POW2) {
+    const int c0 = (int)(p & (cpr - 1)) * 8;
+    const long long per_group = (long long)rows_per_group * cpr;
+    int g = 0;
+    for (long long end = per_group; end - per_group < total; end += per_group, ++g) {
+      load_coef(g, c0);
+#pragma unroll 1
+      for (; p < end; p += stride) item((size_t)p * 8);
+    }
+  } else {
+    for (; p < total; p += stride) {
+      const long long row = p / cpr;
+      const int c0 = (int)(p - row * cpr) * 8;
+      load_coef((int)(row / rows_per_group), c0);
+      item((size_t)row * C + c0);
+    }
+  }
+}
+
 __global__ __launch_bounds__(BN_THREADS) void bn_pool_bwd_apply(const uint16_t* __restrict__ y,
                                                                 const float* __restrict__ coef, int n_coef, int N, int C,
                                                                 int imgs_per_group, int remask,
@@ -671,6 +809,23 @@
                                                               dz, ps);
 }
 
+inline void launch_bn_apply_sc(const uint16_t* y, const uint16_t* yd, const float* scale, const float* shift,
+                               const float* scale_d, const float* shift_d, long long rows, int C, int rpg, int relu,
+                               uint16_t* out, uint8_t* relu_mask, hipStream_t st) {
+  int csh = 0;
+  const auto kernel = chunk_pow2(C, &csh) ? bn_apply_sc<true> : bn_apply_sc<false>;
+  kernel<<<stream_grid(rows * (C >> 3)), BN_THREADS, 0, st>>>(y, yd, scale, shift, scale_d, shift_d, rows, C, rpg, relu, csh,
+                                                              out, relu_mask);
+}
+
+inline void launch_bn_bwd_apply_sc(const uint16_t* y, const uint16_t* yd, const uint16_t* dout, const float* coef,
+                                   const float* coef_d, long long rows, int C, int rpg, uint16_t* dy, uint16_t* dyd,
+                                   hipStream_t st) {
+  int csh = 0;
+  const auto kernel = chunk_pow2(C, &csh) ? bn_bwd_apply_sc<true> : bn_bwd_apply_sc<false>;
+  kernel<<<stream_grid(rows * (C >> 3)), BN_THREADS, 0, st>>>(y, yd, dout, coef, coef_d, rows, C, rpg, csh, dy, dyd);
+}
+
 constexpr int BN_WIDE_MAX_C = 16384;
 
 __global__ __launch_bounds__(BN_THREADS) void bn_col_fwd(const uint16_t* __restrict__ y, const uint16_t* __restrict__ res,
@@ -1056,6 +1211,89 @@
                   coef, 1);
   WM_LAUNCH_CHECK();
   launch_bn_bwd_apply(0, bf16(y), bf16(g), nullptr, coef, rows, C, rpg, false, bf16(dy), nullptr, PoolSrc{}, st);
+  WM_LAUNCH_CHECK();
+  return WM_OK;
+}
+
+extern "C" size_t wm_bn_shortcut_workspace_bytes(long long rows, int C, int G, int stat_tiles_a, int stat_tiles_b) {
+  if (rows <= 0 || C <= 0 || G <= 0 || C % 8 || stat_tiles_a < 0 || stat_tiles_b < 0) return 0;
+  const int nblk = reduce_blocks((int)(rows / G), C);
+  return ((size_t)14 * G * C + (size_t)G * nblk * 2 * C + stat_scratch_floats(stat_tiles_a, G, C) +
+          stat_scratch_floats(stat_tiles_b, G, C)) * sizeof(float) + 256;
+}
+
+extern "C" int wm_bn_train_fwd_from_stats_sc(const void* y, const void* y_d, const float* gamma, const float* beta,
+                                             float* running_mean, float* running_var, long long* num_batches_tracked,
+                                             const float* gamma_d, const float* beta_d, float* running_mean_d,
+                                             float* running_var_d, long long* num_batches_tracked_d, long long rows, int C,
+                                             int G, float eps, float momentum, float eps_d, float momentum_d, int relu,
+                                             float* save_mean, float* save_invstd, float* save_mean_d, float* save_invstd_d,
+                                             void* out, void* relu_mask, const float* stat_part, int stat_tiles,
+                                             const float* stat_part_d, int stat_tiles_d, void* workspace,
+                                             size_t workspace_bytes, void* stream) {
+  WM_REQUIRE(y && y_d && out && save_mean && save_invstd && save_mean_d && save_invstd_d && workspace && stat_part &&
+                 stat_part_d && stat_tiles > 0 && stat_tiles_d > 0,
+             WM_EINVAL);
+  const int rc = bn_shape_check(rows, C, G);
+  if (rc != WM_OK) return rc;
+  WM_REQUIRE(C <= 2048, WM_EUNSUPPORTED);
+  const size_t scr = stat_scratch_floats(stat_tiles, G, C), scr_d = stat_scratch_floats(stat_tiles_d, G, C);
+  WM_REQUIRE(workspace_bytes >= ((size_t)4 * G * C + scr + scr_d) * sizeof(float), WM_EWORKSPACE);
+  hipStream_t st = static_cast<hipStream_t>(stream);
+  const int rpg = (int)(rows / G);
+  float* scale = static_cast<float*>(workspace);
+  float* shift = scale + (size_t)G * C;
+  float* scale_d = shift + (size_t)G * C;
+  float* shift_d = scale_d + (size_t)G * C;
+  float* scratch = shift_d + (size_t)G * C;
+  int rs = bn_fwd_stats(bf16(y_d), stat_part_d, stat_tiles_d, gamma_d, beta_d, running_mean_d, running_var_d,
+                        num_batches_tracked_d, rpg, C, G, eps_d, momentum_d, save_mean_d, save_invstd_d, scale_d, shift_d,
+                        scratch + scr, st);
+  if (rs != WM_OK) return rs;
+  rs = bn_fwd_stats(bf16(y), stat_part, stat_tiles, gamma, beta, running_mean, running_var, num_batches_tracked, rpg, C, G,
+                    eps, momentum, save_mean, save_invstd, scale, shift, scratch, st);
+  if (rs != WM_OK) return rs;
+  launch_bn_apply_sc(bf16(y), bf16(y_d), scale, shift, scale_d, shift_d, rows, C, rpg, relu, bf16(out),
+                     static_cast<uint8_t*>(relu_mask), st);
+  WM_LAUNCH_CHECK();
+  return WM_OK;
+}
+
+extern "C" int wm_bn_train_bwd_from_stats_sc(const void* y, const void* y_d, const void* g, const float* gamma,
+                                             const float* beta, const float* save_mean, const float* save_invstd,
+                                             const float* gamma_d, const float* beta_d, const float* save_mean_d,
+                                             const float* save_invstd_d, long long rows, int C, int G, float* dgamma,
+                                             float* dbeta, int accumulate, float* dgamma_d, float* dbeta_d, int accumulate_d,
+                                             void* dy, void* dy_d, const float* stat_part, int stat_tiles, void* workspace,
+                                             size_t workspace_bytes, void* stream) {
+  WM_REQUIRE(y && y_d && g && save_mean && save_invstd && save_mean_d && save_invstd_d && dy && dy_d && stat_part &&
+                 workspace && stat_tiles > 0,
+             WM_EINVAL);
+  const int rc = bn_shape_check(rows, C, G);
+  if (rc != WM_OK) return rc;
+  WM_REQUIRE(C <= 2048, WM_EUNSUPPORTED);
+  const int rpg = (int)(rows / G);
+  const int nblk_d = reduce_blocks(rpg, C);
+  const size_t scr = stat_scratch_floats(stat_tiles, G, C);
+  WM_REQUIRE(workspace_bytes >= ((size_t)14 * G * C + scr + (size_t)G * nblk_d * 2 * C) * sizeof(float), WM_EWORKSPACE);
+  hipStream_t st = static_cast<hipStream_t>(stream);
+  float* coef = static_cast<float*>(workspace);
+  float* coef_d = coef + (size_t)7 * G * C;
+  float* scratch = coef_d + (size_t)7 * G * C;
+  float* part_d = scratch + scr;
+  int nblk = 0;
+  const float* part = stat_partials(stat_part, stat_tiles, G, C, scratch, &nblk, st);
+  WM_LAUNCH_CHECK();
+  launch_finalize(bn_bwd_finalize, C, st, part, nblk, G, C, rpg, gamma, beta, save_mean, save_invstd, dgamma, dbeta, accumulate,
+                  coef, 1);
+  WM_LAUNCH_CHECK();
+  launch_reduce<1>(bf16(y_d), bf16(g), nullptr, save_mean_d, save_invstd_d, nullptr, nullptr, rpg, C, G, nblk_d, part_d,
+                   PoolSrc{}, st);
+  WM_LAUNCH_CHECK();
+  launch_finalize(bn_bwd_finalize, C, st, part_d, nblk_d, G, C, rpg, gamma_d, beta_d, save_mean_d, save_invstd_d, dgamma_d,
+                  dbeta_d, accumulate_d, coef_d, 0);
+  WM_LAUNCH_CHECK();
+  launch_bn_bwd_apply_sc(bf16(y), bf16(y_d), bf16(g), coef, coef_d, rows, C, rpg, bf16(dy), bf16(dy_d), st);
   WM_LAUNCH_CHECK();
   return WM_OK;
 }
diff --git a/self-supervised-wafermaps_amd/csrc/conv.hip b/self-supervised-wafermaps_amd/csrc/conv.hip
--- a/self-supervised-wafermaps_amd/csrc/conv.hip
+++ b/self-supervised-wafermaps_amd/csrc/conv.hip
@@ -26,6 +26,7 @@
   const float* bn_gamma;
   const float* bn_beta;
   const uint16_t* res;
+  int res_compact;
   const float* bias;
   const uint16_t* pre_in;
   uint16_t* pre_out;
@@ -173,8 +174,8 @@
 __device__ __forceinline__ void bnb_load16(u32x4_t& dst, const void* p) {
   dst = __builtin_nontemporal_load(reinterpret_cast<const u32x4_t*>(p));
 }
-template <int BNC, typename PixOf>
-__device__ __forceinline__ void bnb_prefetch(const ConvArgs& a, BnbRegs<BNC>& R, int n0, int tid, PixOf pix_of) {
+template <int BNC, typename PixOf, typename ResRow>
+__device__ __forceinline__ void bnb_prefetch(const ConvArgs& a, BnbRegs<BNC>& R, int n0, int tid, PixOf pix_of, ResRow res_row) {
   constexpr int CPR = BNC / 8;
   const int c0 = n0 + (tid % CPR) * 8;
 #pragma unroll
@@ -183,7 +184,8 @@
     const size_t pix = pix_of(row);
     R.pixs[it] = pix;
     bnb_load16(R.yv[it], a.bn_y + pix * a.DC + c0);
-    if (a.res != nullptr) bnb_load16(R.rv[it], a.res + pix * a.DC + c0);
+    const long long rrow = res_row(row, pix);
+    if (rrow >= 0) bnb_load16(R.rv[it], a.res + (size_t)rrow * a.DC + c0);
     if (a.bn_x != nullptr) bnb_load16(R.xv[it], a.bn_x + pix * a.DC + c0);
     R.mk[it] = a.bn_mask != nullptr ? a.bn_mask[pix * (a.DC >> 3) + (c0 >> 3)] : 0u;
   }
@@ -191,7 +193,7 @@
 
 template <int BNC>
 __device__ __forceinline__ void bnb_epilogue(const ConvArgs& a, const BnbRegs<BNC>& R, const uint8_t* smem, int CS, float* red,
-                                             StatSlot slot, int n0, int tid) {
+                                             StatSlot slot, int n0, int tid, bool has_res) {
   constexpr int CPR = BNC / 8;
   constexpr int NIT = BnbRegs<BNC>::NIT;
   const int chl = tid % CPR;
@@ -233,7 +235,7 @@
       for (int h = 0; h < 2; ++h) {
         const int e = q * 2 + h;
         float v = __builtin_bit_cast(float, h ? (vv[q] & 0xffff0000u) : (vv[q] << 16));
-        if (a.res != nullptr) v += __builtin_bit_cast(float, h ? (rr[q] & 0xffff0000u) : (rr[q] << 16));
+        if (has_res) v += __builtin_bit_cast(float, h ? (rr[q] & 0xffff0000u) : (rr[q] << 16));
         const float y = __builtin_bit_cast(float, h ? (yy[q] & 0xffff0000u) : (yy[q] << 16));
         const bool keep = remask ? fmaf(y, sc[e], sh[e]) > 0.f
                           : bitmask ? ((R.mk[it] >> e) & 1u) != 0u
@@ -287,6 +289,15 @@
     } else {
       return (size_t)(m0 + row);
     }
+  };
+  bool tile_res = a.res != nullptr;
+  if constexpr (MODE == 2) tile_res = tile_res && (!a.res_compact || m0 < (a.M >> 2));
+  auto res_row = [&](int row, size_t pix) -> long long {
+    if (!tile_res) return -1;
+    if constexpr (MODE == 2) {
+      if (a.res_compact) return (long long)(m0 + row);
+    }
+    return (long long)pix;
   };
   const int rowl = tid >> 3;
   const int chunk = (tid & 7) ^ (rowl & 7);
@@ -447,7 +458,7 @@
 
   BnbRegs<BNB ? BN : 64> bnb;
   if constexpr (BNB) {
-    bnb_prefetch<BN>(a, bnb, n0, tid, row_pixel);
+    bnb_prefetch<BN>(a, bnb, n0, tid, row_pixel, res_row);
   }
   if (nkt > 0) issue(0, smem_base);
   for (int kt = 0; kt < nkt; ++kt) {
@@ -483,7 +494,7 @@
     } else {
       slot = stat_slot(a, m0);
     }
-    bnb_epilogue<BN>(a, bnb, cv_smem, CS, reinterpret_cast<float*>(cv_smem + BM * CS), slot, n0, tid);
+    bnb_epilogue<BN>(a, bnb, cv_smem, CS, reinterpret_cast<float*>(cv_smem + BM * CS), slot, n0, tid, tile_res);
     return;
   }
   if constexpr (EPI) {
@@ -540,7 +551,7 @@
       const size_t pix = row_pixel(row);
       if (m0 + row < a.M) {
         uint4 v = *reinterpret_cast<const uint4*>(cv_smem + row * CS + ch * 16);
-        if (a.res != nullptr) v = bf16x8_add(v, *reinterpret_cast<const uint4*>(a.res + pix * a.DC + n0 + ch * 8));
+        if (tile_res) v = bf16x8_add(v, *reinterpret_cast<const uint4*>(a.res + (size_t)res_row(row, pix) * a.DC + n0 + ch * 8));
         *reinterpret_cast<uint4*>(a.dst + pix * a.DC + n0 + ch * 8) = v;
       }
     }
@@ -598,7 +609,8 @@
   BnbRegs<64> bnb;
   if constexpr (BNB) {
     const size_t org[2] = {pair_origin(a, tn[0], th0[0], tw0[0]), pair_origin(a, tn[1], th0[1], tw0[1])};
-    bnb_prefetch<64>(a, bnb, 0, tid, [&](int row) -> size_t { return pair_pixel(org, row, a.DW); });
+    bnb_prefetch<64>(a, bnb, 0, tid, [&](int row) -> size_t { return pair_pixel(org, row, a.DW); },
+                     [&](int, size_t pix) -> long long { return a.res != nullptr ? (long long)pix : -1; });
   }
   const int rowl = tid >> 3;
   const int wchunk = (tid & 7) ^ (rowl & 7);
@@ -671,7 +683,8 @@
       stage_acc_frag(cv_smem, CS, acc[j][i], wm * 64 + i * 16 + fr, wn * 32 + j * 16 + fg * 4);
   __syncthreads();
   if constexpr (BNB) {
-    bnb_epilogue<64>(a, bnb, cv_smem, CS, reinterpret_cast<float*>(cv_smem + 128 * CS), stat_slot_pair(a, tn[0], bx), 0, tid);
+    bnb_epilogue<64>(a, bnb, cv_smem, CS, reinterpret_cast<float*>(cv_smem + 128 * CS), stat_slot_pair(a, tn[0], bx), 0, tid,
+                     a.res != nullptr);
     return;
   }
   const size_t org[2] = {pair_origin(a, tn[0], th0[0], tw0[0]), pair_origin(a, tn[1], th0[1], tw0[1])};
@@ -1507,8 +1520,9 @@
 };
 
 int conv_dgrad_impl(const void* dy, const void* w_crsk, void* dx, const void* residual, const ConvGeom& g, void* stream,
-                    const void* pre_in = nullptr, const BnbArgs* bnb = nullptr) {
+                    const void* pre_in = nullptr, const BnbArgs* bnb = nullptr, bool res_compact = false) {
   WM_REQUIRE(dy && w_crsk && dx, WM_EINVAL);
+  WM_REQUIRE(!res_compact || residual != nullptr, WM_EINVAL);
   WM_REQUIRE(pre_in == nullptr || (residual == nullptr && g.R == 1 && g.S == 1 && g.stride == 1 && aligned16(pre_in)), WM_EUNSUPPORTED);
   const int rc = conv_check(g);
   if (rc != WM_OK) return rc;
@@ -1523,6 +1537,11 @@
   a.act = pre_in != nullptr ? 2 : 0;
   hipStream_t st = static_cast<hipStream_t>(stream);
   const int route = conv_dgrad_route(g, residual != nullptr, pre_in != nullptr, bnb != nullptr ? bnb->G : 0);
+  if (res_compact) {
+    WM_REQUIRE(g.stride == 2 && dgrad_mode(g) == 2 && pre_in == nullptr, WM_EUNSUPPORTED);
+    WM_REQUIRE(route == route_igemm(g.C, 8, 2, false, bnb != nullptr), WM_EUNSUPPORTED);
+    a.res_compact = 1;
+  }
   if (bnb != nullptr) {
     WM_REQUIRE(pre_in == nullptr, WM_EUNSUPPORTED);
     a.bn_y = static_cast<const uint16_t*>(bnb->bn_y);
@@ -1618,6 +1637,39 @@
              WM_EALIGN);
   BnbArgs b{bn_y, relu_x, relu_mask, save_mean, save_invstd, gamma, beta, G, stat_part, stat_tiles};
   return conv_dgrad_impl(dy, w_crsk, dx, residual, {N, H, W, C, K, R, S, P, Q, stride, pad}, stream, nullptr, &b);
+}
+
+extern "C" int wm_conv2d_dgrad_compact_ok(int N, int H, int W, int C, int K, int R, int S, int P, int Q, int stride,
+                                          int pad) {
+  const ConvGeom g{N, H, W, C, K, R, S, P, Q, stride, pad};
+  return conv_check(g) == WM_OK && g.C % 64 == 0 && g.stride == 2 && dgrad_mode(g) == 2 ? 1 : 0;
+}
+
+extern "C" int wm_conv2d_dgrad_add_compact(const void* dy, const void* w_crsk, const void* residual_compact, void* dx,
+                                           int N, int H, int W, int C, int K, int R, int S, int P, int Q, int stride,
+                                           int pad, void* stream) {
+  WM_REQUIRE(residual_compact, WM_EINVAL);
+  WM_REQUIRE(aligned16(residual_compact), WM_EALIGN);
+  return conv_dgrad_impl(dy, w_crsk, dx, residual_compact, {N, H, W, C, K, R, S, P, Q, stride, pad}, stream, nullptr, nullptr,
+                         true);
+}
+
+extern "C" int wm_conv2d_dgrad_bnstat_compact(const void* dy, const void* w_crsk, const void* residual_compact, void* dx,
+                                              int N, int H, int W, int C, int K, int R, int S, int P, int Q, int stride,
+                                              int pad, const void* bn_y, const void* relu_x, const void* relu_mask,
+                                              const float* gamma, const float* beta, const float* save_mean,
+                                              const float* save_invstd, int G, float* stat_part, int stat_tiles,
+                                              void* stream) {
+  WM_REQUIRE(residual_compact && bn_y && save_mean && save_invstd && stat_part, WM_EINVAL);
+  WM_REQUIRE(G > 0 && stat_tiles == (int)((long long)N * H * W / G / 128), WM_EINVAL);
+  WM_REQUIRE(relu_x || relu_mask || (gamma && beta), WM_EINVAL);
+  WM_REQUIRE(!(relu_x && relu_mask), WM_EINVAL);
+  WM_REQUIRE(wm_conv2d_dgrad_bnstat_ok(N, H, W, C, K, R, S, P, Q, stride, pad, G), WM_EUNSUPPORTED);
+  WM_REQUIRE(aligned16(bn_y) && aligned16(save_mean) && aligned16(save_invstd) && aligned16(relu_x) &&
+                 aligned16(residual_compact),
+             WM_EALIGN);
+  BnbArgs b{bn_y, relu_x, relu_mask, save_mean, save_invstd, gamma, beta, G, stat_part, stat_tiles};
+  return conv_dgrad_impl(dy, w_crsk, dx, residual_compact, {N, H, W, C, K, R, S, P, Q, stride, pad}, stream, nullptr, &b, true);
 }
 
 extern "C" int wm_conv2d_wgrad(const void* dy, const void* x, float* dw_krsc, int N, int H, int W,
diff --git a/self-supervised-wafermaps_amd/models/resnet.py b/self-supervised-wafermaps_amd/models/resnet.py
--- a/self-supervised-wafermaps_amd/models/resnet.py
+++ b/self-supervised-wafermaps_amd/models/resnet.py
@@ -35,12 +35,14 @@
         if self.downsample is not None and torch.is_grad_enabled() and x.requires_grad:
             g = ops.current_bn_groups()
             st = self.bn1.stats_buffer(g) if self.bn1.training else None
-            y, x_alias = self.conv1(x, stats=st, groups=g, passthrough=True)
+            ds = self.downsample[0]
+            y, x_alias = self.conv1(x, stats=st, groups=g, passthrough=True,
+                                    even_pixels=(ds.kernel_size, ds.stride, ds.padding) == (1, 2, 0))
             out = self.bn1(y, relu=True, stats=st)
-            shortcut = conv_bn(self.downsample[0], self.downsample[1], x_alias)
+            shortcut = self._shortcut(x_alias, x if x_alias.shape != x.shape else None)
         elif self.downsample is not None:
             out = conv_bn(self.conv1, self.bn1, x, relu=True)
-            shortcut = conv_bn(self.downsample[0], self.downsample[1], x)
+            shortcut = self._shortcut(x)
         elif torch.is_grad_enabled() and x.requires_grad:
             g = ops.current_bn_groups()
             st = self.bn1.stats_buffer(g) if self.bn1.training else None
@@ -49,7 +51,20 @@
         else:
             out = conv_bn(self.conv1, self.bn1, x, relu=True)
             shortcut = x
+        if isinstance(shortcut, tuple):
+            g = ops.current_bn_groups()
+            st = self.bn2.stats_buffer(g)
+            return self.bn2.forward_shortcut(self.conv2(out, stats=st, groups=g), st, self.downsample[1], *shortcut)
         return conv_bn(self.conv2, self.bn2, out, relu=True, residual=shortcut)
+
+    def _shortcut(self, x, x_full=None):
+        conv, bn = self.downsample
+        g = ops.current_bn_groups()
+        st = bn.stats_buffer(g) if bn.training else None
+        y = conv(x, stats=st, groups=g) if x_full is None else ops.conv2d_downsample(x, x_full, conv.weight, stats=st, groups=g)
+        if self.bn2.shortcut_deferrable(bn):
+            return y, st
+        return bn(y, stats=st)
 
 
 class ResNet18(nn.Module):
diff --git a/self-supervised-wafermaps_amd/nn.py b/self-supervised-wafermaps_amd/nn.py
--- a/self-supervised-wafermaps_amd/nn.py
+++ b/self-supervised-wafermaps_amd/nn.py
@@ -20,9 +20,10 @@
         self.weight = nn.Parameter(torch.empty(out_channels, in_channels, kernel_size, kernel_size))
         nn.init.kaiming_normal_(self.weight, mode="fan_out", nonlinearity="relu")
 
-    def forward(self, x, stats=None, groups=1, passthrough=False):
+    def forward(self, x, stats=None, groups=1, passthrough=False, even_pixels=False):
         if passthrough:
-            return ops.conv2d_passthrough(x, self.weight, self.stride, self.padding, stats=stats, groups=groups)
+            return ops.conv2d_passthrough(x, self.weight, self.stride, self.padding, stats=stats, groups=groups,
+                                          even_pixels=even_pixels)
         return ops.conv2d(x, self.weight, self.stride, self.padding, stats=stats, groups=groups)
 
 
@@ -96,6 +97,21 @@
         return ops.bn_relu_maxpool(x, self.weight, self.bias, rm, rv, self.training,
                                    eps=self.eps, momentum=mom, stats=stats,
                                    num_batches_tracked=self.num_batches_tracked)
+
+    def shortcut_deferrable(self, bn_d: "_BatchNorm") -> bool:
+        return (self.training and bn_d.training and ops.shortcut_fuse() and not _precision.is_f32()
+                and not self._synced() and not bn_d._synced())
+
+    def forward_shortcut(self, y, stats, bn_d: "_BatchNorm", y_d, stats_d):
+        g = ops.current_bn_groups()
+        if not (self.shortcut_deferrable(bn_d) and ops.batch_norm_shortcut_ok(y, y_d, stats, stats_d, g)):
+            return self(y, residual=bn_d(y_d, stats=stats_d), relu=True, stats=stats)
+        bwd = self.stats_buffer(g, "_stat_buf_bwd") if torch.is_grad_enabled() else None
+        rm, rv, mom = self._running()
+        rm_d, rv_d, mom_d = bn_d._running()
+        return ops.batch_norm_shortcut(y, y_d, self.weight, self.bias, (rm, rv), self.num_batches_tracked, self.eps, mom,
+                                       stats, bn_d.weight, bn_d.bias, (rm_d, rv_d), bn_d.num_batches_tracked, bn_d.eps,
+                                       mom_d, stats_d, bwd_stats=bwd, groups=g)
 
 
 class BatchNorm1d(_BatchNorm):
diff --git a/self-supervised-wafermaps_amd/ops.py b/self-supervised-wafermaps_amd/ops.py
--- a/self-supervised-wafermaps_amd/ops.py
+++ b/self-supervised-wafermaps_amd/ops.py
@@ -599,7 +599,12 @@
         ctx.weight = weight
         ctx.geom = geom
         ctx.link = link if (_BN_FUSE_BWD and link is not None and link.y.shape == x.shape) else None
+        ctx.compact = False
         if pass_input:
+            if (pass_input == "even" and stride == 2 and shortcut_fuse() and x.requires_grad
+                    and _lib.load().wm_conv2d_dgrad_compact_ok(*geom)):
+                ctx.compact = True
+                return y, x[:, :, ::2, ::2]
             return y, x.view_as(x)
         return y
 
@@ -621,18 +626,21 @@
                 check(_run("conv_dgrad", 2.0 * n * p * q * k * r * s * c, getattr(lib, entry), dy.data_ptr(), ptr(crsk), *mid,
                            dx.data_ptr(), *ctx.geom, *tail, stream_ptr()), entry)
 
+            sfx = "_compact" if (ctx.compact and dres is not None) else ""
+            if sfx and tuple(dres.shape) != (n, c, h // 2, w // 2):
+                raise ValueError(f"conv2d: compact shortcut gradient {tuple(dres.shape)} for an input {(n, c, h, w)}")
             link = ctx.link
             if (link is not None and not link.ready and getattr(link.stats, "_hip_busy", None) is None
                     and lib.wm_conv2d_dgrad_bnstat_ok(n, h, w, c, k, r, s, p, q, stride, pad, link.groups)):
                 tiles = n * h * w // link.groups // 128
-                dgrad("wm_conv2d_dgrad_bnstat", ptr(dres), tail=(
+                dgrad("wm_conv2d_dgrad_bnstat" + sfx, ptr(dres), tail=(
                     link.y.data_ptr(), x.data_ptr() if (link.has_res and link.mask is None) else 0,
                     ptr(link.mask) if link.has_res else 0, ptr(link.gamma), ptr(link.beta), ptr(link.mean),
                     ptr(link.invstd), link.groups, ptr(link.stats.get(link.groups, tiles, dy.device)), tiles))
                 link.ready, link.g_ptr, link.g_version = True, dx.data_ptr(), dx._version
                 link.stats._hip_busy = True
             elif dres is not None:
-                dgrad("wm_conv2d_dgrad_add", dres.data_ptr())
+                dgrad("wm_conv2d_dgrad_add" + sfx, dres.data_ptr())
             else:
                 dgrad("wm_conv2d_dgrad")
         if ctx.needs_input_grad[1]:
@@ -649,10 +657,54 @@
 
 
 def conv2d_passthrough(x: torch.Tensor, weight: torch.Tensor, stride: int = 1, padding: int = 0,
-                       stats: Optional[torch.Tensor] = None, groups: int = 1):
+                       stats: Optional[torch.Tensor] = None, groups: int = 1, even_pixels: bool = False):
     if _precision.is_f32():
         return f32path.conv2d(x, weight, int(stride), int(padding)), x
-    return _Conv2d.apply(x, weight, int(stride), int(padding), stats, int(groups), True, getattr(x, "_hip_bn", None))
+    return _Conv2d.apply(x, weight, int(stride), int(padding), stats, int(groups), "even" if even_pixels else True,
+                         getattr(x, "_hip_bn", None))
+
+
+class _DownsampleConv(torch.autograd.Function):
+
+    @staticmethod
+    def forward(ctx, x_even, x_full, weight, stats=None, groups=1):
+        x = x_full
+        n, c, h, w = x.shape
+        k = weight.shape[0]
+        p, q = _out_hw(h, w, 1, 1, 2, 0)
+        if tuple(weight.shape) != (k, c, 1, 1) or tuple(x_even.shape) != (n, c, p, q):
+            raise ValueError(f"conv2d_downsample: input {tuple(x.shape)}, even pixels {tuple(x_even.shape)}, weight "
+                             f"{tuple(weight.shape)}")
+        krsc, _ = _WCACHE.get(weight, need_crsk=True)
+        y = _empty_nhwc(n, k, p, q, x.device)
+        geom = (n, h, w, c, k, 1, 1, p, q, 2, 0)
+        _conv_fwd(x, krsc, y, geom, 2.0 * n * p * q * k * c, stats, groups)
+        ctx.save_for_backward(x)
+        ctx.weight = weight
+        ctx.geom = geom
+        return y
+
+    @staticmethod
+    def backward(ctx, dy):
+        (x,) = ctx.saved_tensors
+        weight = ctx.weight
+        n, h, w, c, k, r, s, p, q, stride, pad = ctx.geom
+        dy = _as_nhwc(dy)
+        lib = _lib.load()
+        dx = dw = None
+        if ctx.needs_input_grad[0]:
+            _, crsk = _WCACHE.get(weight, need_crsk=True)
+            dx = _empty_nhwc(n, c, p, q, dy.device)
+            check(_run("conv_dgrad", 2.0 * n * p * q * k * c, lib.wm_conv2d_dgrad, dy.data_ptr(), ptr(crsk), dx.data_ptr(),
+                       n, p, q, c, k, 1, 1, p, q, 1, 0, stream_ptr()), "wm_conv2d_dgrad(downsample)")
+        if ctx.needs_input_grad[2]:
+            slabs, _, ns = wgrad(dy, x, weight, n, h, w, c, k, r, s, p, q, stride, pad)
+            dw, _ = wgrad_deliver(weight, slabs, ns, k, c, r, s)
+        return _pad_grads(ctx, dx, None, dw)
+
+
+def conv2d_downsample(x_even: torch.Tensor, x_full: torch.Tensor, weight: torch.Tensor, stats=None, groups: int = 1):
+    return _DownsampleConv.apply(x_even, _as_nhwc(x_full.detach()), weight, stats, int(groups))
 
 
 class _StemConv(torch.autograd.Function):
@@ -879,6 +931,101 @@
     return out
 
 
+def shortcut_fuse() -> bool:
+    return os.environ.get("WM_SHORTCUT_FUSE", "1") != "0"
+
+
+def _bn_shortcut_workspace(rows: int, c: int, g: int, tiles_a: int, tiles_b: int, device) -> torch.Tensor:
+    ws = _bn_workspace(rows, c, g, device)
+    need = _lib.load().wm_bn_shortcut_workspace_bytes(rows, c, g, tiles_a, tiles_b)
+    if ws.numel() < need:
+        key = (device, torch.cuda.current_stream(device).cuda_stream)
+        ws = _BN_WS[key] = torch.empty(need, dtype=torch.uint8, device=device)
+    return ws
+
+
+class _BatchNormShortcut(torch.autograd.Function):
+
+    @staticmethod
+    def forward(ctx, y, y_d, gamma, beta, gamma_d, beta_d, running, running_d, groups, eps, momentum, eps_d, momentum_d,
+                stats, stats_d, counter, counter_d, bwd_stats):
+        y, y_d, rows, c = _bn_inputs(y, y_d, "batch_norm_shortcut")
+        lib = _lib.load()
+        out = torch.empty_like(y)
+        mean = torch.empty((groups, c), dtype=torch.float32, device=y.device)
+        invstd, mean_d, invstd_d = torch.empty_like(mean), torch.empty_like(mean), torch.empty_like(mean)
+        will_link = bwd_stats is not None and ctx.needs_input_grad[0]
+        mask = torch.empty((rows, c // 8), dtype=torch.uint8, device=y.device) if (will_link and _BN_BITMASK) else None
+        ws = _bn_shortcut_workspace(rows, c, groups, stats.tiles, stats_d.tiles, y.device)
+        check(lib.wm_bn_train_fwd_from_stats_sc(
+            y.data_ptr(), y_d.data_ptr(), ptr(gamma), ptr(beta), ptr(running[0]), ptr(running[1]), ptr(counter),
+            ptr(gamma_d), ptr(beta_d), ptr(running_d[0]), ptr(running_d[1]), ptr(counter_d), rows, c, groups, eps, momentum,
+            eps_d, momentum_d, 1, ptr(mean), ptr(invstd), ptr(mean_d), ptr(invstd_d), out.data_ptr(), ptr(mask),
+            ptr(stats.buf), stats.tiles, ptr(stats_d.buf), stats_d.tiles, ptr(ws), ws.numel(), stream_ptr()),
+            "wm_bn_train_fwd_from_stats_sc")
+        ctx.save_for_backward(y, y_d, out, mean, invstd, mean_d, invstd_d)
+        ctx.affine = (gamma, beta, gamma_d, beta_d)
+        ctx.meta = (rows, c, groups)
+        ctx.branch = current_branch()
+        ctx.link = BnLink(y, mean, invstd, gamma, beta, groups, True, bwd_stats, mask) if will_link else None
+        return out
+
+    @staticmethod
+    def backward(ctx, dout):
+        y, y_d, out, mean, invstd, mean_d, invstd_d = ctx.saved_tensors
+        gamma, beta, gamma_d, beta_d = ctx.affine
+        rows, c, groups = ctx.meta
+        dout = _as_act(dout)
+        lib = _lib.load()
+        dy, dy_d = torch.empty_like(y), torch.empty_like(y_d)
+        dgamma, dbeta, direct, finish = _bn_param_grads(gamma, beta, c, y.device, ctx.branch)
+        dgamma_d, dbeta_d, direct_d, finish_d = _bn_param_grads(gamma_d, beta_d, c, y.device, ctx.branch)
+        link = ctx.link
+        fused = False
+        if link is not None and link.ready:
+            link.ready = False
+            link.stats._hip_busy = None
+            if dout.data_ptr() == link.g_ptr and dout._version == link.g_version:
+                ws = _bn_shortcut_workspace(rows, c, groups, link.stats.tiles, 0, y.device)
+                check(lib.wm_bn_train_bwd_from_stats_sc(
+                    y.data_ptr(), y_d.data_ptr(), dout.data_ptr(), ptr(gamma), ptr(beta), ptr(mean), ptr(invstd),
+                    ptr(gamma_d), ptr(beta_d), ptr(mean_d), ptr(invstd_d), rows, c, groups, ptr(dgamma), ptr(dbeta),
+                    int(direct), ptr(dgamma_d), ptr(dbeta_d), int(direct_d), dy.data_ptr(), dy_d.data_ptr(),
+                    ptr(link.stats.buf), link.stats.tiles, ptr(ws), ws.numel(), stream_ptr()),
+                    "wm_bn_train_bwd_from_stats_sc")
+                fused = True
+        if not fused:
+            ws = _bn_workspace(rows, c, groups, y.device)
+            dz = torch.empty_like(y)
+            check(lib.wm_bn_train_bwd(y.data_ptr(), dout.data_ptr(), out.data_ptr(), 0, ptr(gamma), ptr(beta), ptr(mean),
+                                      ptr(invstd), rows, c, groups, ptr(dgamma), ptr(dbeta), int(direct), dy.data_ptr(),
+                                      dz.data_ptr(), ptr(ws), ws.numel(), stream_ptr()), "wm_bn_train_bwd")
+            check(lib.wm_bn_train_bwd(y_d.data_ptr(), dz.data_ptr(), 0, 0, ptr(gamma_d), ptr(beta_d), ptr(mean_d),
+                                      ptr(invstd_d), rows, c, groups, ptr(dgamma_d), ptr(dbeta_d), int(direct_d),
+                                      dy_d.data_ptr(), 0, ptr(ws), ws.numel(), stream_ptr()), "wm_bn_train_bwd")
+        return _pad_grads(ctx, dy, dy_d, *finish(), *finish_d())
+
+
+def batch_norm_shortcut_ok(y, y_d, stats, stats_d, groups: int) -> bool:
+    if not shortcut_fuse() or _precision.is_f32() or y.dim() != 4 or y.shape != y_d.shape or not y.is_cuda:
+        return False
+    rows, c = _rows_c(y)
+    return (stats is not None and stats_d is not None and stats.buf is not None and stats_d.buf is not None
+            and stats_fusable(rows, groups) and c % 8 == 0 and c <= 2048)
+
+
+def batch_norm_shortcut(y, y_d, gamma, beta, running, counter, eps, momentum, stats, gamma_d, beta_d, running_d, counter_d,
+                        eps_d, momentum_d, stats_d, bwd_stats=None, groups: Optional[int] = None):
+    g = current_bn_groups() if groups is None else groups
+    out = _BatchNormShortcut.apply(y, y_d, gamma, beta, gamma_d, beta_d, running, running_d, int(g), float(eps),
+                                   float(momentum), float(eps_d), float(momentum_d), stats, stats_d, counter, counter_d,
+                                   bwd_stats)
+    link = getattr(out.grad_fn, "link", None) if out.grad_fn is not None else None
+    if link is not None:
+        out._hip_bn = link
+    return out
+
+
 class _SyncBatchNorm(torch.autograd.Function):
 
     @staticmethod
```
